# sieste/greb-climate-model

Measured on AMD Instinct MI355X. Metric: simulated-years/sec at 96x48 grid (ensemble aggregate); diffusion HBM GB/s vs roofline, higher is better.
Workload: dtype f32; 1 GPU; 96x48 GREB ensemble, 512 members/GPU x 1 GPU, CO2 sweep 280-1120 ppm, 32 scenario years after 1 flux-correction year, dt=12h, dt_crcl=0.5h; members_per_gpu=512, arithmetic=fast, gather=none (1 GPU)

## Files before the change

greb_climate_model_amd/csrc/greb_device.h:

```cpp
#pragma once
#include <hip/hip_runtime.h>

namespace greb {

constexpr int kMaxNy = 192;

struct RowTables {
  float dif_ccy, adv_ccy;
  float dif_ccx[kMaxNy], adv_ccx[kMaxNy];
  float dif_ccx2[kMaxNy], adv_ccx2[kMaxNy];
  int dif_time2[kMaxNy], adv_time2[kMaxNy];
  int subcycled[kMaxNy];
};

struct f4 {
  float v[4];
};

typedef __attribute__((address_space(3))) float lfloat;
typedef float vfloat4 __attribute__((ext_vector_type(4)));

__device__ __forceinline__ f4 ld4(const float* p) {
  const vfloat4 a = *reinterpret_cast<const vfloat4*>(p);
  return f4{{a.x, a.y, a.z, a.w}};
// ... 180 lines not shown
  }
}

__device__ __forceinline__ void adv_lon_full_fast(const Flux& f, const float T[12], const float w[12],
                                                  const float u[4], float cs, float d[4]) {
#pragma unroll
  for (int i = 0; i < 4; ++i) {
    const int c = 4 + i;
    const float em2 = w[c - 2] * (T[c] - T[c - 2]), ep2 = w[c + 2] * (T[c] - T[c + 2]);
    d[i] = cs * (split_p(u[i]) * (ep2 - f.Pp[c]) - split_m(u[i]) * (f.Pm[c - 1] + em2));
  }
}

__device__ __forceinline__ void adv_lon_sub_fast(const Flux& f, const float T[12], const float w[12],
                                                 const float u[4], float cs, bool last_quad, float d[4]) {
#pragma unroll
  for (int i = 0; i < 4; ++i) {
    const int c = 4 + i;
    const float am = 10.f * f.Pm[c - 1] + (4.f * f.Pm[c - 2] + f.Pm[c - 3]);
    float ap = 10.f * f.Pp[c] + (4.f * f.Pp[c + 1] + f.Pp[c + 2]);
    if (last_quad && i == 1)
      ap = 10.f * f.Pp[c] - w[c + 3] * (T[c + 1] - T[c + 3]);
    d[i] = cs * (-split_p(u[i]) * ap - split_m(u[i]) * am);
  }
}

__device__ __forceinline__ void clamp_add_fast(float T1h[4], float d[4]) {
#pragma unroll
  for (int i = 0; i < 4; ++i) {
    d[i] = (d[i] <= -T1h[i]) ? -0.9f * T1h[i] : d[i];
    T1h[i] = T1h[i] + d[i];
  }
}

__device__ __forceinline__ void lat_fast(const f4& T0, const f4& Tm2, const f4& Tm1, const f4& Tp1,
                                         const f4& Tp2, const f4& wm2, const f4& wm1, const f4& wp1,
                                         const f4& wp2, const float v[4], float ccy_dif, float am, float ap,
                                         float ddif[4], float dadv[4]) {
#pragma unroll
  for (int i = 0; i < 4; ++i) {
    const float t0 = T0.v[i];
    const float gm1 = wm1.v[i] * (Tm1.v[i] - t0), gp1 = wp1.v[i] * (Tp1.v[i] - t0);
    const float dm2 = wm2.v[i] * (t0 - Tm2.v[i]), dp2 = wp2.v[i] * (t0 - Tp2.v[i]);
    ddif[i] = ccy_dif * (gm1 + gp1);
    dadv[i] = ap * split_p(v[i]) * (dp2 - gp1) - am * split_m(v[i]) * (dm2 - gm1);
  }
}


__device__ __forceinline__ void adv_lon_full_pm(const Flux& f, const float T[12], const float w[12],
                                                const float um[4], const float up[4], float d[4]) {
#pragma unroll
  for (int i = 0; i < 4; ++i) {
    const int c = 4 + i;
    const float em2 = w[c - 2] * (T[c] - T[c - 2]), ep2 = w[c + 2] * (T[c] - T[c + 2]);
    d[i] = up[i] * (ep2 - f.Pp[c]) - um[i] * (f.Pm[c - 1] + em2);
  }
}
__device__ __forceinline__ void adv_lon_sub_pm(const Flux& f, const float T[12], const float w[12],
                                               const float um[4], const float up[4], bool last_quad, float d[4]) {
#pragma unroll
  for (int i = 0; i < 4; ++i) {
    const int c = 4 + i;
    const float am = 10.f * f.Pm[c - 1] + (4.f * f.Pm[c - 2] + f.Pm[c - 3]);
    float ap = 10.f * f.Pp[c] + (4.f * f.Pp[c + 1] + f.Pp[c + 2]);
    if (last_quad && i == 1) ap = 10.f * f.Pp[c] - w[c + 3] * (T[c + 1] - T[c + 3]);
    d[i] = -up[i] * ap - um[i] * am;
  }
}
__device__ __forceinline__ void lat_pm(const f4& T0, const f4& Tm2, const f4& Tm1, const f4& Tp1, const f4& Tp2,
                                       const f4& wm2, const f4& wm1, const f4& wp1, const f4& wp2,
                                       const float vm[4], const float vp[4], float ccy_dif, float ddif[4],
                                       float dadv[4]) {
#pragma unroll
  for (int i = 0; i < 4; ++i) {
    const float t0 = T0.v[i];
    const float gm1 = wm1.v[i] * (Tm1.v[i] - t0), gp1 = wp1.v[i] * (Tp1.v[i] - t0);
    const float dm2 = wm2.v[i] * (t0 - Tm2.v[i]), dp2 = wp2.v[i] * (t0 - Tp2.v[i]);
    ddif[i] = ccy_dif * (gm1 + gp1);
    dadv[i] = vp[i] * (dp2 - gp1) - vm[i] * (dm2 - gm1);
  }
}

__device__ __forceinline__ float wave_sum(float v) {
#pragma unroll
  for (int off = 32; off > 0; off >>= 1) v += __shfl_xor(v, off, 64);
  return v;
}

template <bool EXACT> __device__ __forceinline__ float fdiv(float a, float b) { return EXACT ? a / b : a * __builtin_amdgcn_rcpf(b); }
template <bool EXACT> __device__ __forceinline__ float flog(float x) { return EXACT ? logf(x) : __logf(x); }
template <bool EXACT> __device__ __forceinline__ float fexp(float x) { return EXACT ? expf(x) : __expf(x); }
template <bool EXACT> __device__ __forceinline__ float fsqrt(float x) { return EXACT ? sqrtf(x) : __builtin_amdgcn_sqrtf(x); }

constexpr unsigned kXNoIce = 1u << 0, kXNoHydro = 1u << 1, kXNoDeepOcean = 1u << 2, kXLwLinear = 1u << 3,
                   kXNoCirc = 1u << 4, kXNoQTransport = 1u << 5, kXQDiffOnly = 1u << 6, kXSstPlus1 = 1u << 7;

struct Phys {
  float sig, ct_sens, da_ice, a_no_ice, a_cloud, Tl_ice1, Tl_ice2, To_ice1, To_ice2;
  float co_turb, ce, cq_latent, cq_rain, z_air, r_qviwv, rho_air;
  float p_emi[10];
  float cap_ocean, cap_land, cap_air;
  float dt;
};

__device__ __forceinline__ float pow4_ref(float x) {
#pragma clang fp contract(off)
  return x * x * x * x;
}

template <bool EXACT = true>
__device__ __forceinline__ void sw_radiation(const Phys& P, float Ts, float z_topo, float glacier, float cld,
                                             float sw_solar, float& albedo, float& sw, unsigned xsw = 0) {
#pragma clang fp contract(off)
  const float a_atmos = cld * P.a_cloud;
  float a_surf = 0.f;
  if (z_topo >= 0.f) {
    if (Ts <= P.Tl_ice1) a_surf = P.a_no_ice + P.da_ice;
    if (Ts >= P.Tl_ice2) a_surf = P.a_no_ice;
    if (Ts > P.Tl_ice1 && Ts < P.Tl_ice2)
      a_surf = P.a_no_ice + P.da_ice * (1.f - fdiv<EXACT>(Ts - P.Tl_ice1, P.Tl_ice2 - P.Tl_ice1));
  } else {
    if (Ts <= P.To_ice1) a_surf = P.a_no_ice + P.da_ice;
    if (Ts >= P.To_ice2) a_surf = P.a_no_ice;
    if (Ts > P.To_ice1 && Ts < P.To_ice2)
      a_surf = P.a_no_ice + P.da_ice * (1.f - fdiv<EXACT>(Ts - P.To_ice1, P.To_ice2 - P.To_ice1));
  }
  if (glacier > 0.5f) a_surf = P.a_no_ice + P.da_ice;
  if (xsw & kXNoIce) a_surf = P.a_no_ice;
  albedo = a_surf + a_atmos - a_surf * a_atmos;
  sw = sw_solar * (1.f - albedo);
}

template <bool EXACT = true>
__device__ __forceinline__ void lw_radiation(const Phys& P, float Ts, float Ta, float q, float co2, float ez,
                                             float cld, float tclim, float& LWsurf, float& LWair_down,
                                             float& em, unsigned xsw = 0, float qclim = 0.f) {
#pragma clang fp contract(off)
  const float e_co2 = ez * co2;
  float e_vapor = ez * P.r_qviwv * q;
  if (xsw & kXLwLinear) e_vapor = ez * P.r_qviwv * qclim;
  float e = P.p_emi[3] * flog<EXACT>(P.p_emi[0] * e_co2 + P.p_emi[1] * e_vapor + P.p_emi[2]) + P.p_emi[6]
            + P.p_emi[4] * flog<EXACT>(P.p_emi[0] * e_co2 + P.p_emi[2])
            + P.p_emi[5] * flog<EXACT>(P.p_emi[1] * e_vapor + P.p_emi[2]);
  e = fdiv<EXACT>(P.p_emi[7] - cld, P.p_emi[8]) * (e - P.p_emi[9]) + P.p_emi[9];
  if (xsw & kXLwLinear) e = e + 0.022f / (0.15f * 24.f) * P.r_qviwv * (q - qclim);
  em = e;
  LWsurf = -P.sig * pow4_ref(Ts);
  const float dTrad = -0.16f * tclim - 5.f;
  LWair_down = -e * P.sig * pow4_ref(Ta + dTrad);
}

template <bool EXACT = true>
__device__ __forceinline__ void hydro(const Phys& P, float Ts, float q, float u, float v, float z_topo,
                                      float ez, float swet, float& Qlat, float& Qlat_air, float& dq_eva,
                                      float& dq_rain, unsigned xsw = 0) {
#pragma clang fp contract(off)
  if (xsw & kXNoHydro) { Qlat = Qlat_air = dq_eva = dq_rain = 0.f; return; }
  float abswind = fsqrt<EXACT>(u * u + v * v);
  if (z_topo > 0.f) abswind = fsqrt<EXACT>(abswind * abswind + 2.0f * 2.0f);
  if (z_topo < 0.f) abswind = fsqrt<EXACT>(abswind * abswind + 3.0f * 3.0f);
  float qs = 3.75e-3f * fexp<EXACT>(fdiv<EXACT>(17.08085f * (Ts - 273.15f), Ts - 273.15f + 234.175f));
  qs = qs * ez;
  Qlat = (q - qs) * abswind * P.cq_latent * P.rho_air * P.ce * swet;
  dq_eva = fdiv<EXACT>(fdiv<EXACT>(-Qlat, P.cq_latent), P.r_qviwv);
  dq_rain = P.cq_rain * q;
  Qlat_air = -dq_rain * P.cq_latent * P.r_qviwv;
}

template <bool EXACT = true>
__device__ __forceinline__ void deep_ocean(const Phys& P, float Ts, float To, float z_topo, float mld,
                                           float mld_prev, float z_ocean, float& dT_ocean, float& dTo,
                                           unsigned xsw = 0) {
#pragma clang fp contract(off)
  if (xsw & kXNoDeepOcean) { dT_ocean = dTo = 0.f; return; }
  float a = 0.f, b = 0.f;
  const float dmld = mld - mld_prev;
  if (z_topo < 0.f && Ts >= P.To_ice2 && dmld < 0.f) a = fdiv<EXACT>(-dmld, z_ocean - mld) * (Ts - To);
  if (z_topo < 0.f && Ts >= P.To_ice2 && dmld > 0.f) b = fdiv<EXACT>(dmld, mld) * (To - Ts);
  a = 0.5f * a; b = 0.5f * b;
  const float Tx = P.To_ice2 > Ts ? P.To_ice2 : Ts;
  a = a + fdiv<EXACT>(P.dt * P.co_turb * (Tx - To), P.cap_ocean * (z_ocean - mld));
  b = b + fdiv<EXACT>(P.dt * P.co_turb * (To - Tx), P.cap_ocean * mld);
  dTo = a; dT_ocean = b;
}

template <bool EXACT = true>
__device__ __forceinline__ float seaice(const Phys& P, float Ts, float z_topo, float glacier, float mld,
                                        float cap_surf, unsigned xsw = 0) {
#pragma clang fp contract(off)
  if (z_topo < 0.f) {
    if (Ts <= P.To_ice1) cap_surf = P.cap_land;
    if (Ts >= P.To_ice2) cap_surf = P.cap_ocean * mld;
    if (Ts > P.To_ice1 && Ts < P.To_ice2)
      cap_surf = P.cap_land + fdiv<EXACT>(P.cap_ocean * mld - P.cap_land, P.To_ice2 - P.To_ice1) * (Ts - P.To_ice1);
  }
  if (xsw & kXNoIce) {
    if (z_topo > 0.f) cap_surf = P.cap_land;
    if (z_topo < 0.f) cap_surf = P.cap_ocean * mld;
  }
  if (glacier > 0.5f) cap_surf = P.cap_land;
  return cap_surf;
}

}
```

greb_climate_model_amd/csrc/greb_engine.cpp:

```cpp
#include "../../include/greb_engine.h"

#include <hip/hip_runtime.h>

#include <cmath>
#include <cstdlib>
#include <cstdio>
#include <cstring>
#include <functional>
#include <map>
#include <mutex>
#include <new>
#include <string>
#include <vector>

#include "greb_kernels.h"
#include "greb_diag.h"
#include "greb_clim.h"
#include "greb_ens.h"

using namespace greb;

namespace {

thread_local std::string g_last_error;

int fail(greb_engine* e, int code, const std::string& msg);

#define HIP_TRY(e, expr)                                                                      \
  do {                                                                                        \
    hipError_t _err = (expr);                                                                 \
    if (_err != hipSuccess)                                                                   \
      return fail((e), (int)_err, std::string(#expr) + ": " + hipGetErrorString(_err));       \
  } while (0)

int nint_f(float x) { return (int)lroundf(x); }

void compute_row_tables(const greb_params& p, float kappa, int nx, int ny, RowTables& g) {
  std::memset(&g, 0, sizeof(g));
  const float dlon = 360.f / (float)nx, dlat = 180.f / (float)ny;
  const float deg = 2.f * p.pi * 6.371e6f / 360.f;
  const float dx = dlon, dy = dlat, dyy = dy * deg;
  const float dtc = (float)p.dt_crcl;
  g.dif_ccy = kappa * dtc / (dyy * dyy);
  g.adv_ccy = dtc / dyy / 2.f;
  for (int k = 0; k < ny; ++k) {
    const float lat = dlat * (float)(k + 1) - dlat / 2.f - 90.f;
    const float dxlat = dx * deg * cosf(2.f * p.pi / 360.f * lat);
    g.dif_ccx[k] = kappa * dtc / (dxlat * dxlat);
    g.adv_ccx[k] = dtc / dxlat / 2.f;
    g.subcycled[k] = !(dxlat > 2.5e5f);
    {
      float dd = (float)nint_f(dtc / (1.f * (dxlat * dxlat) / kappa));
      if (dd < 1.f) dd = 1.f;
      const int dtdff2 = (int)(dtc / dd);
      int t2 = dtdff2 == 0 ? 1 : nint_f(dtc / (float)dtdff2);
      g.dif_time2[k] = t2 < 1 ? 1 : t2;
      g.dif_ccx2[k] = kappa * (float)dtdff2 / (dxlat * dxlat);
    }
    {
      float dd = (float)nint_f(dtc / (dxlat / 10.0f / 1.f));
      if (dd < 1.f) dd = 1.f;
      const int dtdff2 = (int)(dtc / dd);
      int t2 = dtdff2 == 0 ? 1 : nint_f(dtc / (float)dtdff2);
      g.adv_time2[k] = t2 < 1 ? 1 : t2;
      g.adv_ccx2[k] = (float)dtdff2 / dxlat / 2.f;
    }
  }
}

Phys make_phys(const greb_params& p) {
  Phys P;
  P.sig = p.sig; P.ct_sens = p.ct_sens;
  P.da_ice = p.da_ice; P.a_no_ice = p.a_no_ice; P.a_cloud = p.a_cloud;
  P.Tl_ice1 = p.Tl_ice1; P.Tl_ice2 = p.Tl_ice2; P.To_ice1 = p.To_ice1; P.To_ice2 = p.To_ice2;
  P.co_turb = p.co_turb; P.ce = p.ce; P.cq_latent = p.cq_latent; P.cq_rain = p.cq_rain;
  P.z_air = p.z_air; P.r_qviwv = p.r_qviwv; P.rho_air = p.rho_air;
  for (int i = 0; i < 10; ++i) P.p_emi[i] = p.p_emi[i];
  P.cap_ocean = p.cp_ocean * p.rho_ocean;
  P.cap_land = p.cp_land * p.rho_land * p.d_land;
  P.cap_air = p.cp_air * p.rho_air * p.d_air;
  P.dt = (float)p.dt;
  return P;
}

template <typename T>
hipError_t dev_alloc(T** p, size_t n) { return hipMalloc(reinterpret_cast<void**>(p), n * sizeof(T)); }

struct StripPlan {
  RowsTask* step_tasks = nullptr;
  int n_step = 0;
  RowsTask head[kStepHeadTasks] = {};
  CircOrder circ;
  int form = 0;
  float ms_substep = 0.f, ms_call = 0.f;
  hipEvent_t ev[3] = {nullptr, nullptr, nullptr};
};

void free_plan(StripPlan& p) {
  if (p.step_tasks) (void)hipFree(p.step_tasks);
  circ_rows_free_order(&p.circ);
  for (hipEvent_t ev : p.ev) if (ev) (void)hipEventDestroy(ev);
  p = StripPlan{};
}

}

struct greb_engine {
  greb_params p{};
  int nx = 0, ny = 0, np = 0, nm = 0, device = 0;
  bool strict = false;
  unsigned xsw = 0;
  std::vector<unsigned> h_xsw;
  bool xsw_uniform = true;
  unsigned* xsw_dev = nullptr;
  float* co2_flux_dev = nullptr;
  int n_phys_sets = 1;
  bool shared_corr = true;
  bool fused = true;
  float *Xa = nullptr, *Xb = nullptr, *red = nullptr, *W2 = nullptr;
  hipStream_t stream = nullptr;
  hipStream_t copy_stream = nullptr;
  hipEvent_t ev_done[2] = {nullptr, nullptr};
  hipEvent_t ev_free[2] = {nullptr, nullptr};
  float *z_topo = nullptr, *glacier = nullptr, *sw_solar = nullptr;
  float *tclim = nullptr, *qclim = nullptr, *uclim = nullptr, *vclim = nullptr, *mldclim = nullptr,
        *cldclim = nullptr, *swetclim = nullptr;
  float *toclim = nullptr, *z_ocean = nullptr, *wz_air = nullptr, *wz_vapor = nullptr;
  float *state = nullptr, *acc = nullptr, *corr = nullptr;
  int *corr_index = nullptr, *tab_index = nullptr;
  RowTables* tabs = nullptr;
  Phys* phys = nullptr;
  float* co2_dev = nullptr; size_t co2_cap = 0;
  float* monthly_dev = nullptr; size_t monthly_cap = 0;
  float* bsum = nullptr;
  float* budget_dev = nullptr; size_t budget_cap = 0;
  long long budget_runs = 0;
  int n_patterns = 0, n_solar = 0;
  float *f_space = nullptr, *f_season = nullptr, *f_solar = nullptr;
  std::vector<greb_member_forcing> h_force;
  MemberForcing* force_dev = nullptr;
  int forced_members = 0;
  struct BoundSet {
    float* dev[kBoundaryFields] = {};
    bool own[kBoundaryFields] = {};
    unsigned over = 0;
    std::vector<float> t_last, q_last, toclim, z_topo, mld0;
  };
  std::vector<BoundSet> bound;
  std::vector<int> h_bset;
  int members_on_sets = 0;
  BoundarySet* bsets_dev = nullptr;
  int* bset_dev = nullptr;
  MemberForcing* neutral_force_dev = nullptr;
  float* yearly_dev = nullptr; size_t yearly_cap = 0;
  float* diag_out = nullptr; size_t diag_out_cap = 0;
  float* diag_reg = nullptr; size_t diag_reg_cap = 0;
  float* clim_out = nullptr; size_t clim_out_cap = 0;
  float* ens_out = nullptr; size_t ens_out_cap = 0;
  std::vector<RowTables> h_tabs;
  std::vector<int> h_tab_index;
  bool strips = false;
  enum { kCallNever, kCallTrial, kCallAlways } call = kCallNever;
  int cus = 0;
  int slots_granted = -1;
  std::map<int, StripPlan> plans;
  std::vector<Phys> h_phys;
  long long it_flux = 0;
  long long it_scnr = 0;
  unsigned long long* stamps = nullptr;
  std::string last_error;
};

namespace {
int fail(greb_engine* e, int code, const std::string& msg) {
  if (e) e->last_error = msg;
  g_last_error = msg;
  return code;
}

int nsub_of(const greb_params& p) {
  int t = nint_f((float)p.dt / (float)p.dt_crcl);
  return t < 1 ? 1 : t;
}

MemberArgs base_args(greb_engine* e) {
  MemberArgs a{};
  a.nx = e->nx; a.ny = e->ny; a.np = e->np;
  a.z_topo = e->z_topo; a.glacier = e->glacier; a.sw_solar = e->sw_solar;
  a.tclim = e->tclim; a.qclim = e->qclim; a.uclim = e->uclim; a.vclim = e->vclim;
  a.mldclim = e->mldclim; a.cldclim = e->cldclim; a.swetclim = e->swetclim;
  a.toclim = e->toclim; a.z_ocean = e->z_ocean; a.wz_air = e->wz_air; a.wz_vapor = e->wz_vapor;
  a.state = e->state; a.acc = e->acc; a.corr = e->corr; a.corr_index = e->corr_index;
  a.tabs = e->tabs; a.tab_index = e->tab_index; a.phys = e->phys;
  a.nsub = nsub_of(e->p);
  a.nsub = tuning_int("GREB_DEBUG_NSUB", a.nsub);
  a.co2_flux = e->p.co2_flux;
  a.ipx = e->p.ipx; a.ipy = e->p.ipy;
  a.xsw = e->xsw_uniform ? e->xsw : 0u;
  a.xsw_m = e->xsw_uniform ? nullptr : e->xsw_dev;
  a.co2_flux_m = e->co2_flux_dev;
  a.stamps = e->stamps;
  a.dbg = tuning_int("GREB_DEBUG_PHYS", 0);
  unsigned all = GREB_X_NO_CIRCULATION;
  for (unsigned x : e->h_xsw) all &= x;
  if (all) a.nsub = 0;
  if (e->members_on_sets > 0) { a.bsets = e->bsets_dev; a.bset_m = e->bset_dev; }
  return a;
}

void apply_forcing(const greb_engine* e, MemberArgs& a) {
  if (e->forced_members <= 0 && e->members_on_sets > 0) a.force_m = e->neutral_force_dev;
  if (e->forced_members <= 0) return;
  a.force_m = e->force_dev;
  a.f_space = e->f_space; a.f_season = e->f_season; a.f_solar = e->f_solar;
}

struct YearOut {
  float* mon; int mon_years, mon_y;
  float* bud = nullptr; int bud_years = 0, bud_y = 0;
};

MemberArgs scenario_args(greb_engine* e, int years, int y, const YearOut& o) {
  MemberArgs a = base_args(e);
  a.flux_phase = 0;
  a.it0 = e->it_scnr + 1 + (long long)y * kNT; a.nsteps = kNT;
  a.co2 = e->co2_dev; a.co2_stride = years; a.co2_year0 = y;
  a.monthly = o.mon; a.monthly_years = o.mon_years; a.year_out0 = o.mon_y;
  a.yearly = e->yearly_dev; a.yearly_years = years; a.yearly_year0 = y;
  if (o.bud) { a.bsum = e->bsum; a.brec = o.bud; a.brec_years = o.bud_years; a.brec_year0 = o.bud_y; }
  apply_forcing(e, a);
  return a;
}

bool is_forced(const greb_member_forcing& f) { return f.co2_pattern >= 0 || f.solar_table >= 0 || !(f.solar_scale == 1.f); }

bool calm_vapor(const greb_engine* e) { return (e->h_xsw[0] & GREB_X_VAPOR_DIFFUSION_ONLY) != 0; }

int check_transport_switches(greb_engine* e, const char* who, bool fused, const unsigned* sw, int n) {
  if (fused) return 0;
  for (int m = 1; m < n; ++m)
    if ((sw[m] ^ sw[0]) & GREB_X_VAPOR_DIFFUSION_ONLY)
      return fail(e, GREB_E_UNSUPPORTED,
                  std::string(who) + ": member " + std::to_string(m) + " differs from member 0 in GREB_X_VAPOR_DIFFUSION_ONLY, "
                  "which the any-grid engine applies to a whole launch -- run the two groups as two engines beside each "
                  "other (ensemble.run_beside)");
  return 0;
}

bool all_equal(const unsigned* sw, int n) {
  for (int m = 1; m < n; ++m) if (sw[m] != sw[0]) return false;
  return true;
}

int check_member_config(const char* who, const greb_params& p, const greb_member_config& c, int m) {
  const char* bad = nullptr;
  auto differ = [](float a, float b) { return std::memcmp(&a, &b, sizeof(float)) != 0; };
  if (differ(c.p.pi, p.pi)) bad = "pi";
  else if (differ(c.p.z_air, p.z_air)) bad = "z_air";
  else if (differ(c.p.z_vapor, p.z_vapor)) bad = "z_vapor";
  else if (c.p.dt != p.dt) bad = "dt";
  else if (c.p.dt_crcl != p.dt_crcl) bad = "dt_crcl";
  else if (c.p.ipx != p.ipx) bad = "ipx";
  else if (c.p.ipy != p.ipy) bad = "ipy";
  else if (c.p.year0 != p.year0) bad = "year0";
  if (bad)
    return fail(nullptr, GREB_E_INVALID, std::string(who) + ": member " + std::to_string(m) + ": " + bad +
                                             " differs from the engine-wide greb_params (it feeds data every member shares)");
  if (c.switches & ~0xffu)
    return fail(nullptr, GREB_E_INVALID, std::string(who) + ": member " + std::to_string(m) + ": unknown switch bits");
  return 0;
}

int ensure(greb_engine* e, float** buf, size_t* cap, size_t n) {
  if (*cap >= n) return 0;
  if (*buf) HIP_TRY(e, hipFree(*buf));
  *buf = nullptr; *cap = 0;
  HIP_TRY(e, dev_alloc(buf, n));
  *cap = n;
  return 0;
}

struct SlotLedger {
  std::mutex mu;
  struct Entry { greb_engine* e; int device, members, granted; };
  std::vector<Entry> entries;
} g_slots;

void ledger_register(greb_engine* e) {
  std::lock_guard<std::mutex> lock(g_slots.mu);
  g_slots.entries.push_back({e, e->device, e->nm, 0});
}
void ledger_release(greb_engine* e) {
  std::lock_guard<std::mutex> lock(g_slots.mu);
  for (size_t i = 0; i < g_slots.entries.size(); ++i)
    if (g_slots.entries[i].e == e) { g_slots.entries.erase(g_slots.entries.begin() + (long)i); break; }
}
int ledger_grant(greb_engine* e, int device_slots) {
  std::lock_guard<std::mutex> lock(g_slots.mu);
  long long members = 0, taken = 0;
  SlotLedger::Entry* mine = nullptr;
  for (auto& x : g_slots.entries) {
    if (x.device != e->device) continue;
    members += x.members;
    if (x.e == e) mine = &x; else taken += x.granted;
  }
  if (!mine) return 0;
  const long long share = (long long)device_slots * mine->members / std::max<long long>(1, members);
  mine->granted = (int)std::max<long long>(0, std::min<long long>(share, device_slots - taken));
  return mine->granted;
}

int check_circulation(greb_engine* e) {
  for (auto& kv : e->plans) {
    unsigned d[5] = {0, 0, 0, 0, 0};
    const int rc = circ_rows_status(kv.second.circ, d);
    if (rc == -1) {
      char buf[384];
      std::snprintf(buf, sizeof(buf),
                    "circulation launch given up: task %u waited more than %.1f s in sub-step %u for a neighbouring strip "
                    "(its count read %u, wanted %u) -- the launch was not resident as a whole (another process on the "
                    "device?); results are invalid, recreate the engine with GREB_F_NO_PERSISTENT",
                    d[0], kCircSpinTicks / 1e8, d[1], d[2], d[3]);
      return fail(e, GREB_E_STATE, buf);
    }
    if (rc) return fail(e, GREB_E_STATE, "circulation launch: status word unreadable");
  }
  return 0;
}

int make_strip_plan(greb_engine* e, int nrun, StripPlan& p) {
  if (e->cus <= 0) HIP_TRY(e, hipDeviceGetAttribute(&e->cus, hipDeviceAttributeMultiprocessorCount, e->device));
  if (e->call != greb_engine::kCallNever) {
    static const int slots_per_cu = tuning_int("GREB_CIRC_SLOTS_PER_CU", kStepRowsSlotsPerCu);
    if (e->slots_granted < 0) e->slots_granted = ledger_grant(e, e->cus * std::min(slots_per_cu, kStepRowsSlotsPerCu));
    HIP_TRY(e, circ_rows_make_order(e->h_tabs.data(), e->h_tab_index.data(), nrun, e->ny, e->slots_granted, &p.circ));
  }
  p.form = p.circ.n == 0 ? 1 : (e->call == greb_engine::kCallAlways ? 2 : 0);
  if (p.form != 2) {
    static const int step_slots = tuning_int("GREB_STEP_SLOTS_PER_CU", kStepRowsSlotsPerCu);
    HIP_TRY(e, step_rows_make_tasks(e->h_tabs.data(), e->h_tab_index.data(), nrun, e->ny, e->cus * step_slots, &p.step_tasks,
                                    &p.n_step, p.head));
  }
  if (p.form == 0)
    for (hipEvent_t& ev : p.ev) HIP_TRY(e, hipEventCreate(&ev));
  return 0;
}

int run_year(greb_engine* e, const MemberArgs& a, int nrun) {
  if (e->fused) {
    HIP_TRY(e, launch_member_kernel(a, nrun, e->strict, e->stream));
    return 0;
  }
  const size_t np = (size_t)e->np;
  StripPlan* plan = nullptr;
  if (e->strips && a.nsub > 0) {
    auto it = e->plans.find(nrun);
    if (it == e->plans.end()) {
      StripPlan p;
      if (int rc = make_strip_plan(e, nrun, p)) { free_plan(p); return rc; }
      it = e->plans.emplace(nrun, p).first;
    }
    plan = &it->second;
  }
  static const int steps = tuning_int("GREB_DEBUG_NSTEPS", kNT);
  bool trial = plan && plan->form == 0 && steps >= 16;
  int form = plan && plan->form != 1 ? 2 : 1;
  HIP_TRY(e, launch_pack_tracers(e->state, e->Xa, e->np, nrun, e->stream));
  for (int s = 0; s < steps; ++s) {
    const long long it = a.it0 + s;
    const int ityr = (int)((it - 1) % kNT) + 1;
    const size_t off = (size_t)(ityr - 1) * np;
    float *cur = e->Xa, *nxt = e->Xb;
    if (trial) {
      if (s == 2 || s == 5 || s == 8) HIP_TRY(e, hipEventRecord(plan->ev[s == 2 ? 0 : (s == 5 ? 1 : 2)], e->stream));
      if (s == 8) {
        HIP_TRY(e, hipEventSynchronize(plan->ev[2]));
        HIP_TRY(e, hipEventElapsedTime(&plan->ms_substep, plan->ev[0], plan->ev[1]));
        HIP_TRY(e, hipEventElapsedTime(&plan->ms_call, plan->ev[1], plan->ev[2]));
        form = plan->form = plan->ms_call <= plan->ms_substep ? 2 : 1;
        trial = false;
      } else form = (s >= 2 && s < 5) ? 1 : 2;
    }
    if (form == 2) {
      HIP_TRY(e, launch_circulation_rows(e->Xa, e->Xb, e->W2, e->uclim + off, e->vclim + off, e->tabs, plan->circ, e->cus * 4, e->nx, e->ny,
                                         a.nsub, e->strict, e->stream, calm_vapor(e)));
      if (a.nsub & 1) cur = e->Xb;
    } else
    for (int tt = 0; tt < a.nsub; ++tt) {
      if (plan)
        HIP_TRY(e, launch_substep_rows(cur, e->W2, e->uclim + off, e->vclim + off, nxt, e->tabs, e->tab_index, plan->step_tasks,
                                       plan->head, plan->n_step, e->cus * 4, e->nx, e->ny, e->strict, e->stream, calm_vapor(e)));
      else
        HIP_TRY(e, launch_substep_fused(cur, e->W2, e->uclim + off, e->vclim + off, nxt, e->tabs, e->tab_index, e->nx,
                                        e->ny, nrun, e->strict, e->stream, calm_vapor(e)));
      float* t = cur; cur = nxt; nxt = t;
    }
    MemberArgs b = a;
    b.it0 = it; b.nsteps = 1;
    HIP_TRY(e, launch_physics_step(b, cur, e->Xa, e->red, nrun, e->strict, e->stream));
    if (ityr == kNT && a.yearly)
      HIP_TRY(e, launch_yearly(e->red, a.yearly, e->np, e->nx, a.ipx, a.ipy, a.yearly_years, a.yearly_year0, nrun, e->strict, e->stream));
  }
  return 0;
}
}

extern "C" {

void greb_params_default(greb_params* p) {
  std::memset(p, 0, sizeof(*p));
  p->pi = 3.1416f; p->sig = 5.6704e-8f; p->rho_ocean = 999.1f; p->rho_land = 2600.f; p->rho_air = 1.2f;
  p->cp_ocean = 4186.f; p->cp_land = 926.222f; p->cp_air = 1005.f; p->eps = 1.f;
  p->d_ocean = 50.f; p->d_land = 2.f; p->d_air = 5000.f; p->ct_sens = 22.5f; p->da_ice = 0.25f;
  p->a_no_ice = 0.1f; p->a_cloud = 0.35f;
  p->Tl_ice1 = 273.15f - 10.f; p->Tl_ice2 = 273.15f; p->To_ice1 = 273.15f - 7.f; p->To_ice2 = 273.15f - 1.7f;
  p->co_turb = 5.0f; p->kappa = 8e5f; p->ce = 2e-3f; p->cq_latent = 2.257e6f;
  p->cq_rain = -0.1f / 24.f / 3600.f; p->z_air = 8400.f; p->z_vapor = 5000.f; p->r_qviwv = 2.6736e3f;
  const float pe[10] = {9.0721f, 106.7252f, 61.5562f, 0.0179f, 0.0028f, 0.0570f, 0.3462f, 2.3406f, 0.7032f, 1.0662f};
  std::memcpy(p->p_emi, pe, sizeof(pe));
  p->co2_flux = 298.f;
  p->ipx = 1; p->ipy = 1; p->year0 = 1940; p->dt = 12 * 3600; p->dt_crcl = 1800;
}

const char* greb_engine_last_error(const greb_engine* e) {
  return e ? e->last_error.c_str() : g_last_error.c_str();
}

const char* greb_device_info(int device) {
  static thread_local std::string s;
  int n = 0;
  if (hipGetDeviceCount(&n) != hipSuccess || n <= device || device < 0) {
    s = "{\"error\": \"no HIP device\"}";
    return s.c_str();
  }
  hipDeviceProp_t pr;
  if (hipGetDeviceProperties(&pr, device) != hipSuccess) { s = "{\"error\": \"hipGetDeviceProperties\"}"; return s.c_str(); }
  char buf[512];
  std::snprintf(buf, sizeof(buf),
                "{\"name\": \"%s\", \"arch\": \"%s\", \"cus\": %d, \"clock_mhz\": %d, \"mem_clock_mhz\": %d, "
                "\"hbm_gb\": %.1f, \"lds_per_block\": %zu, \"l2_mb\": %.1f, \"wave\": %d}",
                pr.name, pr.gcnArchName, pr.multiProcessorCount, pr.clockRate / 1000, pr.memoryClockRate / 1000,
                pr.totalGlobalMem / 1073741824.0, pr.sharedMemPerBlock, pr.l2CacheSize / 1048576.0, pr.warpSize);
  s = buf;
  return s.c_str();
}

}

namespace {
void derive_fields(const greb_params& p, size_t np, const float* z_topo, const float* tclim, const float* mldclim, float* toclim,
                   float* z_ocean, float* wz_air, float* wz_vapor) {
  for (size_t i = 0; i < np; ++i) {
    if (tclim) {
      float mn = tclim[i];
      for (int t = 0; t < kNT; ++t) { const float v = tclim[(size_t)t * np + i]; if (v < mn) mn = v; }
      if (mn - 273.15f < -1.7f) mn = -1.7f + 273.15f;
      toclim[i] = mn;
    }
    if (mldclim) {
      float mx = 0.f;
      for (int t = 0; t < kNT; ++t) { const float d = mldclim[(size_t)t * np + i]; if (d > mx) mx = d; }
      z_ocean[i] = 3.0f * mx;
    }
    if (z_topo) {
      wz_air[i] = expf(-z_topo[i] / p.z_air);
      wz_vapor[i] = expf(-z_topo[i] / p.z_vapor);
    }
  }
}

void initial_state(const greb_engine::BoundSet& b, const Phys& P, size_t np, float* st) {
  for (size_t i = 0; i < np; ++i) {
    st[i] = b.t_last[i]; st[np + i] = st[i]; st[2 * np + i] = b.toclim[i]; st[3 * np + i] = b.q_last[i];
    float c = 0.f;
    if (b.z_topo[i] > 0.f) c = P.cap_land;
    if (b.z_topo[i] <= 0.f) c = P.cap_ocean * b.mld0[i];
    st[4 * np + i] = c;
  }
}

const char* const kBoundaryNames[kBoundaryFields] = {"z_topo", "glacier", "tclim", "qclim", "uclim", "vclim", "mldclim", "cldclim",
                                                     "swetclim", "toclim", "z_ocean", "wz_air", "wz_vapor"};
enum { kBfZtopo, kBfGlacier, kBfTclim, kBfQclim, kBfUclim, kBfVclim, kBfMld, kBfCld, kBfSwet, kBfToclim, kBfZocean, kBfWzAir, kBfWzVapor };
size_t boundary_floats(int field, size_t np) { return (field >= kBfTclim && field <= kBfSwet) ? np * kNT : np; }

hipError_t copy_shared_corrections(greb_engine* e, float** corr, const char** what) {
  const size_t nm = (size_t)e->nm, set = (size_t)3 * kNT * e->np;
  hipError_t err = hipStreamSynchronize(e->stream);
  *what = "hipStreamSynchronize";
  if (err != hipSuccess) return err;
  *what = "hipMalloc of the members' correction sets";
  if ((err = dev_alloc(corr, nm * set)) != hipSuccess) return err;
  *what = "hipMemcpy";
  for (size_t m = 0; m < nm; ++m)
    if ((err = hipMemcpy(*corr + m * set, e->corr, set * sizeof(float), hipMemcpyDeviceToDevice)) != hipSuccess) return err;
  return hipSuccess;
}
hipError_t adopt_member_corrections(greb_engine* e, float* corr) {
  std::vector<int> corr_index((size_t)e->nm);
  for (int m = 0; m < e->nm; ++m) corr_index[(size_t)m] = m;
  hipError_t err = hipMemcpy(e->corr_index, corr_index.data(), corr_index.size() * sizeof(int), hipMemcpyHostToDevice);
  if (err != hipSuccess) return err;
  (void)hipFree(e->corr);
  e->corr = corr;
  e->shared_corr = false;
  return hipSuccess;
}

int create_engine(const char* who, const greb_params* p, int nx, int ny, const greb_fields* f, int n_members,
                  const greb_member_config* members, int device, unsigned flags, greb_engine** out) {
  if (!p || !f || !out || !members || n_members < 1 || nx < 12 || (nx & 3) || ny < 5 || ny > kMaxNy)
    return fail(nullptr, GREB_E_INVALID, std::string(who) + ": bad argument");
  for (int m = 0; m < n_members; ++m)
    if (int rc = check_member_config(who, *p, members[m], m)) return rc;
  int ndev = 0;
  if (hipGetDeviceCount(&ndev) != hipSuccess || ndev < 1 || device < 0 || device >= ndev)
    return fail(nullptr, GREB_E_NOGPU, std::string(who) + ": no HIP device (the engine has no CPU path)");
  bool fused = true;
  std::vector<unsigned> switches((size_t)n_members);
  for (int m = 0; m < n_members; ++m) {
    RowTables t; compute_row_tables(*p, members[m].p.kappa, nx, ny, t);
    fused = fused && member_layout_supported(t, nx, ny);
    switches[(size_t)m] = members[m].switches;
  }
  fused = fused && !(flags & GREB_F_MULTILAUNCH);
  if (p->ipx < 1 || p->ipx > nx || p->ipy < 1 || p->ipy > ny)
    return fail(nullptr, GREB_E_INVALID, std::string(who) + ": ipx/ipy outside the grid");
  if (int rc = check_transport_switches(nullptr, who, fused, switches.data(), n_members)) return rc;
  greb_engine* e = new (std::nothrow) greb_engine();
  if (!e) return fail(nullptr, GREB_E_INVALID, "out of host memory");
  *out = e;
  e->p = *p; e->nx = nx; e->ny = ny; e->np = nx * ny; e->nm = n_members; e->device = device;
  e->strict = (flags & GREB_F_STRICT) != 0;
  e->fused = fused;
  e->h_xsw = switches;
  e->xsw_uniform = all_equal(switches.data(), n_members);
  e->xsw = e->xsw_uniform ? switches[0] : 0u;
  const size_t np = (size_t)e->np, n3 = np * kNT, nm = (size_t)n_members;
  HIP_TRY(e, hipSetDevice(device));
  HIP_TRY(e, hipStreamCreate(&e->stream));

  auto up = [&](float** d, const float* h, size_t n) -> hipError_t {
    hipError_t err = dev_alloc(d, n);
    if (err != hipSuccess) return err;
    return hipMemcpy(*d, h, n * sizeof(float), hipMemcpyHostToDevice);
  };
  HIP_TRY(e, up(&e->z_topo, f->z_topo, np));
  HIP_TRY(e, up(&e->glacier, f->glacier, np));
  HIP_TRY(e, up(&e->sw_solar, f->sw_solar, (size_t)kNT * ny));
  HIP_TRY(e, up(&e->tclim, f->tclim, n3));
  HIP_TRY(e, up(&e->qclim, f->qclim, n3));
  HIP_TRY(e, up(&e->uclim, f->uclim, n3));
  HIP_TRY(e, up(&e->vclim, f->vclim, n3));
  HIP_TRY(e, up(&e->mldclim, f->mldclim, n3));
  HIP_TRY(e, up(&e->cldclim, f->cldclim, n3));
  HIP_TRY(e, up(&e->swetclim, f->swetclim, n3));

  std::vector<float> toclim(np), z_ocean(np), wz_air(np), wz_vapor(np);
  derive_fields(*p, np, f->z_topo, f->tclim, f->mldclim, toclim.data(), z_ocean.data(), wz_air.data(), wz_vapor.data());
  HIP_TRY(e, up(&e->toclim, toclim.data(), np));
  HIP_TRY(e, up(&e->z_ocean, z_ocean.data(), np));
  HIP_TRY(e, up(&e->wz_air, wz_air.data(), np));
  HIP_TRY(e, up(&e->wz_vapor, wz_vapor.data(), np));
  {
    const size_t last = (size_t)(kNT - 1) * np;
    greb_engine::BoundSet b0;
    float* const dev[kBoundaryFields] = {e->z_topo, e->glacier, e->tclim, e->qclim, e->uclim, e->vclim, e->mldclim, e->cldclim,
                                         e->swetclim, e->toclim, e->z_ocean, e->wz_air, e->wz_vapor};
    for (int i = 0; i < kBoundaryFields; ++i) b0.dev[i] = dev[i];
    b0.t_last.assign(f->tclim + last, f->tclim + last + np); b0.q_last.assign(f->qclim + last, f->qclim + last + np);
    b0.toclim = toclim; b0.z_topo.assign(f->z_topo, f->z_topo + np); b0.mld0.assign(f->mldclim, f->mldclim + np);
    e->bound.push_back(std::move(b0));
  }

  e->h_phys.resize(nm);
  std::vector<int> tab_index(nm), corr_index(nm);
  std::vector<float> kappas;
  e->shared_corr = true;
  std::vector<float> co2_flux(nm);
  bool own_co2_flux = false;
  std::vector<size_t> phys_sets;
  for (size_t m = 0; m < nm; ++m) {
    e->h_phys[m] = make_phys(members[m].p);
    const float kap = members[m].p.kappa;
    co2_flux[m] = members[m].p.co2_flux;
    own_co2_flux = own_co2_flux || !(co2_flux[m] == p->co2_flux);
    size_t ps = 0;
    for (; ps < phys_sets.size(); ++ps) if (!std::memcmp(&e->h_phys[phys_sets[ps]], &e->h_phys[m], sizeof(Phys))) break;
    if (ps == phys_sets.size()) phys_sets.push_back(m);
    size_t ti = 0;
    for (; ti < kappas.size(); ++ti) if (kappas[ti] == kap) break;
    if (ti == kappas.size()) {
      kappas.push_back(kap);
      RowTables t; compute_row_tables(*p, kap, nx, ny, t);
      e->h_tabs.push_back(t);
    }
    tab_index[m] = (int)ti;
    if (ps != 0 || ti != 0 || !(co2_flux[m] == co2_flux[0]) || switches[m] != switches[0]) e->shared_corr = false;
  }
  e->n_phys_sets = (int)phys_sets.size();
  if (own_co2_flux) {
    HIP_TRY(e, dev_alloc(&e->co2_flux_dev, nm));
    HIP_TRY(e, hipMemcpy(e->co2_flux_dev, co2_flux.data(), nm * sizeof(float), hipMemcpyHostToDevice));
  }
  if (!e->xsw_uniform) {
    HIP_TRY(e, dev_alloc(&e->xsw_dev, nm));
    HIP_TRY(e, hipMemcpy(e->xsw_dev, switches.data(), nm * sizeof(unsigned), hipMemcpyHostToDevice));
  }
  for (size_t m = 0; m < nm; ++m) corr_index[m] = e->shared_corr ? 0 : (int)m;
  HIP_TRY(e, dev_alloc(&e->phys, nm));
  HIP_TRY(e, hipMemcpy(e->phys, e->h_phys.data(), nm * sizeof(Phys), hipMemcpyHostToDevice));
  HIP_TRY(e, dev_alloc(&e->tabs, e->h_tabs.size()));
  HIP_TRY(e, hipMemcpy(e->tabs, e->h_tabs.data(), e->h_tabs.size() * sizeof(RowTables), hipMemcpyHostToDevice));
  HIP_TRY(e, dev_alloc(&e->tab_index, nm));
  HIP_TRY(e, hipMemcpy(e->tab_index, tab_index.data(), nm * sizeof(int), hipMemcpyHostToDevice));
  e->h_tab_index = tab_index;
  HIP_TRY(e, dev_alloc(&e->corr_index, nm));
  HIP_TRY(e, hipMemcpy(e->corr_index, corr_index.data(), nm * sizeof(int), hipMemcpyHostToDevice));

  const size_t ncorr = e->shared_corr ? 1 : nm;
  HIP_TRY(e, dev_alloc(&e->corr, ncorr * 3 * n3));
  HIP_TRY(e, hipMemset(e->corr, 0, ncorr * 3 * n3 * sizeof(float)));
  HIP_TRY(e, dev_alloc(&e->acc, nm * 6 * np));
  HIP_TRY(e, hipMemset(e->acc, 0, nm * 6 * np * sizeof(float)));

  std::vector<float> st(5 * np);
  HIP_TRY(e, dev_alloc(&e->state, nm * 5 * np));
  for (size_t m = 0; m < nm; ++m) {
    initial_state(e->bound[0], e->h_phys[m], np, st.data());
    HIP_TRY(e, hipMemcpy(e->state + m * 5 * np, st.data(), 5 * np * sizeof(float), hipMemcpyHostToDevice));
  }
  if (!e->fused) {
    HIP_TRY(e, dev_alloc(&e->Xa, nm * 2 * np));
    HIP_TRY(e, dev_alloc(&e->Xb, nm * 2 * np));
    HIP_TRY(e, dev_alloc(&e->red, nm * np));
    HIP_TRY(e, dev_alloc(&e->W2, 2 * np));
    HIP_TRY(e, hipMemcpy(e->W2, wz_air.data(), np * sizeof(float), hipMemcpyHostToDevice));
    HIP_TRY(e, hipMemcpy(e->W2 + np, wz_vapor.data(), np * sizeof(float), hipMemcpyHostToDevice));
    static const bool no_step_rows = tuning_int("GREB_NO_STEP_ROWS", 0) != 0;
    e->strips = !no_step_rows && (!e->strict || (flags & GREB_F_ROW_STRIPS)) &&
                n_members < (1 << (kStepFieldBits - 1)) &&
                step_rows_supported(e->h_tabs.data(), (int)e->h_tabs.size(), nx, ny);
    if (e->strips && !(flags & GREB_F_NO_PERSISTENT)) {
      e->call = (flags & GREB_F_PERSISTENT) ? greb_engine::kCallAlways : greb_engine::kCallTrial;
      ledger_register(e);
    }
  }
  return 0;
}

int clear_yearly(greb_engine* e, int years) {
  const size_t n = (size_t)e->nm * years * 2;
  if (int rc = ensure(e, &e->yearly_dev, &e->yearly_cap, n)) return rc;
  HIP_TRY(e, hipMemsetAsync(e->yearly_dev, 0, n * sizeof(float), e->stream));
  return 0;
}
int finish_years(greb_engine* e) {
  HIP_TRY(e, hipStreamSynchronize(e->stream));
  return check_circulation(e);
}
int yearly_to_host(greb_engine* e, int years, float* yearly) {
  if (yearly) HIP_TRY(e, hipMemcpy(yearly, e->yearly_dev, (size_t)e->nm * years * 2 * sizeof(float), hipMemcpyDeviceToHost));
  return 0;
}

size_t year_records(const greb_engine* e) { return (size_t)e->nm * 12 * 5 * (size_t)e->np; }
float* staging_slot(const greb_engine* e, int y) { return e->monthly_dev + (size_t)(y & 1) * year_records(e); }

hipError_t unit_to_host(greb_engine* e, float* host, int n, int u, const float* dev, size_t rec) {
  return hipMemcpy2DAsync(host + (size_t)u * rec, (size_t)n * rec * sizeof(float), dev, rec * sizeof(float), rec * sizeof(float),
                          (size_t)e->nm, hipMemcpyDeviceToHost, e->copy_stream);
}

struct YearCalls {
  std::function<int(int y, const YearOut& o)> integrate;
  std::function<int(int u)> writing;
  std::function<int(int u)> complete;
};

struct RunSink {
  std::function<int()> prepare;
  std::function<int(const YearCalls&, int y)> year;
  std::function<int(int u, int slot)> deliver;
  std::function<int()> finish;
};

int run_years(greb_engine* e, int years, const float* co2_ppm, float* yearly, const RunSink& s) {
  HIP_TRY(e, hipSetDevice(e->device));
  const size_t nm = (size_t)e->nm;
  if (int rc = ensure(e, &e->co2_dev, &e->co2_cap, nm * years)) return rc;
  HIP_TRY(e, hipMemcpyAsync(e->co2_dev, co2_ppm, nm * years * sizeof(float), hipMemcpyHostToDevice, e->stream));
  if (int rc = clear_yearly(e, years)) return rc;
  const bool delivers = (bool)s.deliver;
  if (delivers) if (int rc = ensure(e, &e->monthly_dev, &e->monthly_cap, 2 * year_records(e))) return rc;
  if (int rc = s.prepare()) { e->last_error = g_last_error; return rc; }
  if (delivers && !e->copy_stream) HIP_TRY(e, hipStreamCreateWithFlags(&e->copy_stream, hipStreamNonBlocking));
  for (int i = 0; delivers && i < 2; ++i) {
    if (!e->ev_done[i]) HIP_TRY(e, hipEventCreateWithFlags(&e->ev_done[i], hipEventDisableTiming));
    if (!e->ev_free[i]) HIP_TRY(e, hipEventCreateWithFlags(&e->ev_free[i], hipEventDisableTiming));
  }
  int completed = 0, delivered = 0;
  YearCalls calls;
  calls.integrate = [&](int y, const YearOut& o) -> int { return run_year(e, scenario_args(e, years, y, o), e->nm); };
  calls.writing = [&](int u) -> int {
    if (u >= 2) HIP_TRY(e, hipStreamWaitEvent(e->stream, e->ev_free[u & 1], 0));
    return 0;
  };
  calls.complete = [&](int u) -> int {
    HIP_TRY(e, hipEventRecord(e->ev_done[u & 1], e->stream));
    completed = u + 1;
    return 0;
  };
  auto deliver = [&](int u) -> int {
    HIP_TRY(e, hipStreamWaitEvent(e->copy_stream, e->ev_done[u & 1], 0));
    if (int rc = s.deliver(u, u & 1)) return rc;
    HIP_TRY(e, hipEventRecord(e->ev_free[u & 1], e->copy_stream));
    return 0;
  };
  const int rc_years = [&]() -> int {
    for (int y = 0; y < years; ++y) {
      const int before = completed;
      if (int rc = s.year(calls, y)) return rc;
      for (; delivered < before; ++delivered) if (int rc = deliver(delivered)) return rc;
    }
    for (; delivered < completed; ++delivered) if (int rc = deliver(delivered)) return rc;
    if (delivers) HIP_TRY(e, hipStreamSynchronize(e->copy_stream));
    return 0;
  }();
  if (rc_years && delivers) {
    (void)hipStreamSynchronize(e->copy_stream);
    (void)hipStreamSynchronize(e->stream);
  }
  if (rc_years) return rc_years;
  if (int rc = finish_years(e)) return rc;
  e->it_scnr += (long long)years * kNT;
  if (s.finish) if (int rc = s.finish()) return rc;
  return yearly_to_host(e, years, yearly);
}

int run_records(greb_engine* e, int years, const float* co2_ppm, float* monthly, float* budget, float* yearly,
                unsigned run_flags) {
  const size_t np = (size_t)e->np, nm = (size_t)e->nm;
  const size_t rec_year = 12 * 5 * np, bud_year = (size_t)12 * GREB_NBUDGET * np;
  const bool dev_out = (run_flags & GREB_RUN_DEVICE_OUT) != 0;
  auto budget_slot = [&](int y) { return e->budget_dev + (size_t)(y & 1) * nm * bud_year; };
  RunSink s;
  s.prepare = [&]() -> int {
    if (!budget) return 0;
    if (!e->bsum) {
      HIP_TRY(e, dev_alloc(&e->bsum, nm * GREB_NBUDGET * np));
      HIP_TRY(e, hipMemsetAsync(e->bsum, 0, nm * GREB_NBUDGET * np * sizeof(float), e->stream));
    }
    ++e->budget_runs;
    if (!dev_out) return ensure(e, &e->budget_dev, &e->budget_cap, 2 * nm * bud_year);
    return monthly ? 0 : ensure(e, &e->monthly_dev, &e->monthly_cap, year_records(e));
  };
  if (dev_out) {
    s.year = [&](const YearCalls& run, int y) -> int {
      return run.integrate(y, monthly ? YearOut{monthly, years, y, budget, years, y} : YearOut{e->monthly_dev, 1, 0, budget, years, y});
    };
    return run_years(e, years, co2_ppm, yearly, s);
  }
  s.year = [&](const YearCalls& run, int y) -> int {
    if (int rc = run.writing(y)) return rc;
    if (int rc = run.integrate(y, {staging_slot(e, y), 1, 0, budget ? budget_slot(y) : nullptr, 1, 0})) return rc;
    return run.complete(y);
  };
  s.deliver = [&](int y, int sl) -> int {
    if (monthly) HIP_TRY(e, unit_to_host(e, monthly, years, y, staging_slot(e, sl), rec_year));
    if (budget) HIP_TRY(e, unit_to_host(e, budget, years, y, budget_slot(sl), bud_year));
    return 0;
  };
  return run_years(e, years, co2_ppm, yearly, s);
}
}

extern "C" {

int greb_engine_create_members(const greb_params* p, int nx, int ny, const greb_fields* f, int n_members,
                               const greb_member_config* members, int device, unsigned flags, greb_engine** out) {
  return create_engine("greb_engine_create_members", p, nx, ny, f, n_members, members, device, flags, out);
}

int greb_engine_create(const greb_params* p, int nx, int ny, const greb_fields* f, int n_members,
                       const greb_member_overrides* overrides, int device, unsigned flags, greb_engine** out) {
  if (!p || n_members < 1) return fail(nullptr, GREB_E_INVALID, "greb_engine_create: bad argument");
  std::vector<greb_member_config> members((size_t)n_members);
  auto pick = [](float base, float ov) { return std::isnan(ov) ? base : ov; };
  for (int m = 0; m < n_members; ++m) {
    greb_member_config& c = members[(size_t)m];
    c.p = *p; c.switches = 0;
    if (!overrides) continue;
    c.p.da_ice = pick(p->da_ice, overrides[m].da_ice);
    c.p.a_no_ice = pick(p->a_no_ice, overrides[m].a_no_ice);
    c.p.a_cloud = pick(p->a_cloud, overrides[m].a_cloud);
    c.p.kappa = pick(p->kappa, overrides[m].kappa);
  }
  return create_engine("greb_engine_create", p, nx, ny, f, n_members, members.data(), device, flags, out);
}

int greb_engine_destroy(greb_engine* e) {
  if (!e) return 0;
  (void)hipSetDevice(e->device);
  void* ptrs[] = {e->z_topo, e->glacier, e->sw_solar, e->tclim, e->qclim, e->uclim, e->vclim, e->mldclim,
                  e->cldclim, e->swetclim, e->toclim, e->z_ocean, e->wz_air, e->wz_vapor, e->state, e->acc,
                  e->corr, e->corr_index, e->tab_index, e->tabs, e->phys, e->co2_dev, e->monthly_dev, e->yearly_dev,
                  e->Xa, e->Xb, e->red, e->W2, e->xsw_dev, e->co2_flux_dev, e->diag_out, e->diag_reg, e->clim_out, e->ens_out, e->bsum, e->budget_dev,
                  e->f_space, e->f_season, e->f_solar, e->force_dev, e->bsets_dev, e->bset_dev, e->neutral_force_dev};
  for (void* q : ptrs) if (q) (void)hipFree(q);
  for (size_t k = 1; k < e->bound.size(); ++k)
    for (int i = 0; i < kBoundaryFields; ++i) if (e->bound[k].own[i]) (void)hipFree(e->bound[k].dev[i]);
  for (auto& kv : e->plans) free_plan(kv.second);
  if (e->call != greb_engine::kCallNever) ledger_release(e);
  for (int i = 0; i < 2; ++i) {
    if (e->ev_done[i]) (void)hipEventDestroy(e->ev_done[i]);
    if (e->ev_free[i]) (void)hipEventDestroy(e->ev_free[i]);
  }
  if (e->copy_stream) (void)hipStreamDestroy(e->copy_stream);
  if (e->stream) (void)hipStreamDestroy(e->stream);
  delete e;
  return 0;
}

int greb_engine_flux_correction(greb_engine* e, int years, float* yearly) {
  if (!e || years < 0) return fail(e, GREB_E_INVALID, "flux_correction: bad argument");
  if (years == 0) return 0;
  HIP_TRY(e, hipSetDevice(e->device));
  const size_t np = (size_t)e->np;
  const int nrun = e->shared_corr ? 1 : e->nm;
  if (int rc = clear_yearly(e, years)) return rc;
  for (int y = 0; y < years; ++y) {
    MemberArgs a = base_args(e);
    a.flux_phase = 1;
    a.it0 = e->it_flux + 1 + (long long)y * kNT; a.nsteps = kNT;
    a.monthly = nullptr; a.monthly_years = years; a.year_out0 = y;
    a.yearly = e->yearly_dev; a.yearly_years = years; a.yearly_year0 = y;
    if (int rc = run_year(e, a, nrun)) return rc;
  }
  if (e->shared_corr && e->nm > 1) {
    for (int m = 1; m < e->nm; ++m)
      HIP_TRY(e, hipMemcpyAsync(e->state + (size_t)m * 5 * np, e->state, 5 * np * sizeof(float),
                                hipMemcpyDeviceToDevice, e->stream));
  }
  if (int rc = finish_years(e)) return rc;
  e->it_flux += (long long)years * kNT;
  if (int rc = yearly_to_host(e, years, yearly)) return rc;
  if (yearly && e->shared_corr)
    for (int m = 1; m < e->nm; ++m) std::memcpy(yearly + (size_t)m * years * 2, yearly, (size_t)years * 2 * sizeof(float));
  return 0;
}

int greb_engine_run(greb_engine* e, int years, const float* co2_ppm, float* monthly, float* yearly,
                    unsigned run_flags) {
  if (!e || years < 1 || !co2_ppm || !monthly) return fail(e, GREB_E_INVALID, "run: bad argument");
  return run_records(e, years, co2_ppm, monthly, nullptr, yearly, run_flags);
}

int greb_engine_run_budget(greb_engine* e, int years, const float* co2_ppm, float* monthly, float* budget, float* yearly,
                           unsigned run_flags) {
  if (!e || years < 1 || !co2_ppm) return fail(e, GREB_E_INVALID, "run_budget: bad argument (engine, years or co2_ppm)");
  if (!budget) return fail(e, GREB_E_INVALID, "run_budget: `budget` is NULL (greb_engine_run is the run without budget output)");
  return run_records(e, years, co2_ppm, monthly, budget, yearly, run_flags);
}

const char* greb_budget_name(int i) {
  static const char* const names[GREB_NBUDGET] = {"sw", "LW_surf", "LWair_down", "LW_abs", "Q_sens", "Q_lat", "Q_lat_air",
                                                  "dq_eva", "dq_rain", "dT_ocean", "dTo", "dTa_crcl", "dq_crcl"};
  return i >= 0 && i < GREB_NBUDGET ? names[i] : nullptr;
}

}

struct greb_diag {
  int nx = 0, ny = 0, nr = 0;
  std::vector<double> w;
  std::vector<double> inv_sum;
  struct Dev { int device; double* w; double* inv_sum; double* partials; size_t partials_cap; };
  std::vector<Dev> devs;
};

namespace {
int diag_on_device(greb_diag* d, int device, int n_members, bool regions, greb_diag::Dev** out) {
  greb_diag::Dev* dv = nullptr;
  for (auto& x : d->devs) if (x.device == device) dv = &x;
  if (!dv) {
    greb_diag::Dev n{device, nullptr, nullptr, nullptr, 0};
    HIP_TRY(nullptr, dev_alloc(&n.w, d->w.size()));
    hipError_t err = dev_alloc(&n.inv_sum, d->inv_sum.size());
    if (err == hipSuccess) err = hipMemcpy(n.w, d->w.data(), d->w.size() * sizeof(double), hipMemcpyHostToDevice);
    if (err == hipSuccess) err = hipMemcpy(n.inv_sum, d->inv_sum.data(), d->inv_sum.size() * sizeof(double), hipMemcpyHostToDevice);
    if (err != hipSuccess) {
      (void)hipFree(n.w);
      if (n.inv_sum) (void)hipFree(n.inv_sum);
      HIP_TRY(nullptr, err);
    }
    d->devs.push_back(n);
    dv = &d->devs.back();
  }
  const size_t need = regions ? diag_partials(d->nx, d->ny, n_members, d->nr) : 0;
  if (dv->partials_cap < need) {
    if (dv->partials) {
      HIP_TRY(nullptr, hipDeviceSynchronize());
      HIP_TRY(nullptr, hipFree(dv->partials));
      dv->partials = nullptr; dv->partials_cap = 0;
    }
    HIP_TRY(nullptr, dev_alloc(&dv->partials, need));
    dv->partials_cap = need;
  }
  *out = dv;
  return 0;
}

DiagArgs diag_args(const greb_diag* d, const greb_diag::Dev* dv, const float* monthly, float* regions, size_t regions_stride,
                   float* zonal, float* annual) {
  DiagArgs a{};
  a.monthly = monthly; a.nx = d->nx; a.ny = d->ny; a.nr = d->nr;
  a.w = dv->w; a.inv_sum = dv->inv_sum; a.partials = dv->partials;
  a.regions = regions; a.regions_stride = regions_stride; a.zonal = zonal; a.annual = annual;
  return a;
}
}

extern "C" {

int greb_diag_create(int nx, int ny, const float* region_w, int n_regions, greb_diag** out) {
  if (!out) return fail(nullptr, GREB_E_INVALID, "diag_create: `out` is NULL");
  *out = nullptr;
  if (nx < 12 || (nx & 3) || ny < 5 || ny > kMaxNy)
    return fail(nullptr, GREB_E_INVALID, "diag_create: grid " + std::to_string(nx) + " x " + std::to_string(ny) +
                                             " (nx % 4 == 0, nx >= 12, 5 <= ny <= " + std::to_string(kMaxNy) + ")");
  if (n_regions < 0 || n_regions > kDiagMaxRegions)
    return fail(nullptr, GREB_E_INVALID, "diag_create: n_regions = " + std::to_string(n_regions) + " (0 ... " +
                                             std::to_string(kDiagMaxRegions) + "; the globe is region 0 on top of them)");
  if (n_regions > 0 && !region_w) return fail(nullptr, GREB_E_INVALID, "diag_create: region_w is NULL with n_regions > 0");
  const size_t np = (size_t)nx * ny;
  for (int k = 0; k < n_regions; ++k)
    for (size_t i = 0; i < np; ++i) {
      const float v = region_w[(size_t)k * np + i];
      if (!(v >= 0.f && v <= 1.f)) {
        char buf[160];
        std::snprintf(buf, sizeof(buf), "diag_create: region %d: weight %g at row %zu, column %zu is not in [0, 1]", k + 1,
                      (double)v, i / (size_t)nx, i % (size_t)nx);
        return fail(nullptr, GREB_E_INVALID, buf);
      }
    }
  greb_diag* d = new (std::nothrow) greb_diag();
  if (!d) return fail(nullptr, GREB_E_INVALID, "out of host memory");
  d->nx = nx; d->ny = ny; d->nr = 1 + n_regions;
  d->w.resize((size_t)d->nr * np);
  d->inv_sum.resize((size_t)d->nr);
  const double pi = 3.14159265358979323846;
  for (int r = 0; r < d->nr; ++r) {
    double sum = 0.0;
    for (int j = 0; j < ny; ++j) {
      const double c = std::cos(((j + 0.5) * 180.0 / ny - 90.0) * pi / 180.0);
      for (int i = 0; i < nx; ++i) {
        const size_t q = (size_t)j * nx + i;
        const double w = r == 0 ? c : (double)region_w[(size_t)(r - 1) * np + q] * c;
        d->w[(size_t)r * np + q] = w;
        sum += w;
      }
    }
// ... 403 lines not shown
  }
  for (int g = 0; g < n_groups; ++g)
    if (count[(size_t)g] == 0) return fail(nullptr, GREB_E_INVALID, "ens_create: group " + std::to_string(g) + " is empty");
  EnsProbs pr{};
  if (what & GREB_S_QUANTILES) {
    if (n_probs < 1 || n_probs > kEnsMaxProbs || !probs)
      return fail(nullptr, GREB_E_INVALID, "ens_create: GREB_S_QUANTILES with n_probs = " + std::to_string(n_probs) +
                                               (probs ? "" : " and `probs` NULL") + " (1 ... " + std::to_string(kEnsMaxProbs) + ")");
    pr.n = n_probs;
    for (int i = 0; i < n_probs; ++i) {
      if (!(probs[i] >= 0.f && probs[i] <= 1.f)) {
        char buf[128];
        std::snprintf(buf, sizeof(buf), "ens_create: probability %d = %g is not in [0, 1]", i, (double)probs[i]);
        return fail(nullptr, GREB_E_INVALID, buf);
      }
      pr.p[i] = probs[i];
    }
    for (int g = 0; g < n_groups; ++g)
      if (count[(size_t)g] > kEnsMaxSorted)
        return fail(nullptr, GREB_E_UNSUPPORTED, "ens_create: GREB_S_QUANTILES with group " + std::to_string(g) + " of " +
                                                     std::to_string(count[(size_t)g]) + " members (at most " +
                                                     std::to_string(kEnsMaxSorted) + " are sorted in one compute unit's LDS)");
  }
  greb_ens* s = new (std::nothrow) greb_ens();
  if (!s) return fail(nullptr, GREB_E_INVALID, "out of host memory");
  s->nx = nx; s->ny = ny; s->nm = n_members; s->ng = n_groups; s->what = what; s->probs = pr; s->has_control = control != nullptr;
  s->offs.assign((size_t)n_groups + 1, 0);
  for (int g = 0; g < n_groups; ++g) s->offs[(size_t)g + 1] = s->offs[(size_t)g] + count[(size_t)g];
  s->member.resize((size_t)s->offs[(size_t)n_groups]);
  if (control) s->control.resize(s->member.size());
  std::vector<int> at(s->offs.begin(), s->offs.end() - 1);
  for (int m = 0; m < n_members; ++m) {
    if (group[m] < 0) continue;
    const size_t k = (size_t)at[(size_t)group[m]]++;
    s->member[k] = m;
    if (control) s->control[k] = control[m];
  }
  *out = s;
  return 0;
}

int greb_ens_destroy(greb_ens* s) {
  if (!s) return 0;
  int prev = 0;
  const bool have_prev = !s->devs.empty() && hipGetDevice(&prev) == hipSuccess;
  for (auto& x : s->devs)
    if (hipSetDevice(x.device) == hipSuccess) {
      (void)hipDeviceSynchronize();
      (void)hipFree(x.lists);
    }
  if (have_prev) (void)hipSetDevice(prev);
  delete s;
  return 0;
}

int greb_ens_reduce_dev(greb_ens* s, int device, const float* x_dev, size_t n, float* mean_dev, float* var_dev, float* min_dev,
                        float* max_dev, float* quant_dev, void* stream) {
  if (!s) return fail(nullptr, GREB_E_INVALID, "ens_reduce_dev: no plan (greb_ens is NULL)");
  if (!x_dev) return fail(nullptr, GREB_E_INVALID, "ens_reduce_dev: x_dev is NULL");
  if (reinterpret_cast<uintptr_t>(x_dev) & 15) return fail(nullptr, GREB_E_INVALID, "ens_reduce_dev: x_dev is not 16-byte aligned");
  if (n < 1) return fail(nullptr, GREB_E_INVALID, "ens_reduce_dev: n = 0");
  size_t size[5];
  ens_sizes(s, n, size);
  float* out[5] = {mean_dev, var_dev, min_dev, max_dev, quant_dev};
  for (int i = 0; i < 5; ++i) {
    if (!size[i]) { out[i] = nullptr; continue; }
    if (!out[i])
      return fail(nullptr, GREB_E_INVALID, std::string("ens_reduce_dev: ") + kEnsFlagNames[i] + " selected but `" + kEnsOutNames[i] +
                                               "_dev` is NULL");
  }
  int ndev = 0;
  if (hipGetDeviceCount(&ndev) != hipSuccess || ndev < 1 || device < 0 || device >= ndev)
    return fail(nullptr, GREB_E_NOGPU, "ens_reduce_dev: no HIP device (no CPU path)");
  HIP_TRY(nullptr, hipSetDevice(device));
  EnsLists l{};
  if (int rc = ens_on_device(s, device, &l)) return rc;
  return ens_launch(nullptr, s, l, x_dev, n, out, (hipStream_t)stream);
}

int greb_engine_run_ens(greb_engine* e, int years, const float* co2_ppm, greb_ens* s, float* mean, float* var, float* min,
                        float* max, float* quant, float* yearly) {
  if (!s) return fail(e, GREB_E_INVALID, "run_ens: no plan (greb_ens is NULL)");
  if (years < 1) return fail(e, GREB_E_INVALID, "run_ens: years = " + std::to_string(years));
  const size_t n = (size_t)12 * 5 * s->nx * s->ny;
  size_t size[5];
  ens_sizes(s, n, size);
  float* host[5] = {mean, var, min, max, quant};
  for (int i = 0; i < 5; ++i)
    if (size[i] && !host[i])
      return fail(e, GREB_E_INVALID, std::string("run_ens: ") + kEnsFlagNames[i] + " selected but `" + kEnsOutNames[i] + "` is NULL");
  if (!e || !co2_ppm) return fail(e, GREB_E_INVALID, "run_ens: bad argument (engine or co2_ppm)");
  if (s->nx != e->nx || s->ny != e->ny)
    return fail(e, GREB_E_INVALID, "run_ens: the plan's grid " + std::to_string(s->nx) + " x " + std::to_string(s->ny) +
                                       " differs from the engine's " + std::to_string(e->nx) + " x " + std::to_string(e->ny));
  if (s->nm != e->nm)
    return fail(e, GREB_E_INVALID, "run_ens: the plan is for " + std::to_string(s->nm) + " members, the engine has " +
                                       std::to_string(e->nm));
  const size_t ng = (size_t)s->ng;
  size_t at[5], out_slot = 0;
  for (int i = 0; i < 5; ++i) { at[i] = out_slot; out_slot += ng * size[i]; }
  EnsLists l{};
  RunSink k;
  k.prepare = [&]() -> int {
    if (int rc = ensure(e, &e->ens_out, &e->ens_out_cap, 2 * out_slot)) return rc;
    return ens_on_device(s, e->device, &l);
  };
  k.year = [&](const YearCalls& run, int y) -> int {
    float* mon = staging_slot(e, y);
    if (int rc = run.integrate(y, {mon, 1, 0})) return rc;
    if (int rc = run.writing(y)) return rc;
    float* out[5];
    for (int i = 0; i < 5; ++i) out[i] = size[i] ? e->ens_out + (size_t)(y & 1) * out_slot + at[i] : nullptr;
    if (int rc = ens_launch(e, s, l, mon, n, out, e->stream)) return rc;
    return run.complete(y);
  };
  k.deliver = [&](int y, int sl) -> int {
    for (int i = 0; i < 5; ++i)
      if (size[i])
        HIP_TRY(e, hipMemcpy2DAsync(host[i] + (size_t)y * size[i], (size_t)years * size[i] * sizeof(float),
                                    e->ens_out + (size_t)sl * out_slot + at[i], size[i] * sizeof(float), size[i] * sizeof(float), ng,
                                    hipMemcpyDeviceToHost, e->copy_stream));
    return 0;
  };
  return run_years(e, years, co2_ppm, yearly, k);
}

const char* greb_engine_describe(greb_engine* e) {
  static thread_local std::string s;
  if (!e) { s = "{}"; return s.c_str(); }
  char buf[256];
  std::snprintf(buf, sizeof(buf), "{\"grid\": [%d, %d], \"members\": %d, \"arithmetic\": \"%s\", \"engine\": \"%s\"", e->nx, e->ny, e->nm,
                e->strict ? "strict" : "fast", e->fused ? "fused member kernel" : (e->strips ? "row strips" : "latitude bands"));
  s = buf;
  std::snprintf(buf, sizeof(buf), ", \"member_switches\": \"%s\", \"correction_sets\": %d, \"physics_sets\": %d",
                e->xsw_uniform ? "uniform" : "per member", e->shared_corr ? 1 : e->nm, e->n_phys_sets);
  s += buf;
  std::snprintf(buf, sizeof(buf), ", \"budget_runs\": %lld", e->budget_runs);
  s += buf;
  std::snprintf(buf, sizeof(buf), ", \"forcing\": {\"patterns\": %d, \"solar_tables\": %d, \"forced_members\": %d}", e->n_patterns,
                e->n_solar, e->forced_members);
  s += buf;
  std::snprintf(buf, sizeof(buf), ", \"boundary\": {\"sets\": %d, \"members_on_sets\": %d, \"fields\": [", (int)e->bound.size() - 1,
                e->members_on_sets);
  s += buf;
  for (size_t k = 1; k < e->bound.size(); ++k) {
    s += k > 1 ? ", [" : "[";
    bool first = true;
    for (int i = 0; i < kBoundaryInputs; ++i)
      if (e->bound[k].over & (1u << i)) { s += std::string(first ? "\"" : ", \"") + kBoundaryNames[i] + "\""; first = false; }
    s += "]";
  }
  s += "]}";
  {
    unsigned v;
    auto family = [&v](const MemberArgs& a) { return select_variant(a, &v) == hipSuccess ? variant_family(v) : "none"; };
    MemberArgs flux = base_args(e), scenario = base_args(e);
    flux.flux_phase = 1;
    apply_forcing(e, scenario);
    std::snprintf(buf, sizeof(buf), ", \"kernel_family\": {\"flux_correction\": \"%s\", \"scenario\": \"%s\"}", family(flux),
                  family(scenario));
    s += buf;
  }
  if (e->call != greb_engine::kCallNever) {
    std::snprintf(buf, sizeof(buf), ", \"wavefront_slots_granted\": %d, \"circulation\": [", e->slots_granted);
    s += buf;
    bool first = true;
    for (const auto& kv : e->plans) {
      const StripPlan& p = kv.second;
      std::snprintf(buf, sizeof(buf), "%s{\"members_run\": %d, \"tasks_of_one_launch_per_call\": %d, \"form\": \"%s\", \"trial_ms_per_3_steps\": [%.4f, %.4f]}",
                    first ? "" : ", ", kv.first, p.circ.n,
                    p.circ.n == 0 ? "one launch per sub-step (slots)" : (p.form == 2 ? "one launch per call" : (p.form == 1 ? "one launch per sub-step" : "undecided")),
                    p.ms_substep, p.ms_call);
      s += buf;
      first = false;
    }
    s += "]";
  }
  s += "}";
  return s.c_str();
}

int greb_engine_get_state(greb_engine* e, int member, float* state5) {
  if (!e || member < 0 || member >= e->nm || !state5) return fail(e, GREB_E_INVALID, "get_state: bad argument");
  HIP_TRY(e, hipSetDevice(e->device));
  HIP_TRY(e, hipMemcpy(state5, e->state + (size_t)member * 5 * e->np, (size_t)5 * e->np * sizeof(float), hipMemcpyDeviceToHost));
  return 0;
}

int greb_engine_get_corrections(greb_engine* e, int member, float* corr, float* state5) {
  if (!e || member < 0 || member >= e->nm) return fail(e, GREB_E_INVALID, "get_corrections: bad argument");
  HIP_TRY(e, hipSetDevice(e->device));
  const size_t n = (size_t)3 * kNT * e->np, ci = e->shared_corr ? 0 : (size_t)member;
  if (corr) HIP_TRY(e, hipMemcpy(corr, e->corr + ci * n, n * sizeof(float), hipMemcpyDeviceToHost));
  if (state5) return greb_engine_get_state(e, member, state5);
  return 0;
}

static_assert(GREB_V_FLUX == kVFlux && GREB_V_SWITCHES == kVExp && GREB_V_BUDGET == kVBudget && GREB_V_FORCING == kVForce &&
              GREB_V_BOUNDARY == kVBound, "variant bits mirror the ABI");
static_assert(GREB_X_NO_ICE == kXNoIce && GREB_X_NO_HYDRO == kXNoHydro && GREB_X_NO_DEEP_OCEAN == kXNoDeepOcean &&
              GREB_X_LW_LINEAR_VAPOR == kXLwLinear && GREB_X_NO_CIRCULATION == kXNoCirc &&
              GREB_X_NO_VAPOR_TRANSPORT == kXNoQTransport && GREB_X_VAPOR_DIFFUSION_ONLY == kXQDiffOnly &&
              GREB_X_SST_PLUS1 == kXSstPlus1, "device switch constants mirror the ABI");

unsigned greb_log_exp_switches(int le) {
  unsigned x = 0;
  if (le <= 5) x |= GREB_X_NO_ICE;
  if (le <= 6 || le == 13 || le == 15) x |= GREB_X_NO_HYDRO;
  if (le <= 9 || le == 11 || (le >= 14 && le <= 16)) x |= GREB_X_NO_DEEP_OCEAN;
  if (le == 11) x |= GREB_X_LW_LINEAR_VAPOR;
  if (le <= 4) x |= GREB_X_NO_CIRCULATION;
  if (le == 7 || le == 16) x |= GREB_X_NO_VAPOR_TRANSPORT;
  if (le == 8) x |= GREB_X_VAPOR_DIFFUSION_ONLY;
  if (le >= 14 && le <= 16) x |= GREB_X_SST_PLUS1;
  return x;
}

int greb_engine_set_experiment(greb_engine* e, unsigned switches) {
  if (!e || (switches & ~0xffu)) return fail(e, GREB_E_INVALID, "set_experiment: unknown switch bits");
  e->xsw = switches;
  e->h_xsw.assign((size_t)e->nm, switches);
  e->xsw_uniform = true;
  return 0;
}

int greb_engine_set_member_experiments(greb_engine* e, const uint32_t* switches) {
  if (!e || !switches) return fail(e, GREB_E_INVALID, "set_member_experiments: bad argument");
  const size_t nm = (size_t)e->nm;
  for (size_t m = 0; m < nm; ++m)
    if (switches[m] & ~0xffu)
      return fail(e, GREB_E_INVALID, "set_member_experiments: member " + std::to_string(m) + ": unknown switch bits");
  std::vector<unsigned> sw(switches, switches + nm);
  if (int rc = check_transport_switches(e, "set_member_experiments", e->fused, sw.data(), e->nm)) return rc;
  const bool uniform = all_equal(sw.data(), e->nm);
  HIP_TRY(e, hipSetDevice(e->device));
  unsigned* xsw_dev = nullptr;
  float* corr = nullptr;
  auto step = [&](hipError_t err, const char* what) -> int {
    if (err == hipSuccess) return 0;
    if (corr) (void)hipFree(corr);
    if (xsw_dev) (void)hipFree(xsw_dev);
    return fail(e, (int)err, std::string("set_member_experiments: ") + what + ": " + hipGetErrorString(err));
  };
  if (!uniform) {
    if (int rc = step(dev_alloc(&xsw_dev, nm), "hipMalloc")) return rc;
    if (int rc = step(hipMemcpy(xsw_dev, sw.data(), nm * sizeof(unsigned), hipMemcpyHostToDevice), "hipMemcpy")) return rc;
    if (e->shared_corr && nm > 1) {
      const char* what = "";
      const hipError_t err = copy_shared_corrections(e, &corr, &what);
      if (int rc = step(err, what)) return rc;
      if (int rc = step(adopt_member_corrections(e, corr), "hipMemcpy")) return rc;
    }
  }
  if (xsw_dev) {
    if (e->xsw_dev) (void)hipFree(e->xsw_dev);
    e->xsw_dev = xsw_dev;
  }
  e->h_xsw = sw;
  e->xsw_uniform = uniform;
  e->xsw = uniform ? sw[0] : 0u;
  return 0;
}

static_assert(sizeof(greb_member_forcing) == sizeof(MemberForcing) && sizeof(MemberForcing) == 16,
              "the kernels read greb_member_forcing as it is");

int greb_engine_set_forcing_tables(greb_engine* e, int n_patterns, const float* co2_space, const float* co2_season, int n_solar,
                                   const float* sw_solar) {
  const char* who = "set_forcing_tables: ";
  if (!e) return fail(nullptr, GREB_E_INVALID, std::string(who) + "no engine (greb_engine is NULL)");
  if (n_patterns < 0 || n_patterns > GREB_MAX_FORCING_TABLES)
    return fail(e, GREB_E_INVALID, who + ("n_patterns = " + std::to_string(n_patterns)) + " (0 ... " + std::to_string(GREB_MAX_FORCING_TABLES) + ")");
  if (n_solar < 0 || n_solar > GREB_MAX_FORCING_TABLES)
    return fail(e, GREB_E_INVALID, who + ("n_solar = " + std::to_string(n_solar)) + " (0 ... " + std::to_string(GREB_MAX_FORCING_TABLES) + ")");
  if (n_patterns > 0 && !co2_space) return fail(e, GREB_E_INVALID, std::string(who) + "co2_space is NULL with n_patterns > 0");
  if (n_solar > 0 && !sw_solar) return fail(e, GREB_E_INVALID, std::string(who) + "sw_solar is NULL with n_solar > 0");
  const size_t np = (size_t)e->np, nx = (size_t)e->nx, ny = (size_t)e->ny;
  char buf[200];
  for (int k = 0; k < n_patterns; ++k) {
    for (size_t i = 0; i < np; ++i) {
      const float v = co2_space[(size_t)k * np + i];
      if (!(v >= 0.f && v <= 1.f)) {
        std::snprintf(buf, sizeof(buf), "%sco2_space: pattern %d: weight %g at row %zu, column %zu is not in [0, 1]", who, k, (double)v,
                      i / nx, i % nx);
        return fail(e, GREB_E_INVALID, buf);
      }
    }
    for (int t = 0; co2_season && t < kNT; ++t) {
      const float v = co2_season[(size_t)k * kNT + t];
      if (!(v >= 0.f && v <= 1.f)) {
        std::snprintf(buf, sizeof(buf), "%sco2_season: pattern %d: weight %g at step %d is not in [0, 1]", who, k, (double)v, t + 1);
        return fail(e, GREB_E_INVALID, buf);
      }
    }
  }
  for (int t = 0; t < n_solar; ++t)
    for (size_t i = 0; i < (size_t)kNT * ny; ++i) {
      const float v = sw_solar[(size_t)t * kNT * ny + i];
      if (!(v >= 0.f && std::isfinite(v))) {
        std::snprintf(buf, sizeof(buf), "%ssw_solar: table %d: value %g at step %zu, row %zu is negative or not finite", who, t, (double)v,
                      i / ny + 1, i % ny);
        return fail(e, GREB_E_INVALID, buf);
      }
    }
  for (size_t m = 0; m < e->h_force.size(); ++m) {
    const greb_member_forcing& f = e->h_force[m];
    if (f.co2_pattern >= n_patterns || f.solar_table >= n_solar) {
      std::snprintf(buf, sizeof(buf), "%smember %zu is forced with co2_pattern %d, solar_table %d: outside the new %d patterns, %d tables "
                    "(change or clear the member forcing first)", who, m, f.co2_pattern, f.solar_table, n_patterns, n_solar);
      return fail(e, GREB_E_INVALID, buf);
    }
  }
  HIP_TRY(e, hipSetDevice(e->device));
  float *space = nullptr, *season = nullptr, *solar = nullptr;
  auto step = [&](hipError_t err, const char* what) -> int {
    if (err == hipSuccess) return 0;
    if (space) (void)hipFree(space);
    if (season) (void)hipFree(season);
    if (solar) (void)hipFree(solar);
    return fail(e, (int)err, std::string(who) + what + ": " + hipGetErrorString(err));
  };
  if (n_patterns > 0) {
    std::vector<float> ones;
    if (!co2_season) ones.assign((size_t)n_patterns * kNT, 1.f);
    if (int rc = step(dev_alloc(&space, (size_t)n_patterns * np), "hipMalloc")) return rc;
    if (int rc = step(dev_alloc(&season, (size_t)n_patterns * kNT), "hipMalloc")) return rc;
    if (int rc = step(hipMemcpy(space, co2_space, (size_t)n_patterns * np * sizeof(float), hipMemcpyHostToDevice), "hipMemcpy")) return rc;
    if (int rc = step(hipMemcpy(season, co2_season ? co2_season : ones.data(), (size_t)n_patterns * kNT * sizeof(float),
                                hipMemcpyHostToDevice), "hipMemcpy")) return rc;
  }
  if (n_solar > 0) {
    if (int rc = step(dev_alloc(&solar, (size_t)n_solar * kNT * ny), "hipMalloc")) return rc;
    if (int rc = step(hipMemcpy(solar, sw_solar, (size_t)n_solar * kNT * ny * sizeof(float), hipMemcpyHostToDevice), "hipMemcpy")) return rc;
  }
  if (int rc = step(hipStreamSynchronize(e->stream), "hipStreamSynchronize")) return rc;
  if (e->f_space) (void)hipFree(e->f_space);
  if (e->f_season) (void)hipFree(e->f_season);
  if (e->f_solar) (void)hipFree(e->f_solar);
  e->f_space = space; e->f_season = season; e->f_solar = solar;
  e->n_patterns = n_patterns; e->n_solar = n_solar;
  return 0;
}

int greb_engine_set_member_forcing(greb_engine* e, const greb_member_forcing* f) {
  const char* who = "set_member_forcing: ";
  if (!e) return fail(nullptr, GREB_E_INVALID, std::string(who) + "no engine (greb_engine is NULL)");
  if (!f) {
    e->h_force.clear();
    e->forced_members = 0;
    return 0;
  }
  const size_t nm = (size_t)e->nm;
  char buf[200];
  int forced = 0;
  for (size_t m = 0; m < nm; ++m) {
    const greb_member_forcing& x = f[m];
    buf[0] = 0;
    if (x.co2_pattern < -1 || x.co2_pattern >= e->n_patterns)
      std::snprintf(buf, sizeof(buf), "%smember %zu: co2_pattern %d is outside -1 ... %d (set_forcing_tables gave %d patterns)", who, m,
                    x.co2_pattern, e->n_patterns - 1, e->n_patterns);
    else if (x.solar_table < -1 || x.solar_table >= e->n_solar)
      std::snprintf(buf, sizeof(buf), "%smember %zu: solar_table %d is outside -1 ... %d (set_forcing_tables gave %d tables)", who, m,
                    x.solar_table, e->n_solar - 1, e->n_solar);
    else if (x.co2_pattern >= 0 && !(std::isfinite(x.co2_ref) && x.co2_ref > 0.f))
      std::snprintf(buf, sizeof(buf), "%smember %zu: co2_ref %g is not finite or not positive", who, m, (double)x.co2_ref);
    else if (!(std::isfinite(x.solar_scale) && x.solar_scale >= 0.f))
      std::snprintf(buf, sizeof(buf), "%smember %zu: solar_scale %g is not finite or negative", who, m, (double)x.solar_scale);
    if (buf[0]) return fail(e, GREB_E_INVALID, buf);
    forced += is_forced(x);
  }
  std::vector<MemberForcing> w(nm);
  for (size_t m = 0; m < nm; ++m)
    w[m] = MemberForcing{f[m].co2_pattern, f[m].co2_pattern >= 0 ? f[m].co2_ref : 1.f, f[m].solar_table, f[m].solar_scale};
  if (forced > 0) {
    HIP_TRY(e, hipSetDevice(e->device));
    MemberForcing* dev = nullptr;
    HIP_TRY(e, dev_alloc(&dev, nm));
    hipError_t err = hipMemcpy(dev, w.data(), nm * sizeof(MemberForcing), hipMemcpyHostToDevice);
    if (err == hipSuccess) err = hipStreamSynchronize(e->stream);
    if (err != hipSuccess) { (void)hipFree(dev); HIP_TRY(e, err); }
    if (e->force_dev) (void)hipFree(e->force_dev);
    e->force_dev = dev;
  }
  e->h_force.assign(f, f + nm);
  e->forced_members = forced;
  return 0;
}

static_assert(GREB_MAX_BOUNDARY_SETS == kMaxBoundarySets, "the set table's size mirrors the ABI");

int greb_engine_add_boundary_set(greb_engine* e, const greb_fields* over, int* set_id) {
  const char* who = "add_boundary_set: ";
  if (!e) return fail(nullptr, GREB_E_INVALID, std::string(who) + "no engine (greb_engine is NULL)");
  if (!over || !set_id) return fail(e, GREB_E_INVALID, std::string(who) + (over ? "set_id is NULL" : "`over` is NULL"));
  if (over->sw_solar)
    return fail(e, GREB_E_INVALID, std::string(who) + "sw_solar is not part of a boundary set: insolation tables are per-member forcing "
                                   "(greb_engine_set_forcing_tables, greb_engine_set_member_forcing)");
  const float* const src[kBoundaryInputs] = {over->z_topo, over->glacier, over->tclim, over->qclim, over->uclim, over->vclim,
                                             over->mldclim, over->cldclim, over->swetclim};
  unsigned mask = 0;
  for (int i = 0; i < kBoundaryInputs; ++i) if (src[i]) mask |= 1u << i;
  if (!mask) return fail(e, GREB_E_INVALID, std::string(who) + "every field of `over` is NULL: the set would be the engine's own data (set 0)");
  if ((int)e->bound.size() - 1 >= GREB_MAX_BOUNDARY_SETS)
    return fail(e, GREB_E_INVALID, who + ("the engine already has " + std::to_string(GREB_MAX_BOUNDARY_SETS)) + " boundary sets (GREB_MAX_BOUNDARY_SETS)");
  const size_t np = (size_t)e->np;
  for (int i = 0; i < kBoundaryInputs; ++i)
    for (size_t j = 0, n = src[i] ? boundary_floats(i, np) : 0; j < n; ++j)
      if (!std::isfinite(src[i][j])) {
        char buf[160];
        std::snprintf(buf, sizeof(buf), "%s%s: value %g at index %zu is not finite", who, kBoundaryNames[i], (double)src[i][j], j);
        return fail(e, GREB_E_INVALID, buf);
      }
  HIP_TRY(e, hipSetDevice(e->device));
  greb_engine::BoundSet b = e->bound[0];
  for (bool& o : b.own) o = false;
  b.over = mask;
  auto step = [&](hipError_t err, const char* what) -> int {
    if (err == hipSuccess) return 0;
    for (int i = 0; i < kBoundaryFields; ++i) if (b.own[i]) (void)hipFree(b.dev[i]);
    return fail(e, (int)err, std::string(who) + what + ": " + hipGetErrorString(err));
  };
  auto put = [&](int field, const float* host) -> int {
    float* d = nullptr;
    if (int rc = step(dev_alloc(&d, boundary_floats(field, np)), "hipMalloc")) return rc;
    b.dev[field] = d; b.own[field] = true;
    return step(hipMemcpy(d, host, boundary_floats(field, np) * sizeof(float), hipMemcpyHostToDevice), "hipMemcpy");
  };
  for (int i = 0; i < kBoundaryInputs; ++i)
    if (src[i]) if (int rc = put(i, src[i])) return rc;
  std::vector<float> toclim(over->tclim ? np : 0), z_ocean(over->mldclim ? np : 0), wz_air(over->z_topo ? np : 0), wz_vapor(over->z_topo ? np : 0);
  derive_fields(e->p, np, over->z_topo, over->tclim, over->mldclim, toclim.data(), z_ocean.data(), wz_air.data(), wz_vapor.data());
  if (over->tclim) { if (int rc = put(kBfToclim, toclim.data())) return rc; }
  if (over->mldclim) { if (int rc = put(kBfZocean, z_ocean.data())) return rc; }
  if (over->z_topo) {
    if (int rc = put(kBfWzAir, wz_air.data())) return rc;
    if (int rc = put(kBfWzVapor, wz_vapor.data())) return rc;
  }
  const size_t last = (size_t)(kNT - 1) * np;
  if (over->tclim) { b.t_last.assign(over->tclim + last, over->tclim + last + np); b.toclim = toclim; }
  if (over->qclim) b.q_last.assign(over->qclim + last, over->qclim + last + np);
  if (over->z_topo) b.z_topo.assign(over->z_topo, over->z_topo + np);
  if (over->mldclim) b.mld0.assign(over->mldclim, over->mldclim + np);
  auto entry = [](const greb_engine::BoundSet& x) {
    return BoundarySet{x.dev[0], x.dev[1], x.dev[2], x.dev[3], x.dev[4], x.dev[5], x.dev[6], x.dev[7], x.dev[8], x.dev[9], x.dev[10],
                       x.dev[11], x.dev[12]};
  };
  BoundarySet* table = e->bsets_dev;
  if (!table) {
    if (int rc = step(dev_alloc(&table, (size_t)1 + GREB_MAX_BOUNDARY_SETS), "hipMalloc")) return rc;
    const BoundarySet own = entry(e->bound[0]);
    if (int rc = step(hipMemcpy(table, &own, sizeof(own), hipMemcpyHostToDevice), "hipMemcpy")) { (void)hipFree(table); return rc; }
  }
  const BoundarySet mine = entry(b);
  if (int rc = step(hipMemcpy(table + e->bound.size(), &mine, sizeof(mine), hipMemcpyHostToDevice), "hipMemcpy")) {
    if (!e->bsets_dev) (void)hipFree(table);
    return rc;
  }
  e->bsets_dev = table;
  e->bound.push_back(std::move(b));
  *set_id = (int)e->bound.size() - 1;
  return 0;
}

int greb_engine_set_member_boundary(greb_engine* e, const int32_t* set, unsigned flags) {
  const char* who = "set_member_boundary: ";
  if (!e) return fail(nullptr, GREB_E_INVALID, std::string(who) + "no engine (greb_engine is NULL)");
  if (flags & ~GREB_BS_REINIT) return fail(e, GREB_E_INVALID, who + ("unknown flag bits in " + std::to_string(flags)));
  const size_t nm = (size_t)e->nm, np = (size_t)e->np;
  const int made = (int)e->bound.size() - 1;
  std::vector<int> bs(nm, 0);
  int on_sets = 0;
  bool uniform = true;
  for (size_t m = 0; set && m < nm; ++m) {
    if (set[m] < 0 || set[m] > made)
      return fail(e, GREB_E_INVALID, who + ("member " + std::to_string(m)) + ": set " + std::to_string(set[m]) + " is outside 0 ... " +
                                         std::to_string(made) + " (add_boundary_set made " + std::to_string(made) + ")");
    bs[m] = set[m];
    on_sets += bs[m] > 0;
    uniform = uniform && bs[m] == bs[0];
  }
  for (size_t m = 0; !e->fused && m < nm; ++m) {
    const unsigned t = e->bound[(size_t)bs[m]].over & ((1u << kBfZtopo) | (1u << kBfUclim) | (1u << kBfVclim));
    if (t)
      return fail(e, GREB_E_UNSUPPORTED,
                  who + ("member " + std::to_string(m)) + ": set " + std::to_string(bs[m]) + " overrides " +
                      kBoundaryNames[(t & (1u << kBfZtopo)) ? kBfZtopo : ((t & (1u << kBfUclim)) ? kBfUclim : kBfVclim)] +
                      ", which the any-grid engine (latitude bands, row strips) transports all members of a launch with -- create an "
                      "engine with those fields or run the groups beside each other (ensemble.run_beside)");
  }
  HIP_TRY(e, hipSetDevice(e->device));
  int* bset_dev = nullptr;
  MemberForcing* neutral = nullptr;
  float *corr = nullptr, *state = nullptr;
  auto step = [&](hipError_t err, const char* what) -> int {
    if (err == hipSuccess) return 0;
    if (bset_dev) (void)hipFree(bset_dev);
    if (neutral) (void)hipFree(neutral);
    if (corr) (void)hipFree(corr);
    if (state) (void)hipFree(state);
    return fail(e, (int)err, std::string(who) + what + ": " + hipGetErrorString(err));
  };
  if (on_sets > 0) {
    if (int rc = step(dev_alloc(&bset_dev, nm), "hipMalloc")) return rc;
    if (int rc = step(hipMemcpy(bset_dev, bs.data(), nm * sizeof(int), hipMemcpyHostToDevice), "hipMemcpy")) return rc;
    if (!e->neutral_force_dev) {
      const std::vector<MemberForcing> w(nm, MemberForcing{-1, 1.f, -1, 1.f});
      if (int rc = step(dev_alloc(&neutral, nm), "hipMalloc")) return rc;
      if (int rc = step(hipMemcpy(neutral, w.data(), nm * sizeof(MemberForcing), hipMemcpyHostToDevice), "hipMemcpy")) return rc;
    }
  }
  if (flags & GREB_BS_REINIT) {
    std::vector<float> st(5 * np);
    if (int rc = step(dev_alloc(&state, nm * 5 * np), "hipMalloc of the members' states")) return rc;
    for (size_t m = 0; m < nm; ++m) {
      initial_state(e->bound[(size_t)bs[m]], e->h_phys[m], np, st.data());
      if (int rc = step(hipMemcpy(state + m * 5 * np, st.data(), 5 * np * sizeof(float), hipMemcpyHostToDevice), "hipMemcpy")) return rc;
    }
  }
  if (int rc = step(hipStreamSynchronize(e->stream), "hipStreamSynchronize")) return rc;
  if (!uniform && e->shared_corr && nm > 1) {
    const char* what = "";
    const hipError_t err = copy_shared_corrections(e, &corr, &what);
    if (int rc = step(err, what)) return rc;
    if (int rc = step(adopt_member_corrections(e, corr), "hipMemcpy")) return rc;
  }
  if (state) { (void)hipFree(e->state); e->state = state; }
  if (neutral) e->neutral_force_dev = neutral;
  if (bset_dev) {
    if (e->bset_dev) (void)hipFree(e->bset_dev);
    e->bset_dev = bset_dev;
  }
  if (set) e->h_bset = bs; else e->h_bset.clear();
  e->members_on_sets = on_sets;
  return 0;
}

int greb_engine_set_corrections(greb_engine* e, int member, const float* corr, const float* state5) {
  if (!e || member < -1 || member >= e->nm) return fail(e, GREB_E_INVALID, "set_corrections: bad argument");
  HIP_TRY(e, hipSetDevice(e->device));
  const size_t n = (size_t)3 * kNT * e->np, s5 = (size_t)5 * e->np;
  const int m0 = member < 0 ? 0 : member, m1 = member < 0 ? e->nm : member + 1;
  for (int m = m0; m < m1; ++m) {
    const size_t ci = e->shared_corr ? 0 : (size_t)m;
    if (corr && (ci == (size_t)m || m == m0)) HIP_TRY(e, hipMemcpy(e->corr + ci * n, corr, n * sizeof(float), hipMemcpyHostToDevice));
    if (state5) HIP_TRY(e, hipMemcpy(e->state + (size_t)m * s5, state5, s5 * sizeof(float), hipMemcpyHostToDevice));
  }
  return 0;
}

int greb_engine_set_state(greb_engine* e, int member, const float* state5) {
  if (!state5) return fail(e, GREB_E_INVALID, "set_state: bad argument");
  return greb_engine_set_corrections(e, member, nullptr, state5);
}

namespace {
struct DevBuf {
  float* p = nullptr;
  ~DevBuf() { if (p) (void)hipFree(p); }
};
int batched_common(const greb_params* p, int nx, int ny, int batch, int device) {
  if (!p || nx < 12 || (nx & 3) || ny < 5 || ny > kMaxNy || batch < 1) return fail(nullptr, GREB_E_INVALID, "batched: bad argument");
  int ndev = 0;
  if (hipGetDeviceCount(&ndev) != hipSuccess || ndev < 1 || device < 0 || device >= ndev)
    return fail(nullptr, GREB_E_NOGPU, "batched: no HIP device (no CPU path)");
  hipError_t err = hipSetDevice(device);
  if (err != hipSuccess) return fail(nullptr, (int)err, "hipSetDevice");
  return 0;
}
}

#define HIP_TRY0(expr) HIP_TRY(nullptr, expr)

namespace {
struct TabCache {
  struct Entry { int device; RowTables* dev; RowTables host; unsigned long long used; };
  std::mutex mu;
  std::vector<Entry> entries;
  unsigned long long clock = 0;
  static constexpr size_t kMax = 32;
} g_tab_cache;
}

#ifdef GREB_TUNING
int greb_tuning_set_stamps(greb_engine* e, unsigned long long* stamps_dev) {
  if (!e) return GREB_E_INVALID;
  e->stamps = stamps_dev;
  return 0;
}
#endif

int greb_release_caches(void) {
  rows_release_cache();
  std::lock_guard<std::mutex> lock(g_tab_cache.mu);
  int prev = 0;
  const bool have_prev = hipGetDevice(&prev) == hipSuccess;
  for (auto& e : g_tab_cache.entries)
    if (e.dev && hipSetDevice(e.device) == hipSuccess) { (void)hipDeviceSynchronize(); (void)hipFree(e.dev); }
  g_tab_cache.entries.clear();
  if (have_prev) (void)hipSetDevice(prev);
  return 0;
}

int greb_diffusion_batched_dev(const greb_params* p, int nx, int ny, int batch, const float* T1_dev,
                               const float* wz_dev, float* dX_dev, int strict, int sweeps, void* stream) {
  if (!p || nx < 12 || (nx & 3) || ny < 5 || ny > kMaxNy || batch < 1 || sweeps < 1)
    return fail(nullptr, GREB_E_INVALID, "diffusion_batched_dev: bad argument");
  int dev = 0;
  HIP_TRY0(hipGetDevice(&dev));
  hipPointerAttribute_t attr;
  if (hipPointerGetAttributes(&attr, T1_dev) != hipSuccess || attr.device != dev) {
    (void)hipGetLastError();
    return fail(nullptr, GREB_E_INVALID, "diffusion_batched_dev: T1_dev is not a device pointer of the current device");
  }
  RowTables t; compute_row_tables(*p, p->kappa, nx, ny, t);
  RowTables* tab_dev = nullptr;
  {
    std::lock_guard<std::mutex> lock(g_tab_cache.mu);
    for (TabCache::Entry& ce : g_tab_cache.entries)
      if (ce.device == dev && std::memcmp(&t, &ce.host, sizeof(t)) == 0) { tab_dev = ce.dev; ce.used = ++g_tab_cache.clock; break; }
    if (!tab_dev && g_tab_cache.entries.size() >= TabCache::kMax) {
      size_t lru = g_tab_cache.entries.size();
      for (size_t i = 0; i < g_tab_cache.entries.size(); ++i)
        if (g_tab_cache.entries[i].device == dev && (lru == g_tab_cache.entries.size() || g_tab_cache.entries[i].used < g_tab_cache.entries[lru].used)) lru = i;
      if (lru < g_tab_cache.entries.size()) {
        HIP_TRY0(hipDeviceSynchronize());
        (void)hipFree(g_tab_cache.entries[lru].dev);
        g_tab_cache.entries.erase(g_tab_cache.entries.begin() + (long)lru);
      }
    }
    if (!tab_dev) {
      TabCache::Entry ce{dev, nullptr, t, ++g_tab_cache.clock};
      HIP_TRY0(dev_alloc(&ce.dev, 1));
      hipError_t he = hipMemcpy(ce.dev, &t, sizeof(t), hipMemcpyHostToDevice);
      if (he != hipSuccess) { (void)hipFree(ce.dev); HIP_TRY0(he); }
      g_tab_cache.entries.push_back(ce);
      tab_dev = ce.dev;
    }
  }
  for (int i = 0; i < sweeps; ++i)
    HIP_TRY0(launch_diffusion(T1_dev, wz_dev, dX_dev, tab_dev, t, nx, ny, batch, strict != 0, (hipStream_t)stream));
  return 0;
}

int greb_diffusion_launch_order(const greb_params* p, int nx, int ny, int batch, int* field, int* k0, int* k1, int* up,
                                int capacity) {
  if (!p || nx < 12 || (nx & 3) || ny < 5 || ny > kMaxNy || batch < 1 || capacity < 0 ||
      (capacity > 0 && (!field || !k0 || !k1 || !up)))
    return fail(nullptr, GREB_E_INVALID, "diffusion_launch_order: bad argument");
  RowTables t; compute_row_tables(*p, p->kappa, nx, ny, t);
  if (!rows_supported(t, nx, ny)) return 0;
  std::vector<RowsTask> tasks;
  rows_tasks(t, ny, batch, rows_default_tuning(), tasks);
  for (size_t i = 0; i < tasks.size() && (int)i < capacity; ++i) {
    field[i] = tasks[i].field; k0[i] = tasks[i].rows & 0xff; k1[i] = (tasks[i].rows >> 8) & 0x1ff;
    up[i] = (tasks[i].rows & kRowsUp) != 0;
  }
  return (int)tasks.size();
}

int greb_step_variant(int flux_phase, int switches, int budget, int forced, int on_sets, unsigned* variant) {
  if (!variant) return fail(nullptr, GREB_E_INVALID, "step_variant: bad argument");
  static float budget_words[1];
  static const MemberForcing force_words[1] = {};
  static const BoundarySet sets[1] = {};
  static const int set_of_member[1] = {};
  MemberArgs a{};
  a.flux_phase = flux_phase != 0;
  a.xsw = switches ? 1u : 0u;
  if (budget) a.bsum = a.brec = budget_words;
  if (on_sets) { a.bsets = sets; a.bset_m = set_of_member; }
  if (forced || (on_sets && !flux_phase)) a.force_m = force_words;
  if (select_variant(a, variant) != hipSuccess) return fail(nullptr, GREB_E_INVALID, "step_variant: no launch carries this combination");
  return 0;
}

int greb_step_variants(unsigned* out, int capacity) {
  if (capacity < 0 || (capacity > 0 && !out)) return fail(nullptr, GREB_E_INVALID, "step_variants: bad argument");
  for (int i = 0; i < kNVariants && i < capacity; ++i) out[i] = kVariants[i];
  return kNVariants;
}

int greb_member_deal_cover(int strict, int* counts) {
  if (!counts) return fail(nullptr, GREB_E_INVALID, "member_deal_cover: bad argument");
  member_deal_cover(strict != 0, counts);
  return 0;
}

int greb_substep_launch_order(const greb_params* p, int nx, int ny, int n_members, const float* kappa, int* field, int* k0,
                              int* k1, int capacity) {
  if (!p || nx < 12 || (nx & 3) || ny < 5 || ny > kMaxNy || n_members < 1 || capacity < 0 || (capacity > 0 && (!field || !k0 || !k1)))
    return fail(nullptr, GREB_E_INVALID, "substep_launch_order: bad argument");
  std::vector<RowTables> tabs((size_t)n_members);
  std::vector<int> idx((size_t)n_members);
  for (int m = 0; m < n_members; ++m) { compute_row_tables(*p, kappa ? kappa[m] : p->kappa, nx, ny, tabs[m]); idx[m] = m; }
  if (n_members >= (1 << (kStepFieldBits - 1)) || !step_rows_supported(tabs.data(), n_members, nx, ny)) return 0;
  std::vector<RowsTask> tasks;
  step_rows_tasks(tabs.data(), idx.data(), n_members, ny, 256 * kStepRowsSlotsPerCu, tasks);
  for (size_t i = 0; i < tasks.size() && (int)i < capacity; ++i) {
    field[i] = tasks[i].field & ((1 << kStepFieldBits) - 1); k0[i] = tasks[i].rows & 0xff; k1[i] = (tasks[i].rows >> 8) & 0x1ff;
  }
  return (int)tasks.size();
}

int greb_circulation_launch_plan(const greb_params* p, int nx, int ny, int n_members, const float* kappa, int slots,
                                 int* field, int* k0, int* k1, int* chain, int* dep4, int capacity) {
  if (!p || nx < 12 || (nx & 3) || ny < 5 || ny > kMaxNy || n_members < 1 || slots < 1 || capacity < 0 ||
      (capacity > 0 && (!field || !k0 || !k1 || !chain || !dep4)))
    return fail(nullptr, GREB_E_INVALID, "circulation_launch_plan: bad argument");
  std::vector<RowTables> tabs((size_t)n_members);
  std::vector<int> idx((size_t)n_members);
  for (int m = 0; m < n_members; ++m) { compute_row_tables(*p, kappa ? kappa[m] : p->kappa, nx, ny, tabs[m]); idx[m] = m; }
  if (n_members >= (1 << (kStepFieldBits - 1)) || !step_rows_supported(tabs.data(), n_members, nx, ny)) return 0;
  std::vector<CircTask> tasks;
  circ_rows_tasks(tabs.data(), idx.data(), n_members, ny, slots, tasks);
  if ((int)tasks.size() > slots) return 0;
  for (size_t i = 0; i < tasks.size() && (int)i < capacity; ++i) {
    field[i] = tasks[i].field & ((1 << kStepFieldBits) - 1); k0[i] = tasks[i].rows & 0xff; k1[i] = (tasks[i].rows >> 8) & 0x1ff;
    chain[i] = (tasks[i].rows & kCircChain) != 0;
    for (int j = 0; j < 4; ++j) dep4[4 * i + j] = tasks[i].dep[j];
  }
  return (int)tasks.size();
}

int greb_diffusion_batched(const greb_params* p, int nx, int ny, int batch, const float* T1, const float* wz,
                           float* dX, int strict, int device) {
  if (int rc = batched_common(p, nx, ny, batch, device)) return rc;
  const size_t n = (size_t)batch * nx * ny;
  DevBuf a, b, c;
  HIP_TRY0(dev_alloc(&a.p, n)); HIP_TRY0(dev_alloc(&b.p, n)); HIP_TRY0(dev_alloc(&c.p, n));
  HIP_TRY0(hipMemcpy(a.p, T1, n * 4, hipMemcpyHostToDevice));
  HIP_TRY0(hipMemcpy(b.p, wz, n * 4, hipMemcpyHostToDevice));
  if (int rc = greb_diffusion_batched_dev(p, nx, ny, batch, a.p, b.p, c.p, strict, 1, nullptr)) return rc;
  HIP_TRY0(hipDeviceSynchronize());
  HIP_TRY0(hipMemcpy(dX, c.p, n * 4, hipMemcpyDeviceToHost));
  return 0;
}

static int adv_or_circ(bool circ, const greb_params* p, int nx, int ny, int batch, const float* X, const float* wz,
                       const float* u, const float* v, float* dX, int strict, int device) {
  if (int rc = batched_common(p, nx, ny, batch, device)) return rc;
  const size_t n = (size_t)batch * nx * ny;
  DevBuf a, b, c, d, o, scr;
  RowTables t; compute_row_tables(*p, p->kappa, nx, ny, t);
  RowTables* tab_dev = nullptr;
  HIP_TRY0(dev_alloc(&tab_dev, 1));
  DevBuf tabhold; tabhold.p = reinterpret_cast<float*>(tab_dev);
  HIP_TRY0(hipMemcpy(tab_dev, &t, sizeof(t), hipMemcpyHostToDevice));
  HIP_TRY0(dev_alloc(&a.p, n)); HIP_TRY0(dev_alloc(&b.p, n)); HIP_TRY0(dev_alloc(&c.p, n));
  HIP_TRY0(dev_alloc(&d.p, n)); HIP_TRY0(dev_alloc(&o.p, n));
  HIP_TRY0(hipMemcpy(a.p, X, n * 4, hipMemcpyHostToDevice));
  HIP_TRY0(hipMemcpy(b.p, wz, n * 4, hipMemcpyHostToDevice));
  HIP_TRY0(hipMemcpy(c.p, u, n * 4, hipMemcpyHostToDevice));
  HIP_TRY0(hipMemcpy(d.p, v, n * 4, hipMemcpyHostToDevice));
  if (circ) {
    HIP_TRY0(dev_alloc(&scr.p, 3 * n));
    HIP_TRY0(launch_circulation(a.p, b.p, c.p, d.p, o.p, scr.p, tab_dev, t, nx, ny, batch, nsub_of(*p), strict != 0, nullptr));
  } else {
    HIP_TRY0(launch_advection(a.p, b.p, c.p, d.p, o.p, tab_dev, nx, ny, batch, strict != 0, nullptr));
  }
  HIP_TRY0(hipDeviceSynchronize());
  HIP_TRY0(hipMemcpy(dX, o.p, n * 4, hipMemcpyDeviceToHost));
  return 0;
}

int greb_advection_batched(const greb_params* p, int nx, int ny, int batch, const float* T1, const float* wz,
                           const float* u, const float* v, float* dX, int strict, int device) {
  return adv_or_circ(false, p, nx, ny, batch, T1, wz, u, v, dX, strict, device);
}

int greb_circulation_batched(const greb_params* p, int nx, int ny, int batch, const float* X, const float* wz,
                             const float* u, const float* v, float* dX, int strict, int device) {
  return adv_or_circ(true, p, nx, ny, batch, X, wz, u, v, dX, strict, device);
}

int greb_engine_point_physics(greb_engine* e, int ityr, float co2, const float* in5, float* out15) {
  if (!e || ityr < 1 || ityr > kNT || !in5 || !out15) return fail(e, GREB_E_INVALID, "point_physics: bad argument");
  HIP_TRY(e, hipSetDevice(e->device));
  const size_t np = (size_t)e->np;
  DevBuf in, out;
  HIP_TRY(e, dev_alloc(&in.p, 5 * np)); HIP_TRY(e, dev_alloc(&out.p, 15 * np));
  HIP_TRY(e, hipMemcpy(in.p, in5, 5 * np * 4, hipMemcpyHostToDevice));
  PointArgs a{};
  a.nx = e->nx; a.ny = e->ny; a.np = e->np; a.ityr = ityr; a.co2 = co2;
  a.z_topo = e->z_topo; a.glacier = e->glacier; a.sw_solar = e->sw_solar; a.tclim = e->tclim;
  a.uclim = e->uclim; a.vclim = e->vclim; a.mldclim = e->mldclim; a.cldclim = e->cldclim; a.swetclim = e->swetclim;
  a.z_ocean = e->z_ocean; a.wz_air = e->wz_air; a.phys = e->h_phys[0]; a.in5 = in.p; a.out15 = out.p;
  a.xsw = e->h_xsw[0]; a.qclim = e->qclim;
  HIP_TRY(e, launch_point_physics(a, e->stream));
  HIP_TRY(e, hipStreamSynchronize(e->stream));
  HIP_TRY(e, hipMemcpy(out15, out.p, 15 * np * 4, hipMemcpyDeviceToHost));
  return 0;
}

}
```

greb_climate_model_amd/csrc/greb_kernels.h:

```cpp
#pragma once
#include <hip/hip_runtime.h>

#include <cstdlib>
#include <utility>
#include <vector>

#include "greb_device.h"

namespace greb {

constexpr int kNT = 730;

#ifdef GREB_TUNING
inline int tuning_int(const char* name, int dflt) {
  const char* e = getenv(name);
  return e ? atoi(e) : dflt;
}
#else
constexpr int tuning_int(const char*, int dflt) { return dflt; }
#endif

constexpr int kMaxDynamicLds = 160 * 1024;

struct MemberForcing {
  int co2_pattern;
  float co2_ref;
  int solar_table;
  float solar_scale;
};

struct BoundarySet {
  const float *z_topo, *glacier;
  const float *tclim, *qclim, *uclim, *vclim, *mldclim, *cldclim, *swetclim;
  const float *toclim, *z_ocean, *wz_air, *wz_vapor;
};
constexpr int kBoundaryFields = 13;
constexpr int kBoundaryInputs = 9;
constexpr int kMaxBoundarySets = 16;

struct MemberArgs {
  int nx, ny, np;
  const float *z_topo, *glacier, *sw_solar;
  const float *tclim, *qclim, *uclim, *vclim, *mldclim, *cldclim, *swetclim;
  const float *toclim, *z_ocean, *wz_air, *wz_vapor;
  float* state;
  float* acc;
  float* corr;
  const int* corr_index;
  const RowTables* tabs;
  const int* tab_index;
  const Phys* phys;
  int flux_phase;
  long long it0;
  int nsteps;
  int nsub;
  const float* co2;
  int co2_stride;
  int co2_year0;
  float co2_flux;
  float* monthly;
  int monthly_years;
  int year_out0;
  float* yearly;
  int yearly_years, yearly_year0;
  int ipx, ipy;
  unsigned xsw;
  unsigned long long* stamps;
  int dbg;
  const unsigned* xsw_m;
  const float* co2_flux_m;
  float* bsum;
  float* brec;
  int brec_years;
  int brec_year0;
  const MemberForcing* force_m;
  const float* f_space;
  const float* f_season;
  const float* f_solar;
  const BoundarySet* bsets;
  const int* bset_m;
};

enum { kBsw, kBLWsurf, kBLWdown, kBLWabs, kBQsens, kBQlat, kBQlatAir, kBdqEva, kBdqRain, kBdTocean, kBdTo, kBdTaCrcl, kBdqCrcl, kNBudget };

enum : unsigned { kVFlux = 1, kVExp = 2, kVBudget = 4, kVForce = 8, kVBound = 16 };
constexpr bool variant_valid(unsigned v) {
  const bool flux = v & kVFlux, exp = v & kVExp, budget = v & kVBudget, force = v & kVForce, bound = v & kVBound;
  return v < 32u && !(budget && flux) && (!force || (exp && !flux)) && (!bound || (exp && (flux || force)));
}
constexpr unsigned kVariants[] = {0u, kVFlux, kVExp, kVFlux | kVExp, kVBudget, kVExp | kVBudget, kVExp | kVForce,
                                  kVExp | kVBudget | kVForce, kVFlux | kVExp | kVBound, kVExp | kVForce | kVBound,
                                  kVExp | kVBudget | kVForce | kVBound};
constexpr int kNVariants = (int)(sizeof(kVariants) / sizeof(kVariants[0]));

inline hipError_t select_variant(const MemberArgs& a, unsigned* v) {
  const bool flux = a.flux_phase != 0, budget = a.bsum != nullptr;
  if (budget && (flux || !a.brec)) return hipErrorInvalidValue;
  unsigned r = (flux ? kVFlux : 0u) | (budget ? kVBudget : 0u);
  if (a.bset_m) {
    if (!a.bsets || (!flux && !a.force_m)) return hipErrorInvalidValue;
    r |= kVExp | kVBound | (flux ? 0u : kVForce);
  } else if (a.force_m) {
    if (flux) return hipErrorInvalidValue;
    r |= kVExp | kVForce;
  } else if (a.xsw || a.xsw_m) r |= kVExp;
  *v = r;
  return hipSuccess;
}
inline const char* variant_family(unsigned v) {
  return (v & kVBound) ? "boundary" : (v & kVForce) ? "forcing" : (v & kVExp) ? "switches" : "default";
}
template <template <bool, unsigned> class Family, size_t... I>
auto pick_variant(bool strict, unsigned v, std::index_sequence<I...>) {
  decltype(Family<false, 0u>::kernel()) k = nullptr;
  ((kVariants[I] == v ? (void)(k = strict ? Family<true, kVariants[I]>::kernel() : Family<false, kVariants[I]>::kernel()) : (void)0), ...);
  return k;
}
template <template <bool, unsigned> class Family>
auto pick_variant(bool strict, unsigned v) { return pick_variant<Family>(strict, v, std::make_index_sequence<kNVariants>{}); }

bool member_layout_supported(const RowTables& tab, int nx, int ny);
void member_deal_cover(bool strict, int* counts);
hipError_t launch_member_kernel(const MemberArgs& a, int n_members, bool strict, hipStream_t s);
hipError_t launch_circulation_g96(const float* X, const float* wz, const float* u, const float* v, float* dX,
                                  const RowTables* tab_dev, int batch, int nsub, bool strict, hipStream_t s);

hipError_t launch_diffusion(const float* T1, const float* wz, float* dX, const RowTables* tab_dev,
                            const RowTables& tab_host, int nx, int ny, int batch, bool strict, hipStream_t s);
bool rows_supported(const RowTables& t, int nx, int ny);
struct RowsTask { int field, rows; };
constexpr int kRowsUp = 1 << 20;
struct RowsTuning {
  int chain_target;
  int chain_span;
  int parts[4];
  int level_tasks[4];
};
inline RowsTuning rows_default_tuning() { return RowsTuning{3000, 70, {8, 8, 16, 39}, {0, 0, 2048, 1024}}; }
void rows_tasks(const RowTables& t, int ny, int batch, const RowsTuning& tu, std::vector<RowsTask>& tasks);
void rows_release_cache();
hipError_t launch_diffusion_rows(const float* T1, const float* wz, float* dX, const RowTables& t, int ny, int batch,
                                 bool strict, hipStream_t s);
bool step_rows_supported(const RowTables* tabs, int n_tabs, int nx, int ny);
constexpr int kStepRowsSlotsPerCu = 8;
void step_rows_tasks(const RowTables* tabs, const int* tab_index, int n_members, int ny, int n_slots,
                     std::vector<RowsTask>& tasks);
constexpr int kStepFieldBits = 16;
constexpr int kStepHeadTasks = 16;
hipError_t step_rows_make_tasks(const RowTables* tabs_host, const int* tab_index_host, int n_members, int ny,
                                int n_slots, RowsTask** dev, int* n, RowsTask* head );
hipError_t launch_substep_rows(const float* X, const float* W2, const float* u, const float* v, float* Xnew,
                               const RowTables* tabs_dev, const int* tab_index_dev, const RowsTask* tasks, const RowsTask* head_host,
                               int n_tasks, int n_simd, int nx, int ny, bool strict, hipStream_t s, bool calm_vapor);
struct CircTask {
  int field;
  int rows;
  int dep[4];
  int issue;
  int pad;
};
constexpr int kCircChain = 1 << 21;
constexpr int kChainTaskMinSweeps = 64;
constexpr unsigned kCircSpinTicks = 100u * 1000u * 1000u;
void circ_rows_tasks(const RowTables* tabs, const int* tab_index, int n_members, int ny, int n_slots,
                     std::vector<CircTask>& tasks);
struct CircOrder {
  CircTask* tasks = nullptr;
  unsigned* flags = nullptr;
  unsigned* ctrl = nullptr;
  int n = 0;
  unsigned epoch = 0;
};
hipError_t circ_rows_make_order(const RowTables* tabs_host, const int* tab_index_host, int n_members, int ny, int n_slots,
                                CircOrder* out);
void circ_rows_free_order(CircOrder* o);
hipError_t launch_circulation_rows(float* X0, float* X1, const float* W2, const float* u, const float* v,
                                   const RowTables* tabs_dev, CircOrder& order, int n_simd, int nx, int ny, int nsub, bool strict,
                                   hipStream_t s, bool calm_vapor);
int circ_rows_status(const CircOrder& o, unsigned* diag5);
hipError_t launch_advection(const float* T1, const float* wz, const float* u, const float* v, float* dX,
                            const RowTables* tab_dev, int nx, int ny, int batch, bool strict, hipStream_t s);
hipError_t launch_circulation(const float* X, const float* wz, const float* u, const float* v, float* dX,
                              float* scratch , const RowTables* tab_dev, const RowTables& tab_host,
                              int nx, int ny, int batch, int nsub, bool strict, hipStream_t s);

hipError_t launch_substep_fused(const float* X, const float* W2, const float* u, const float* v, float* Xnew,
                                const RowTables* tabs, const int* tab_index, int nx, int ny, int n_members,
                                bool strict, hipStream_t s, bool calm_vapor = false);
hipError_t launch_physics_step(const MemberArgs& a, const float* X, float* Xout, float* red, int n_members,
                               bool strict, hipStream_t s);
hipError_t launch_yearly(const float* red, float* yearly, int np, int nx, int ipx, int ipy, int yearly_years,
                         int year_index, int n_members, bool strict, hipStream_t s);
hipError_t launch_pack_tracers(const float* state, float* X, int np, int n_members, hipStream_t s);

struct PointArgs {
  int nx, ny, np, ityr;
  float co2;
  const float *z_topo, *glacier, *sw_solar, *tclim, *uclim, *vclim, *mldclim, *cldclim, *swetclim;
  const float *z_ocean, *wz_air;
  Phys phys;
  unsigned xsw;
  const float* qclim;
  const float* in5;
  float* out15;
};
hipError_t launch_point_physics(const PointArgs& a, hipStream_t s);

}
```

greb_climate_model_amd/csrc/greb_member.hip:

```cpp
#include <cstdlib>

#include "greb_kernels.h"
#include "greb_pair.h"
#include "greb_physics_step.h"
#include "greb_stencil.h"

namespace greb {

constexpr int NX = 96, NY = 48, NQ = 24, NP = 4608;
constexpr int kThreads = 512;
constexpr int RS = 2 * NX + 16;
constexpr int XB = (NY + 2) * RS;
constexpr int kOffX = RS;
constexpr int kOffW = 2 * XB + RS;
constexpr int kOffWX = 3 * XB;
constexpr int kOffWY = kOffWX + NP;
constexpr int kOffRowK = kOffWY + NP;
constexpr int kRowKCsDif = 7;
constexpr int kLdsFloats = kOffRowK + NY * kRowKWords;
constexpr size_t kLdsBytes = (size_t)kLdsFloats * sizeof(float);

bool member_layout_supported(const RowTables& t, int nx, int ny) {
  if (nx != NX || ny != NY) return false;
  for (int k = 0; k < NY; ++k) {
// ... 554 lines not shown
    const bool calm_q = NOT_CALM ? false : calm_runtime;
    constexpr bool kPolar = is_polar_wave<STRICT>(WAVE);
    BulkTasks tasks;
    BulkSigns signs;
    QuadChain quad;
    if constexpr (!kPolar) tasks = make_tasks<STRICT>(WAVE, lane);
    else if constexpr (!STRICT) quad_chain_setup(lds, cur, lane, calm_q, quad);
    if constexpr (!kPolar && !STRICT) make_signs<WAVE>(lds, tasks, signs);
    float ccy_dif = 0.f;
    if constexpr (!kPolar && !STRICT) ccy_dif = __int_as_float(__builtin_amdgcn_readfirstlane(__float_as_int(lds[kOffRowK + 2])));
#pragma unroll 1
    for (int tt = 0; tt < nsub; ++tt) {
#ifdef GREB_TUNING
      const unsigned long long t0 = stamp ? __builtin_amdgcn_s_memtime() : 0;
#endif
      if constexpr (kPolar && STRICT) { if (!(dbg & 4)) chain_substep_strict(lds, cur, WAVE - 2, lane, calm_q); }
      else if constexpr (kPolar) { if (!(dbg & 4)) quad_chain_substep(lds, cur, quad); }
      else bulk_substep<STRICT, WAVE>(lds, cur, tasks, signs, ccy_dif, dbg, calm_q);
#ifdef GREB_TUNING
      if (stamp) busy += __builtin_amdgcn_s_memtime() - t0;
#endif
      __syncthreads();
      cur ^= 1;
    }
  }
  __device__ __forceinline__ void substeps(lfloat* lds, int cur, int nsub, int dbg = 0, bool calm_q = false
#ifdef GREB_TUNING
                                           , bool stamp = false, unsigned long long* busy = nullptr
#endif
  ) {
    int lane = threadIdx.x & 63;
    asm volatile("" : "+v"(lane));
#ifdef GREB_TUNING
    unsigned long long b = 0;
#define GREB_ROLE(W) case W: if (!STRICT && !calm_q) role_loop<W, true>(lds, cur, nsub, lane, dbg, false, stamp, b); \
                             else role_loop<W, false>(lds, cur, nsub, lane, dbg, calm_q, stamp, b); break;
#else
#define GREB_ROLE(W) case W: if (!STRICT && !calm_q) role_loop<W, true>(lds, cur, nsub, lane, dbg, false); \
                             else role_loop<W, false>(lds, cur, nsub, lane, dbg, calm_q); break;
#endif
    switch (__builtin_amdgcn_readfirstlane(threadIdx.x >> 6)) {
      GREB_ROLE(0) GREB_ROLE(1) GREB_ROLE(2) GREB_ROLE(3) GREB_ROLE(4) GREB_ROLE(5) GREB_ROLE(6) GREB_ROLE(7)
    }
#undef GREB_ROLE
#ifdef GREB_TUNING
    if (busy) *busy += b;
#endif
  }
};

template <bool STRICT>
__global__ __launch_bounds__(kThreads) void circulation_g96_kernel(const float* __restrict__ Xin,
                                                                   const float* __restrict__ wz,
                                                                   const float* __restrict__ ug,
                                                                   const float* __restrict__ vg,
                                                                   float* __restrict__ dX,
                                                                   const RowTables* __restrict__ tab, int nsub,
                                                                   int dbg) {
  extern __shared__ __align__(16) float lds_raw[];
  lfloat* lds = (lfloat*)lds_raw;
  const size_t fo = (size_t)blockIdx.x * NP;
  Circ<STRICT> c;
  c.init(lds, wz + fo, wz + fo, tab);
  for (int i = threadIdx.x; i < NP / 4; i += kThreads) {
    const f4 x = ld4(Xin + fo + 4 * i);
    st8(lds + kOffX + (i / NQ) * RS, i % NQ, zip(x, x));
  }
  __syncthreads();
  stage_winds<STRICT>(lds, ug + fo, vg + fo, tab);
  __syncthreads();
  c.substeps(lds, 0, nsub, dbg);
  const int cur = nsub & 1;
  for (int i = threadIdx.x; i < NP / 4; i += kThreads) {
    const f4 a = comp(ld8(lds + kOffX + cur * XB + (i / NQ) * RS, i % NQ), 0), b = ld4(Xin + fo + 4 * i);
    st4(dX + fo + 4 * i, f4{{a.v[0] - b.v[0], a.v[1] - b.v[1], a.v[2] - b.v[2], a.v[3] - b.v[3]}});
  }
}

hipError_t launch_circulation_g96(const float* X, const float* wz, const float* u, const float* v, float* dX,
                                  const RowTables* tab_dev, int batch, int nsub, bool strict, hipStream_t s) {
  auto kern = strict ? circulation_g96_kernel<true> : circulation_g96_kernel<false>;
  hipError_t e = hipFuncSetAttribute(reinterpret_cast<const void*>(kern),
                                     hipFuncAttributeMaxDynamicSharedMemorySize, (int)kLdsBytes);
  if (e != hipSuccess) return e;
  hipLaunchKernelGGL(kern, dim3(batch), dim3(kThreads), kLdsBytes, s, X, wz, u, v, dX, tab_dev, nsub,
                     tuning_int("GREB_DEBUG_SKIP", 0));
  return hipGetLastError();
}

template <bool STRICT, unsigned V>
__global__ __launch_bounds__(kThreads) void member_kernel(MemberArgs a) {
  constexpr bool FLUX = V & kVFlux, EXP = V & kVExp, BUDGET = V & kVBudget, FORCE = V & kVForce, BOUND = V & kVBound;
  extern __shared__ __align__(16) float lds_raw[];
  lfloat* lds = (lfloat*)lds_raw;
  const int m = blockIdx.x, tid = threadIdx.x;
  float* state = a.state + (size_t)m * 5 * NP;
  float* acc = a.acc + (size_t)m * 6 * NP;
  float* corr = a.corr + (size_t)a.corr_index[m] * 3 * kNT * NP;
  const RowTables* tab = a.tabs + a.tab_index[m];

#ifdef GREB_TUNING
  for (int i = 0; i < (a.dbg >> 8) * (m & 7); ++i) __builtin_amdgcn_s_sleep(16);
#endif
  Circ<STRICT> circ;
  const int bset = member_bset<BOUND>(a, m);
  {
    const BoundPtr B = member_boundary<BOUND>(a, bset);
    circ.init(lds, BOUND ? (const float*)B->wz_air : a.wz_air, BOUND ? (const float*)B->wz_vapor : a.wz_vapor, tab);
  }
  for (int i = tid; i < NP / 4; i += kThreads)
    st8(lds + kOffX + (i / NQ) * RS, i % NQ, zip(ld4(state + NP + 4 * i), ld4(state + 3 * NP + 4 * i)));
  int cur = 0;
  const unsigned xsw = EXP ? member_switches(a, m) : 0u;
  const int nsub = (EXP && (xsw & kXNoCirc)) ? 0 : a.nsub;
  const float co2_flux = FLUX ? (a.co2_flux_m ? a.co2_flux_m[m] : a.co2_flux) : 0.f;
  __syncthreads();
#ifdef GREB_TUNING
  const bool stamp = a.stamps != nullptr;
  unsigned long long st_wind = 0, st_circ = 0, st_busy = 0, st_phys = 0;
  const unsigned long long st_c0 = stamp ? __builtin_amdgcn_s_memtime() : 0, st_r0 = stamp ? __builtin_amdgcn_s_memrealtime() : 0;
#define GREB_STAMP(var) const unsigned long long var = stamp ? __builtin_amdgcn_s_memtime() : 0
#else
#define GREB_STAMP(var)
#endif

#pragma unroll 1
  for (int s = 0; s < a.nsteps; ++s) {
    const long long it = a.it0 + s;
    const StepClock ck = step_clock<FLUX>(a, it, NP);
    const int ityr = ck.ityr, yr_rel = ck.yr_rel;
    const size_t off = ck.off;

    GREB_STAMP(t_a);
    {
      const BoundPtr B = member_boundary<BOUND>(a, bset);
      stage_winds<STRICT, EXP && !STRICT>(lds, (BOUND ? (const float*)B->uclim : a.uclim) + off,
                                          (BOUND ? (const float*)B->vclim : a.vclim) + off, tab);
    }
    __syncthreads();
    GREB_STAMP(t_b);

#ifdef GREB_TUNING
    circ.substeps(lds, cur, nsub, 0, EXP && (xsw & kXQDiffOnly), stamp, &st_busy);
#else
    circ.substeps(lds, cur, nsub, 0, EXP && (xsw & kXQDiffOnly));
#endif
    cur ^= nsub & 1;
    GREB_STAMP(t_c);

    const Phys P = a.phys[m];
    const float co2 = FLUX ? co2_flux : a.co2[(size_t)m * a.co2_stride + a.co2_year0 + yr_rel];
    const MemberForce mf = member_force<FORCE>(a, m, ck);
    const BoundPtr B = member_boundary<BOUND>(a, bset);
    lfloat* Xf = lds + kOffX + cur * XB;
    lfloat* red = lds + kOffX + (cur ^ 1) * XB;
    if constexpr (BUDGET) {
      const BudgetSink bs = budget_sink<true>(a, m, ck);
#pragma unroll 1
      for (int qd = tid; qd < NP / 4; qd += kThreads) {
        const q8 xpair = ld8(Xf + (qd / NQ) * RS, qd % NQ);
        const PhysIn in = physics_load<V>(a, qd, ck, state, acc, corr, xsw, mf, B);
        (void)physics_compute<STRICT, V | kVBudget>(a, P, in, co2, comp(xpair, 0), comp(xpair, 1), xsw, bs, 4 * qd, mf);
      }
    }
#pragma unroll 1
    for (int qd = tid; qd < NP / 4; qd += kThreads) {
#ifdef GREB_TUNING
      if ((a.dbg & 4) && qd >= kThreads) break;
#endif
      const q8 xpair = ld8(Xf + (qd / NQ) * RS, qd % NQ);
      f4 oTa, oq, tsm;
      physics_quad<STRICT, V & ~kVBudget>(a, P, m, qd, ck, co2, state, acc, corr, comp(xpair, 0), comp(xpair, 1), oTa, oq, tsm, xsw, mf, B);
      st8(Xf + (qd / NQ) * RS, qd % NQ, zip(oTa, oq));
      if (ityr == kNT) st4(red + 4 * qd, tsm);
    }
    if (ityr == kNT) {
      __syncthreads();
      if (STRICT) {
        if (tid == 0 && a.yearly) {
#pragma clang fp contract(off)
          float sum = 0.f;
          for (int i = 0; i < NP; ++i) sum += red[i];
          float* y = a.yearly + ((size_t)m * a.yearly_years + (a.yearly_year0 + yr_rel)) * 2;
          y[0] = sum / (float)NP - 273.15f;
          y[1] = red[(a.ipy - 1) * NX + (a.ipx - 1)] - 273.15f;
        }
      } else if (a.yearly) {
        int t0 = tid;
        if (EXP) asm volatile("" : "+v"(t0));
        float part = 0.f;
        for (int i = t0; i < NP; i += kThreads) part += red[i];
        part = wave_sum(part);
        const float point = red[(a.ipy - 1) * NX + (a.ipx - 1)];
        __syncthreads();
        if ((tid & 63) == 0) red[tid >> 6] = part;
        __syncthreads();
        if (tid == 0) {
          float sum = 0.f;
          for (int w = 0; w < kThreads / 64; ++w) sum += red[w];
          float* y = a.yearly + ((size_t)m * a.yearly_years + (a.yearly_year0 + yr_rel)) * 2;
          y[0] = sum / (float)NP - 273.15f;
          y[1] = point - 273.15f;
        }
      }
    }
    __syncthreads();
#ifdef GREB_TUNING
    if (stamp) {
      const unsigned long long t_d = __builtin_amdgcn_s_memtime();
      st_wind += t_b - t_a; st_circ += t_c - t_b; st_phys += t_d - t_c;
    }
#endif
  }
#ifdef GREB_TUNING
  if (stamp && (tid & 63) == 0) {
    unsigned long long* o = a.stamps + ((size_t)m * (kThreads / 64) + (tid >> 6)) * 8;
    o[0] = __builtin_amdgcn_s_memtime() - st_c0; o[1] = __builtin_amdgcn_s_memrealtime() - st_r0;
    o[2] = st_wind; o[3] = st_circ; o[4] = st_busy; o[5] = st_phys; o[6] = (unsigned long long)a.nsteps; o[7] = (unsigned long long)nsub;
  }
#endif
}

template <bool STRICT, unsigned V>
struct MemberFamily { static auto kernel() { return &member_kernel<STRICT, V>; } };

hipError_t launch_member_kernel(const MemberArgs& a, int n_members, bool strict, hipStream_t s) {
  if (a.nx != NX || a.ny != NY) return hipErrorInvalidValue;
  unsigned v;
  if (hipError_t e = select_variant(a, &v); e != hipSuccess) return e;
  const auto kern = pick_variant<MemberFamily>(strict, v);
  if (!kern) return hipErrorInvalidValue;
  hipError_t e = hipFuncSetAttribute(reinterpret_cast<const void*>(kern),
                                     hipFuncAttributeMaxDynamicSharedMemorySize, (int)kLdsBytes);
  if (e != hipSuccess) return e;
  hipLaunchKernelGGL(kern, dim3(n_members), dim3(kThreads), kLdsBytes, s, a);
  return hipGetLastError();
}

}
```

greb_climate_model_amd/csrc/greb_physics_step.h:

```cpp
#pragma once
#include "greb_kernels.h"

namespace greb {

__device__ __constant__ int kMonthEnd[12] = {31, 59, 90, 120, 151, 181, 212, 243, 273, 304, 334, 365};
__device__ __constant__ int kMonthDays[12] = {31, 28, 31, 30, 31, 30, 31, 31, 30, 31, 30, 31};

struct StepClock {
  int ityr, mon, yr_rel;
  size_t off, offm;
};
template <bool FLUX>
__device__ __forceinline__ StepClock step_clock(const MemberArgs& a, long long it, int np) {
  StepClock c;
  c.ityr = (int)((it - 1) % kNT) + 1;
  const int jday = (int)(((it - 1) / 2) % 365) + 1;
  c.off = (size_t)(c.ityr - 1) * np;
  c.offm = (size_t)(c.ityr > 1 ? c.ityr - 2 : kNT - 1) * np;
  c.yr_rel = (int)((it - 1) / kNT - (a.it0 - 1) / kNT);
  c.mon = -1;
  if (!FLUX && (it % 2 == 0))
    for (int mm = 0; mm < 12; ++mm) if (jday == kMonthEnd[mm]) c.mon = mm;
  return c;
}

__device__ __forceinline__ unsigned member_switches(const MemberArgs& a, int m) {
  return (unsigned)__builtin_amdgcn_readfirstlane((int)(a.xsw_m ? a.xsw_m[m] : a.xsw));
}

struct MemberForce {
  const float* space;
  const float* solar;
  float season;
  float ref, scale;
};
__device__ __forceinline__ float uniform_f(float x) { return __int_as_float(__builtin_amdgcn_readfirstlane(__float_as_int(x))); }
template <bool FORCE>
__device__ __forceinline__ MemberForce member_force(const MemberArgs& a, int m, const StepClock& ck) {
  MemberForce f{nullptr, a.sw_solar, 1.f, 0.f, 1.f};
  if (FORCE) {
    const MemberForcing w = a.force_m[m];
    const int k = __builtin_amdgcn_readfirstlane(w.co2_pattern), t = __builtin_amdgcn_readfirstlane(w.solar_table);
    f.ref = uniform_f(w.co2_ref); f.scale = uniform_f(w.solar_scale);
    if (k >= 0) {
      f.space = a.f_space + (size_t)k * a.np;
      f.season = uniform_f(a.f_season[(size_t)k * kNT + (ck.ityr - 1)]);
    }
    if (t >= 0) f.solar = a.f_solar + (size_t)t * kNT * a.ny;
  }
  return f;
}
__device__ __forceinline__ float forced_co2(const MemberForce& f, float w_space, float co2) {
#pragma clang fp contract(off)
  const float w = w_space * f.season;
  const float part = w * co2;
  const float rest = (1.f - w) * f.ref;
  return part + rest;
}

typedef const BoundarySet __attribute__((address_space(4)))* BoundPtr;
template <bool BOUND>
__device__ __forceinline__ int member_bset(const MemberArgs& a, int m) {
  return BOUND ? __builtin_amdgcn_readfirstlane(a.bset_m[m]) : 0;
}
template <bool BOUND>
__device__ __forceinline__ BoundPtr member_boundary(const MemberArgs& a, int bset) {
  unsigned long long p = 0;
  if (BOUND) {
    p = (unsigned long long)(a.bsets + bset);
    asm volatile("" : "+s"(p));
  }
  return (BoundPtr)p;
}
#define GREB_BF(f) (BOUND ? (const float*)B->f : a.f)

struct PhysIn {
  f4 Ts, Ta, To, q, cap;
  f4 zt, gl, zo, ez;
  f4 tcl, cld, mld, mldm, swet, u, v;
  f4 c0, c1, c2;
  f4 acc0, acc1, acc2, acc3, acc4, acc5;
  f4 qcl, tclp;
  f4 fw;
  float solar;
};
struct PhysOut {
  f4 Ts, Ta, To, q, cap, TF, qF, ToF, tsmn;
  f4 s0, s1, s2, s3, s4;
};

template <unsigned V>
__device__ __forceinline__ PhysIn physics_load(const MemberArgs& a, int qd, const StepClock& ck, const float* __restrict__ state,
                                               const float* __restrict__ acc, const float* __restrict__ corr, unsigned xsw_member,
                                               const MemberForce& F, BoundPtr B) {
  constexpr bool FLUX = V & kVFlux, EXP = V & kVExp, FORCE = V & kVForce, BOUND = V & kVBound;
  static_assert(variant_valid(V), "no such variant of the step kernels");
  const int nx = a.nx, ny = a.ny, np = a.np, p0 = 4 * qd;
  const size_t off = ck.off, offm = ck.offm;
  const unsigned xsw = EXP ? xsw_member : 0u;
  PhysIn i;
  i.Ts = ld4(state + p0); i.Ta = ld4(state + np + p0); i.To = ld4(state + 2 * np + p0); i.q = ld4(state + 3 * np + p0);
  i.cap = ld4(state + 4 * np + p0);
  i.zt = ld4(GREB_BF(z_topo) + p0); i.gl = ld4(GREB_BF(glacier) + p0); i.zo = ld4(GREB_BF(z_ocean) + p0); i.ez = ld4(GREB_BF(wz_air) + p0);
  i.tcl = ld4(GREB_BF(tclim) + off + p0); i.cld = ld4(GREB_BF(cldclim) + off + p0); i.mld = ld4(GREB_BF(mldclim) + off + p0);
  i.mldm = ld4(GREB_BF(mldclim) + offm + p0); i.swet = ld4(GREB_BF(swetclim) + off + p0); i.u = ld4(GREB_BF(uclim) + off + p0);
  i.v = ld4(GREB_BF(vclim) + off + p0);
  if (FORCE) {
#pragma clang fp contract(off)
    i.solar = F.solar[(size_t)(ck.ityr - 1) * ny + p0 / nx] * F.scale;
  } else i.solar = a.sw_solar[(size_t)(ck.ityr - 1) * ny + p0 / nx];
  if (FLUX) { i.c0 = ld4(GREB_BF(toclim) + p0); i.c1 = ld4(GREB_BF(qclim) + off + p0); i.c2 = zero4(); }
  else { i.c0 = ld4(corr + off + p0); i.c1 = ld4(corr + (size_t)kNT * np + off + p0); i.c2 = ld4(corr + (size_t)2 * kNT * np + off + p0); }
  i.acc0 = i.acc1 = i.acc2 = i.acc3 = i.acc4 = zero4();
#ifdef GREB_TUNING
  const bool no_acc = a.dbg & 1;
#else
  constexpr bool no_acc = false;
#endif
  i.acc5 = no_acc ? zero4() : ld4(acc + 5 * np + p0);
  if (!FLUX && !no_acc) {
    i.acc0 = ld4(acc + p0); i.acc1 = ld4(acc + np + p0); i.acc2 = ld4(acc + 2 * np + p0); i.acc3 = ld4(acc + 3 * np + p0);
    i.acc4 = ld4(acc + 4 * np + p0);
  }
  i.qcl = zero4(); i.tclp = zero4();
  if (EXP && (xsw & kXLwLinear)) i.qcl = FLUX ? i.c1 : ld4(GREB_BF(qclim) + off + p0);
  if (EXP && !FLUX && (xsw & kXSstPlus1)) i.tclp = ld4(GREB_BF(tclim) + offm + p0);
  i.fw = zero4();
  if (FORCE && F.space) i.fw = ld4(F.space + p0);
  return i;
}

struct BudgetSink {
  float* sum;
  float* rec;
  float ndm;
};
template <bool BUDGET>
__device__ __forceinline__ BudgetSink budget_sink(const MemberArgs& a, int m, const StepClock& ck) {
  BudgetSink b{nullptr, nullptr, 1.f};
  if (BUDGET) {
    b.sum = a.bsum + (size_t)m * kNBudget * a.np;
    if (ck.mon >= 0) {
      b.ndm = (float)(kMonthDays[ck.mon] * 2);
      b.rec = a.brec + (((size_t)m * a.brec_years + (a.brec_year0 + ck.yr_rel)) * 12 + ck.mon) * kNBudget * a.np;
    }
  }
  return b;
}
template <bool BUDGET>
__device__ __forceinline__ void budget_add(const BudgetSink& b, int np, int term, int p, float x) {
  if (BUDGET) {
#pragma clang fp contract(off)
    float* s = b.sum + (size_t)term * np + p;
    float v = *s + x;
    if (b.rec) {
      __builtin_nontemporal_store(v / b.ndm, b.rec + (size_t)term * np + p);
      v = 0.f;
    }
    *s = v;
  }
}

template <bool STRICT, unsigned V>
__device__ __forceinline__ PhysOut physics_compute(const MemberArgs& a, const Phys& P, const PhysIn& in, float co2, const f4& xTa,
                                                   const f4& xq, unsigned xsw_member, const BudgetSink& bs, int p0,
                                                   const MemberForce& F) {
  constexpr bool FLUX = V & kVFlux, EXP = V & kVExp, BUDGET = V & kVBudget, FORCE = V & kVForce;
  static_assert(variant_valid(V), "no such variant of the step kernels");
  const unsigned xsw = EXP ? xsw_member : 0u;
  const int np = a.np;
  PhysOut o;
  o.TF = o.qF = o.ToF = zero4();
#pragma unroll
  for (int e = 0; e < 4; ++e) {
#pragma clang fp contract(off)
    float Ts1 = in.Ts.v[e];
    const float Ta1 = in.Ta.v[e], To1 = in.To.v[e], q1 = in.q.v[e], cap = in.cap.v[e];
    const float zt = in.zt.v[e], gl = in.gl.v[e], ez = in.ez.v[e], tcl = in.tcl.v[e], cld = in.cld.v[e], mld = in.mld.v[e];
    if (EXP && !FLUX && (xsw & kXSstPlus1) && zt < 0.0f) Ts1 = in.tclp.v[e] + 1.0f;
    const bool calm = EXP && (xsw & kXNoCirc);
    const float dTa_crcl = calm ? 0.f : xTa.v[e] - Ta1;
    const float dq_crcl = (calm || (EXP && (xsw & kXNoQTransport))) ? 0.f : xq.v[e] - q1;
    budget_add<BUDGET>(bs, np, kBdTaCrcl, p0 + e, dTa_crcl); budget_add<BUDGET>(bs, np, kBdqCrcl, p0 + e, dq_crcl);
    float albedo, sw, LWsurf, LWdown, em, Qlat, Qlat_air, dq_eva, dq_rain, dT_ocean, dTo;
    sw_radiation<STRICT>(P, Ts1, zt, gl, cld, in.solar, albedo, sw, xsw);
    budget_add<BUDGET>(bs, np, kBsw, p0 + e, sw);
    const float co2_e = (FORCE && F.space) ? forced_co2(F, in.fw.v[e], co2) : co2;
    lw_radiation<STRICT>(P, Ts1, Ta1, q1, co2_e, ez, cld, tcl, LWsurf, LWdown, em, xsw, in.qcl.v[e]);
    budget_add<BUDGET>(bs, np, kBLWsurf, p0 + e, LWsurf); budget_add<BUDGET>(bs, np, kBLWdown, p0 + e, LWdown);
    const float LWabs = em * LWsurf;
    budget_add<BUDGET>(bs, np, kBLWabs, p0 + e, LWabs);
    const float Qsens = P.ct_sens * (Ta1 - Ts1);
    budget_add<BUDGET>(bs, np, kBQsens, p0 + e, Qsens);
    hydro<STRICT>(P, Ts1, q1, in.u.v[e], in.v.v[e], zt, ez, in.swet.v[e], Qlat, Qlat_air, dq_eva, dq_rain, xsw);
    budget_add<BUDGET>(bs, np, kBQlat, p0 + e, Qlat); budget_add<BUDGET>(bs, np, kBQlatAir, p0 + e, Qlat_air);
    budget_add<BUDGET>(bs, np, kBdqEva, p0 + e, dq_eva); budget_add<BUDGET>(bs, np, kBdqRain, p0 + e, dq_rain);
    deep_ocean<STRICT>(P, Ts1, To1, zt, mld, in.mldm.v[e], in.zo.v[e], dT_ocean, dTo, xsw);
    budget_add<BUDGET>(bs, np, kBdTocean, p0 + e, dT_ocean); budget_add<BUDGET>(bs, np, kBdTo, p0 + e, dTo);
    const float LWup = LWdown;
    float Ts0, Ta0, To0, q0;
    if (FLUX) {
      const float dTs = fdiv<STRICT>(P.dt * (sw + LWsurf - LWdown + Qlat + Qsens), cap);
      Ts0 = Ts1 + dTs + dT_ocean;
      const float dTa = fdiv<STRICT>(P.dt * (LWup + LWdown - em * LWsurf + Qlat_air - Qsens), P.cap_air);
      Ta0 = Ta1 + dTa + dTa_crcl;
      To0 = To1 + dTo;
      const float dq = P.dt * (dq_eva + dq_rain);
      q0 = q1 + dq + dq_crcl;
      const float TF = fdiv<STRICT>((tcl - Ts0) * cap, P.dt);
      Ts0 = Ts1 + dTs + dT_ocean + fdiv<STRICT>(TF * P.dt, cap);
      const float ToF = in.c0.v[e] - To0;
      To0 = To1 + dTo + ToF;
      const float qF = in.c1.v[e] - q0;
      q0 = q1 + dq + dq_crcl + qF;
      o.TF.v[e] = TF; o.qF.v[e] = qF; o.ToF.v[e] = ToF;
    } else {
      const float TF = in.c0.v[e], qF = in.c1.v[e], ToF = in.c2.v[e];
      Ts0 = Ts1 + dT_ocean + fdiv<STRICT>(P.dt * (sw + LWsurf - LWdown + Qlat + Qsens + TF), cap);
      Ta0 = Ta1 + dTa_crcl + fdiv<STRICT>(P.dt * (LWup + LWdown - em * LWsurf + Qlat_air - Qsens), P.cap_air);
      To0 = To1 + dTo + ToF;
      float dq = P.dt * (dq_eva + dq_rain) + dq_crcl + qF;
      if (dq <= -q1) dq = -0.9f * q1;
      q0 = q1 + dq;
    }
    o.Ts.v[e] = Ts0; o.Ta.v[e] = Ta0; o.To.v[e] = To0; o.q.v[e] = q0;
    o.cap.v[e] = seaice<STRICT>(P, Ts0, zt, gl, mld, cap, xsw);
    o.tsmn.v[e] = in.acc5.v[e] + Ts0;
    o.s0.v[e] = in.acc0.v[e] + Ts0; o.s1.v[e] = in.acc1.v[e] + Ta0; o.s2.v[e] = in.acc2.v[e] + To0;
    o.s3.v[e] = in.acc3.v[e] + q0; o.s4.v[e] = in.acc4.v[e] + albedo;
  }
  return o;
}

template <bool FLUX>
__device__ __forceinline__ void physics_store(const MemberArgs& a, int m, int qd, const StepClock& ck,
                                              const PhysOut& o, float* __restrict__ state, float* __restrict__ acc,
                                              float* __restrict__ corr, f4& tsmn_mean) {
  const int np = a.np, p0 = 4 * qd, mon = ck.mon;
  const size_t off = ck.off;
#ifdef GREB_TUNING
  const bool no_acc = a.dbg & 1, no_wb = a.dbg & 2;
#else
  constexpr bool no_acc = false, no_wb = false;
#endif
  if (!no_wb) {
    st4(state + p0, o.Ts); st4(state + np + p0, o.Ta); st4(state + 2 * np + p0, o.To); st4(state + 3 * np + p0, o.q);
    st4(state + 4 * np + p0, o.cap);
  }
  if (FLUX) {
    st4(corr + off + p0, o.TF); st4(corr + (size_t)kNT * np + off + p0, o.qF); st4(corr + (size_t)2 * kNT * np + off + p0, o.ToF);
  } else {
#pragma clang fp contract(off)
    f4 s0 = o.s0, s1 = o.s1, s2 = o.s2, s3 = o.s3, s4 = o.s4;
    if (mon >= 0) {
      const float ndm = (float)(kMonthDays[mon] * 2);
      float* rec = a.monthly + (((size_t)m * a.monthly_years + (a.year_out0 + ck.yr_rel)) * 12 + mon) * 5 * np;
      f4 r0, r1, r2, r3, r4;
#pragma unroll
      for (int e = 0; e < 4; ++e) {
        r0.v[e] = s0.v[e] / ndm; r1.v[e] = s1.v[e] / ndm; r2.v[e] = s2.v[e] / ndm; r3.v[e] = s3.v[e] / ndm; r4.v[e] = s4.v[e] / ndm;
      }
      st4_nt(rec + p0, r0); st4_nt(rec + np + p0, r1); st4_nt(rec + 2 * np + p0, r2); st4_nt(rec + 3 * np + p0, r3); st4_nt(rec + 4 * np + p0, r4);
      s0 = s1 = s2 = s3 = s4 = zero4();
    }
    if (!no_acc) { st4(acc + p0, s0); st4(acc + np + p0, s1); st4(acc + 2 * np + p0, s2); st4(acc + 3 * np + p0, s3); st4(acc + 4 * np + p0, s4); }
  }
  if (ck.ityr == kNT) {
#pragma clang fp contract(off)
    f4 t;
#pragma unroll
    for (int e = 0; e < 4; ++e) t.v[e] = o.tsmn.v[e] / (float)kNT;
    tsmn_mean = t;
    if (!no_acc) st4(acc + 5 * np + p0, zero4());
  } else {
    if (!no_acc) st4(acc + 5 * np + p0, o.tsmn);
  }
}

template <bool STRICT, unsigned V>
__device__ __forceinline__ void physics_quad(const MemberArgs& a, const Phys& P, int m, int qd, const StepClock& ck,
                                             float co2, float* __restrict__ state, float* __restrict__ acc,
                                             float* __restrict__ corr, const f4& xTa, const f4& xq, f4& oTa_out,
                                             f4& oq_out, f4& tsmn_mean, unsigned xsw, const MemberForce& F, BoundPtr B) {
  constexpr bool FLUX = V & kVFlux, BUDGET = V & kVBudget;
  const PhysIn in = physics_load<V>(a, qd, ck, state, acc, corr, xsw, F, B);
  const PhysOut o = physics_compute<STRICT, V>(a, P, in, co2, xTa, xq, xsw, budget_sink<BUDGET>(a, m, ck), 4 * qd, F);
  physics_store<FLUX>(a, m, qd, ck, o, state, acc, corr, tsmn_mean);
  oTa_out = o.Ta; oq_out = o.q;
}
#undef GREB_BF

}
```

greb_climate_model_amd/engine.py:

```python
from __future__ import annotations

import ctypes as C
import json
import os

import numpy as np

from . import abi, build, workload

_lib = None


class GrebError(RuntimeError):
    def __init__(self, code: int, msg: str):
        super().__init__(f"greb engine error {code}: {msg}")
        self.code = code


_lib_path = build.LIB


def use_tuning_build() -> None:
    global _lib_path
    if _lib is not None:
        raise GrebError(-100, "use_tuning_build() after the library was loaded")
    _lib_path = build.LIB_TUNING


def lib() -> C.CDLL:
    global _lib
    if _lib is None:
        if not os.path.exists(_lib_path):
            raise GrebError(-100, f"{_lib_path} not built; run `python -c 'import __graft_entry__ as g; g.build()'`")
        L = C.CDLL(_lib_path)
        L.greb_engine_last_error.restype = C.c_char_p
        L.greb_engine_last_error.argtypes = [C.c_void_p]
        L.greb_device_info.restype = C.c_char_p
        L.greb_params_default.restype = None
        abi.ens_prototypes(L)
        _lib = L
    return _lib


EXPORTS = ["greb_params_default", "greb_engine_create", "greb_engine_flux_correction", "greb_engine_run",
           "greb_engine_get_corrections", "greb_engine_set_corrections", "greb_engine_get_state",
           "greb_engine_last_error", "greb_engine_destroy", "greb_device_info", "greb_diffusion_batched",
           "greb_advection_batched", "greb_circulation_batched", "greb_diffusion_batched_dev",
           "greb_engine_point_physics", "greb_log_exp_switches", "greb_engine_set_experiment",
           "greb_ensemble_moments_dev", "greb_ensemble_quantiles_dev", "greb_engine_set_state", "greb_release_caches", "greb_diffusion_launch_order",
           "greb_substep_launch_order", "greb_circulation_launch_plan", "greb_engine_describe",
           "greb_engine_create_members", "greb_engine_set_member_experiments", "greb_diag_create", "greb_diag_destroy",
           "greb_diag_reduce_dev", "greb_engine_run_diag", "greb_engine_run_budget", "greb_budget_name",
           "greb_member_deal_cover", "greb_engine_set_forcing_tables", "greb_engine_set_member_forcing",
           "greb_engine_add_boundary_set", "greb_engine_set_member_boundary", "greb_step_variant", "greb_step_variants",
           "greb_clim_create", "greb_clim_destroy", "greb_clim_add_year_dev", "greb_clim_finish_dev", "greb_engine_run_clim",
           "greb_ens_create", "greb_ens_destroy", "greb_ens_reduce_dev", "greb_engine_run_ens"]


def _check(rc: int, h=None):
    if rc != 0:
        msg = lib().greb_engine_last_error(h)
        raise GrebError(rc, msg.decode() if msg else "")


def device_info(device: int = 0) -> dict:
    return json.loads(lib().greb_device_info(device).decode())


def budget_name(i: int) -> str | None:
    f = lib().greb_budget_name
    f.restype = C.c_char_p
    s = f(int(i))
    return None if s is None else s.decode()


def log_exp_switches(log_exp: int) -> int:
    f = lib().greb_log_exp_switches
    f.restype = C.c_uint
    return int(f(int(log_exp)))


def member_configs(params: abi.GrebParams, members):
    floats = set(abi.GrebParams.PHYSICS_NAMES) | {"co2_flux"}
    arr = (abi.GrebMemberConfig * len(members))()
    for c, d in zip(arr, members):
        C.memmove(C.byref(c.p), C.byref(params), C.sizeof(abi.GrebParams))
        c.switches = 0
        if "switches" in d and "log_exp" in d:
            raise GrebError(-1, "members: give `switches` or `log_exp`, not both")
        for k, v in d.items():
            if k == "switches":
                c.switches = int(v)
            elif k == "log_exp":
                c.switches = log_exp_switches(int(v))
            elif k == "p_emi":
                if len(v) != 10:
                    raise GrebError(-1, "members: p_emi takes ten values")
                for i, x in enumerate(v):
                    c.p.p_emi[i] = float(x)
            elif k in floats:
                setattr(c.p, k, float(v))
            else:
                raise GrebError(-1, f"members: unknown key {k!r}")
    return arr


def boundary_fields(nx: int, ny: int, fields: dict) -> dict:
    out = {}
    for name, x in fields.items():
        if name == "sw_solar":
            raise GrebError(-1, "add_boundary_set: sw_solar is not part of a boundary set: insolation tables are per-member "
                                "forcing (set_forcing_tables, set_member_forcing)")
        if name not in abi.BOUNDARY_FIELDS:
            raise GrebError(-1, f"add_boundary_set: unknown field {name!r} (one of {', '.join(abi.BOUNDARY_FIELDS)})")
        if x is None:
            continue
        x = np.asarray(x)
        if x.dtype.kind not in "fiu":
            raise GrebError(-1, f"add_boundary_set: {name} has dtype {x.dtype}, expected real numbers (float32)")
        want = (ny, nx) if abi.BOUNDARY_FIELDS[name] == 2 else (abi.NSTEP_YR, ny, nx)
        if x.shape != want:
            raise GrebError(-1, f"add_boundary_set: {name} has shape {x.shape}, expected {list(want)}")
        out[name] = np.ascontiguousarray(x, np.float32)
    if not out:
        raise GrebError(-1, "add_boundary_set: no field given: the set would be the engine's own data (set 0)")
    return out


def params_default() -> abi.GrebParams:
    p = abi.GrebParams()
    lib().greb_params_default(C.byref(p))
    return p


class Engine:

    def __init__(self, inp: workload.Inputs, params: abi.GrebParams | None = None, n_members: int = 1,
                 overrides=None, device: int = 0, strict: bool = False, multilaunch: bool = False,
                 row_strips: bool = False, persistent: bool | None = None, members=None):
        L = lib()
        self.params = params or params_default()
        if members is not None:
            if overrides is not None:
                raise GrebError(-1, "Engine: give `members` or `overrides`, not both")
            members = list(members)
            n_members = len(members)
        self.nx, self.ny, self.np, self.nm = inp.nx, inp.ny, inp.nx * inp.ny, n_members
        fields, self._keep = abi.make_fields(inp)
        ov = None
        if overrides is not None:
            ov = (abi.GrebMemberOverrides * n_members)()
            for i, o in enumerate(overrides):
                for k in ("da_ice", "a_no_ice", "a_cloud", "kappa"):
                    setattr(ov[i], k, float(o.get(k, float("nan"))))
        self.h = C.c_void_p()
        flags = ((abi.F_STRICT if strict else 0) | (abi.F_MULTILAUNCH if multilaunch else 0) |
                 (abi.F_ROW_STRIPS if row_strips else 0) |
                 (0 if persistent is None else (abi.F_PERSISTENT if persistent else abi.F_NO_PERSISTENT)))
        if members is not None:
            rc = L.greb_engine_create_members(C.byref(self.params), inp.nx, inp.ny, C.byref(fields), n_members,
                                              member_configs(self.params, members), device, flags, C.byref(self.h))
        else:
            rc = L.greb_engine_create(C.byref(self.params), inp.nx, inp.ny, C.byref(fields), n_members, ov, device, flags,
                                      C.byref(self.h))
        if rc != 0:
            msg = L.greb_engine_last_error(self.h).decode()
            if self.h:
                L.greb_engine_destroy(self.h)
                self.h = None
            raise GrebError(rc, msg)

    def describe(self) -> dict:
        f = lib().greb_engine_describe
        f.restype = C.c_char_p
        return json.loads(f(self.h).decode())

    def close(self):
        if getattr(self, "h", None):
            lib().greb_engine_destroy(self.h)
            self.h = None

    def __del__(self):
        try:
            self.close()
        except Exception:
            pass

    def flux_correction(self, years: int) -> np.ndarray:
        yearly = np.zeros((self.nm, max(years, 1), 2), np.float32)
        _check(lib().greb_engine_flux_correction(self.h, int(years), abi.fptr(yearly)), self.h)
        return yearly[:, :years]

    def _run_arrays(self, years: int, co2_ppm):
        co2 = np.ascontiguousarray(np.broadcast_to(np.asarray(co2_ppm, np.float32), (self.nm, years)))
        return co2, np.zeros((self.nm, years, 2), np.float32)

    def run(self, years: int, co2_ppm, monthly_dev_ptr: int | None = None, out: np.ndarray | None = None):
        co2, yearly = self._run_arrays(years, co2_ppm)
        if monthly_dev_ptr is None:
            shape = (self.nm, years, 12, 5, self.ny, self.nx)
            if out is None:
                monthly = np.empty(shape, np.float32)
            else:
                if out.dtype != np.float32 or not out.flags.c_contiguous or out.size != int(np.prod(shape)):
                    raise GrebError(-1, "run: `out` must be C-contiguous float32 with n_members*years*12*5*ny*nx elements")
                monthly = out.reshape(shape)
            _check(lib().greb_engine_run(self.h, int(years), abi.fptr(co2), abi.fptr(monthly), abi.fptr(yearly), 0), self.h)
            return monthly, yearly
        _check(lib().greb_engine_run(self.h, int(years), abi.fptr(co2), C.c_void_p(monthly_dev_ptr), abi.fptr(yearly),
                                     abi.RUN_DEVICE_OUT), self.h)
        return None, yearly

    def run_budget(self, years: int, co2_ppm, want_monthly: bool = True, monthly_dev_ptr: int | None = None,
                   budget_dev_ptr: int | None = None):
        co2, yearly = self._run_arrays(years, co2_ppm)
        f = lib().greb_engine_run_budget
        if budget_dev_ptr is not None:
            _check(f(self.h, int(years), abi.fptr(co2), None if monthly_dev_ptr is None else C.c_void_p(monthly_dev_ptr),
                     C.c_void_p(budget_dev_ptr), abi.fptr(yearly), abi.RUN_DEVICE_OUT), self.h)
            return None, None, yearly
        if monthly_dev_ptr is not None:
            raise GrebError(-1, "run_budget: monthly_dev_ptr needs budget_dev_ptr (one run delivers to one side)")
        monthly = np.empty((self.nm, years, 12, 5, self.ny, self.nx), np.float32) if want_monthly else None
        budget = np.empty((self.nm, years, 12, abi.NBUDGET, self.ny, self.nx), np.float32)
        _check(f(self.h, int(years), abi.fptr(co2), None if monthly is None else abi.fptr(monthly), abi.fptr(budget),
                 abi.fptr(yearly), 0), self.h)
        return monthly, budget, yearly

    def run_diag(self, years: int, co2_ppm, plan, what: int | None = None):
        from . import diag
        what = diag.ALL if what is None else int(what)
        co2, yearly = self._run_arrays(years, co2_ppm)
        regions = np.empty((self.nm, years, 12, 5, plan.nr), np.float32) if what & abi.D_REGIONS else None
        zonal = np.empty((self.nm, years, 12, 5, self.ny), np.float32) if what & abi.D_ZONAL else None
        annual = np.empty((self.nm, years, 5, self.ny, self.nx), np.float32) if what & abi.D_ANNUAL else None
        ptr = [None if a is None else abi.fptr(a) for a in (regions, zonal, annual)]
        _check(lib().greb_engine_run_diag(self.h, int(years), abi.fptr(co2), plan.h, C.c_uint(what), *ptr, abi.fptr(yearly)),
               self.h)
        return diag.Result(regions, zonal, annual, yearly, plan.names)

    def run_clim(self, years: int, co2_ppm, plan, periods):
        from . import clim
        co2, yearly = self._run_arrays(years, co2_ppm)
        per = np.ascontiguousarray(periods, np.int32).reshape(-1, 2)
        first, count = np.ascontiguousarray(per[:, 0]), np.ascontiguousarray(per[:, 1])
        out = clim.empty_products(plan.what, (self.nm, len(per)), self.ny, self.nx)
        ip = lambda a: a.ctypes.data_as(C.POINTER(C.c_int32))
        _check(lib().greb_engine_run_clim(self.h, int(years), abi.fptr(co2), plan.h, len(per), ip(first), ip(count),
                                          *[None if a is None else abi.fptr(a) for a in out], abi.fptr(yearly)), self.h)
        return clim.Result(*out, yearly)

    def run_ens(self, years: int, co2_ppm, plan):
        from . import ens
        co2, yearly = self._run_arrays(years, co2_ppm)
        out = ens.empty_products(plan, (years,), (12, 5, self.ny, self.nx))
        _check(lib().greb_engine_run_ens(self.h, int(years), abi.fptr(co2), plan.h,
                                         *[None if a is None else abi.fptr(a) for a in out], abi.fptr(yearly)), self.h)
        return ens.Result(*out, yearly)

    def state(self, member: int = 0) -> np.ndarray:
        s = np.empty((5, self.ny, self.nx), np.float32)
        _check(lib().greb_engine_get_state(self.h, member, abi.fptr(s)), self.h)
        return s

    def get_corrections(self, member: int = 0):
        corr = np.empty((3, abi.NSTEP_YR, self.ny, self.nx), np.float32)
        st = np.empty((5, self.ny, self.nx), np.float32)
        _check(lib().greb_engine_get_corrections(self.h, member, abi.fptr(corr), abi.fptr(st)), self.h)
        return corr, st

    def set_corrections(self, corr, state5, member: int = -1):
        corr = None if corr is None else np.ascontiguousarray(corr, np.float32)
        state5 = None if state5 is None else np.ascontiguousarray(state5, np.float32)
        _check(lib().greb_engine_set_corrections(self.h, member, None if corr is None else abi.fptr(corr),
                                                 None if state5 is None else abi.fptr(state5)), self.h)

    def set_experiment(self, switches: int):
        _check(lib().greb_engine_set_experiment(self.h, C.c_uint(int(switches))), self.h)

    def set_member_experiments(self, switches):
        sw = np.ascontiguousarray(switches, np.uint32)
        if sw.shape != (self.nm,):
            raise GrebError(-1, f"set_member_experiments: {self.nm} switch words expected")
        _check(lib().greb_engine_set_member_experiments(self.h, sw.ctypes.data_as(C.POINTER(C.c_uint32))), self.h)

    def set_forcing_tables(self, space, season=None, solar=None):
        def arr(x, tail, what):
            if x is None:
                return None
            x = np.ascontiguousarray(x, np.float32)
            if x.ndim == len(tail):
                x = x[None]
            if x.shape[1:] != tail:
                raise GrebError(-1, f"set_forcing_tables: {what} has shape {x.shape}, expected [n]{list(tail)}")
            return x
        space = arr(space, (self.ny, self.nx), "space")
        season = arr(season, (abi.NSTEP_YR,), "season")
        solar = arr(solar, (abi.NSTEP_YR, self.ny), "solar")
        if season is not None and (space is None or len(season) != len(space)):
            raise GrebError(-1, "set_forcing_tables: season needs one row of 730 per pattern of space")
        ptr = lambda x: None if x is None else abi.fptr(x)
        _check(lib().greb_engine_set_forcing_tables(self.h, 0 if space is None else len(space), ptr(space), ptr(season),
                                                    0 if solar is None else len(solar), ptr(solar)), self.h)

    def set_member_forcing(self, forcing):
        if forcing is None:
            _check(lib().greb_engine_set_member_forcing(self.h, None), self.h)
            return
        forcing = list(forcing)
        if len(forcing) != self.nm:
            raise GrebError(-1, f"set_member_forcing: {self.nm} entries expected")
        arr = (abi.GrebMemberForcing * self.nm)()
        for f, d in zip(arr, forcing):
            d = dict(d or {})
            f.co2_pattern = int(d.pop("co2_pattern", -1)); f.co2_ref = float(d.pop("co2_ref", 340.0))
            f.solar_table = int(d.pop("solar_table", -1)); f.solar_scale = float(d.pop("solar_scale", 1.0))
            if d:
                raise GrebError(-1, f"set_member_forcing: unknown key {sorted(d)[0]!r}")
        _check(lib().greb_engine_set_member_forcing(self.h, arr), self.h)

    def add_boundary_set(self, **fields) -> int:
        arrs = boundary_fields(self.nx, self.ny, fields)
        f = abi.GrebFields()
        for name, x in arrs.items():
            setattr(f, name, abi.fptr(x))
        sid = C.c_int(0)
        _check(lib().greb_engine_add_boundary_set(self.h, C.byref(f), C.byref(sid)), self.h)
        return int(sid.value)

    def set_member_boundary(self, sets, reinit: bool = False):
        flags = abi.BS_REINIT if reinit else 0
        if sets is None:
            _check(lib().greb_engine_set_member_boundary(self.h, None, C.c_uint(flags)), self.h)
            return
        ids = np.ascontiguousarray(sets, np.int32)
        if ids.shape != (self.nm,):
            raise GrebError(-1, f"set_member_boundary: {self.nm} set ids expected")
        _check(lib().greb_engine_set_member_boundary(self.h, ids.ctypes.data_as(C.POINTER(C.c_int32)), C.c_uint(flags)), self.h)

    def point_physics(self, ityr: int, co2: float, in5) -> np.ndarray:
        in5 = np.ascontiguousarray(in5, np.float32)
        out = np.empty((15, self.ny, self.nx), np.float32)
        _check(lib().greb_engine_point_physics(self.h, int(ityr), C.c_float(co2), abi.fptr(in5), abi.fptr(out)), self.h)
        return out


POINT_FIELDS = ("albedo", "sw", "LWsurf", "LWair_down", "em", "Q_sens", "Qlat", "Qlat_air", "dq_eva", "dq_rain",
                "dT_ocean", "dTo", "cap_surf_new")


def _batched(fn_name, params, arrays, strict, device):
    arrs = [np.ascontiguousarray(a, np.float32) for a in arrays]
    shape = arrs[0].shape
    if arrs[0].ndim == 2:
        arrs = [a[None] for a in arrs]
    b, ny, nx = arrs[0].shape
    out = np.empty((b, ny, nx), np.float32)
    p = params or params_default()
    fn = getattr(lib(), fn_name)
    _check(fn(C.byref(p), nx, ny, b, *[abi.fptr(a) for a in arrs], abi.fptr(out), int(bool(strict)), device))
    return out.reshape(shape)


def diffusion(T1, wz, params=None, strict=False, device=0):
    return _batched("greb_diffusion_batched", params, (T1, wz), strict, device)


def advection(T1, wz, u, v, params=None, strict=False, device=0):
    return _batched("greb_advection_batched", params, (T1, wz, u, v), strict, device)


def circulation(X, wz, u, v, params=None, strict=False, device=0):
    return _batched("greb_circulation_batched", params, (X, wz, u, v), strict, device)


def diffusion_launch_order(params, nx, ny, batch):
    params = params if params is not None else params_default()
    f = lib().greb_diffusion_launch_order
    n = f(C.byref(params), nx, ny, batch, None, None, None, None, 0)
    if n < 0:
        _check(n)
    out = [np.zeros(n, np.int32) for _ in range(4)]
    if n:
        ptr = [a.ctypes.data_as(C.POINTER(C.c_int)) for a in out]
        assert f(C.byref(params), nx, ny, batch, *ptr, n) == n
    return out


def substep_launch_order(params, nx, ny, n_members, kappa=None):
    params = params if params is not None else params_default()
    kap = None if kappa is None else np.ascontiguousarray(kappa, np.float32)
    kp = None if kap is None else kap.ctypes.data_as(C.POINTER(C.c_float))
    f = lib().greb_substep_launch_order
    n = f(C.byref(params), nx, ny, n_members, kp, None, None, None, 0)
    if n < 0:
        _check(n)
    out = [np.zeros(n, np.int32) for _ in range(3)]
    if n:
        ptr = [a.ctypes.data_as(C.POINTER(C.c_int)) for a in out]
        assert f(C.byref(params), nx, ny, n_members, kp, *ptr, n) == n
    return out


def member_deal_cover(strict=False):
    out = np.zeros((48, 24), np.int32)
    _check(lib().greb_member_deal_cover(int(bool(strict)), out.ctypes.data_as(C.POINTER(C.c_int))))
    return out


def step_variant(flux_phase=False, switches=False, budget=False, forced=False, on_sets=False):
    v = C.c_uint(0xFFFFFFFF)
    rc = lib().greb_step_variant(int(bool(flux_phase)), int(bool(switches)), int(bool(budget)), int(bool(forced)),
                                 int(bool(on_sets)), C.byref(v))
    return v.value if rc == 0 else None


def step_variants():
    n = lib().greb_step_variants(None, 0)
    out = (C.c_uint * n)()
    assert lib().greb_step_variants(out, n) == n
    return list(out)


def circulation_launch_plan(params, nx, ny, n_members, kappa=None, slots=2048):
    params = params if params is not None else params_default()
    kap = None if kappa is None else np.ascontiguousarray(kappa, np.float32)
    kp = None if kap is None else kap.ctypes.data_as(C.POINTER(C.c_float))
    f = lib().greb_circulation_launch_plan
    n = f(C.byref(params), nx, ny, n_members, kp, slots, None, None, None, None, None, 0)
    if n < 0:
        _check(n)
    out = [np.zeros(n, np.int32) for _ in range(4)] + [np.zeros((n, 4), np.int32)]
    if n:
        ptr = [a.ctypes.data_as(C.POINTER(C.c_int)) for a in out]
        assert f(C.byref(params), nx, ny, n_members, kp, slots, *ptr, n) == n
    return out


def diffusion_dev(params, nx, ny, batch, T1_ptr, wz_ptr, dX_ptr, strict=False, sweeps=1, stream=0):
    _check(lib().greb_diffusion_batched_dev(C.byref(params), nx, ny, batch, C.c_void_p(T1_ptr), C.c_void_p(wz_ptr),
                                            C.c_void_p(dX_ptr), int(bool(strict)), int(sweeps), C.c_void_p(stream)))
```

include/greb_engine.h:

```cpp
#ifndef GREB_ENGINE_H
#define GREB_ENGINE_H

#include <stddef.h>
#include <stdint.h>

#ifdef __cplusplus
extern "C" {
#endif

#define GREB_NSTEP_YR 730
#define GREB_NVAR_OUT 5

#define GREB_E_INVALID   (-1)
#define GREB_E_NOGPU     (-2)
#define GREB_E_STATE     (-3)
#define GREB_E_UNSUPPORTED (-4)

typedef struct greb_params {
  float pi, sig, rho_ocean, rho_land, rho_air, cp_ocean, cp_land, cp_air, eps;
  float d_ocean, d_land, d_air, ct_sens, da_ice, a_no_ice, a_cloud;
  float Tl_ice1, Tl_ice2, To_ice1, To_ice2;
  float co_turb, kappa, ce, cq_latent, cq_rain, z_air, z_vapor, r_qviwv;
  float p_emi[10];
  float co2_flux;
// ... 23 lines not shown
} greb_member_overrides;

typedef struct greb_member_config {
  greb_params p;
  uint32_t switches;
} greb_member_config;

#define GREB_F_STRICT 1u
#define GREB_F_MULTILAUNCH 2u

#define GREB_F_ROW_STRIPS 4u
#define GREB_F_NO_PERSISTENT 8u
#define GREB_F_PERSISTENT 16u

typedef struct greb_engine greb_engine;

int greb_engine_create(const greb_params* p, int nx, int ny, const greb_fields* f, int n_members,
                       const greb_member_overrides* overrides, int device, unsigned flags,
                       greb_engine** out);

int greb_engine_create_members(const greb_params* p, int nx, int ny, const greb_fields* f, int n_members,
                               const greb_member_config* members, int device, unsigned flags, greb_engine** out);

int greb_engine_flux_correction(greb_engine* e, int years, float* yearly);

const char* greb_engine_describe(greb_engine* e);

#define GREB_RUN_DEVICE_OUT 1u
int greb_engine_run(greb_engine* e, int years, const float* co2_ppm, float* monthly, float* yearly,
                    unsigned run_flags);

#define GREB_NBUDGET 13
#define GREB_B_SW          0
#define GREB_B_LW_SURF     1
#define GREB_B_LWAIR_DOWN  2
#define GREB_B_LW_ABS      3
#define GREB_B_Q_SENS      4
#define GREB_B_Q_LAT       5
#define GREB_B_Q_LAT_AIR   6
#define GREB_B_DQ_EVA      7
#define GREB_B_DQ_RAIN     8
#define GREB_B_DT_OCEAN    9
#define GREB_B_DTO         10
#define GREB_B_DTA_CRCL    11
#define GREB_B_DQ_CRCL     12
const char* greb_budget_name(int i);
int greb_engine_run_budget(greb_engine* e, int years, const float* co2_ppm, float* monthly, float* budget, float* yearly,
                           unsigned run_flags);

#define GREB_D_REGIONS 1u
#define GREB_D_ZONAL   2u
#define GREB_D_ANNUAL  4u
typedef struct greb_diag greb_diag;
int greb_diag_create(int nx, int ny, const float* region_w, int n_regions, greb_diag** out);
int greb_diag_destroy(greb_diag* d);
int greb_diag_reduce_dev(greb_diag* d, int device, const float* monthly_year_dev, int n_members, float* regions_dev,
                         float* zonal_dev, float* annual_dev, void* stream);
int greb_engine_run_diag(greb_engine* e, int years, const float* co2_ppm, greb_diag* d, unsigned what, float* regions,
                         float* zonal, float* annual, float* yearly);

#define GREB_C_MEAN     1u
#define GREB_C_SEASONS  2u
#define GREB_C_TREND    4u
#define GREB_C_RESPONSE 8u
typedef struct greb_clim greb_clim;
int greb_clim_create(int nx, int ny, int n_members, const int32_t* control, unsigned what, greb_clim** out);
int greb_clim_destroy(greb_clim* c);
int greb_clim_add_year_dev(greb_clim* c, int device, const float* monthly_year_dev, int k, void* stream);
int greb_clim_finish_dev(greb_clim* c, int device, int n_years, float* mean_dev, float* seasons_dev, float* trend_dev,
                         float* mean_resp_dev, float* seasons_resp_dev, void* stream);
int greb_engine_run_clim(greb_engine* e, int years, const float* co2_ppm, greb_clim* c, int n_periods, const int32_t* first_year,
                         const int32_t* n_years, float* mean, float* seasons, float* trend, float* mean_resp, float* seasons_resp,
                         float* yearly);

#define GREB_S_MEAN      1u
#define GREB_S_VAR       2u
#define GREB_S_RANGE     4u
#define GREB_S_QUANTILES 8u
#define GREB_ENS_MAX_GROUPS 64
#define GREB_ENS_MAX_PROBS  16
#define GREB_ENS_MAX_SORTED 4096
typedef struct greb_ens greb_ens;
int greb_ens_create(int nx, int ny, int n_members, const int32_t* group, int n_groups, const int32_t* control,
                    const float* probs, int n_probs, unsigned what, greb_ens** out);
int greb_ens_destroy(greb_ens* s);
int greb_ens_reduce_dev(greb_ens* s, int device, const float* x_dev, size_t n, float* mean_dev, float* var_dev, float* min_dev,
                        float* max_dev, float* quant_dev, void* stream);
int greb_engine_run_ens(greb_engine* e, int years, const float* co2_ppm, greb_ens* s, float* mean, float* var, float* min,
                        float* max, float* quant, float* yearly);

#define GREB_MAX_FORCING_TABLES 16
int greb_engine_set_forcing_tables(greb_engine* e,
      int n_patterns, const float* co2_space  ,
                      const float* co2_season ,
      int n_solar,    const float* sw_solar   );
typedef struct greb_member_forcing {
  int32_t co2_pattern;
  float   co2_ref;
  int32_t solar_table;
  float   solar_scale;
} greb_member_forcing;
int greb_engine_set_member_forcing(greb_engine* e, const greb_member_forcing* f);

#define GREB_MAX_BOUNDARY_SETS 16
int greb_engine_add_boundary_set(greb_engine* e, const greb_fields* over, int* set_id);
#define GREB_BS_REINIT 1u
int greb_engine_set_member_boundary(greb_engine* e, const int32_t* set, unsigned flags);

#define GREB_X_NO_ICE            (1u << 0)
#define GREB_X_NO_HYDRO          (1u << 1)
#define GREB_X_NO_DEEP_OCEAN     (1u << 2)
#define GREB_X_LW_LINEAR_VAPOR   (1u << 3)
#define GREB_X_NO_CIRCULATION    (1u << 4)
#define GREB_X_NO_VAPOR_TRANSPORT (1u << 5)
#define GREB_X_VAPOR_DIFFUSION_ONLY (1u << 6)
#define GREB_X_SST_PLUS1         (1u << 7)
unsigned greb_log_exp_switches(int log_exp);
int greb_engine_set_experiment(greb_engine* e, unsigned switches);
int greb_engine_set_member_experiments(greb_engine* e, const uint32_t* switches);

int greb_engine_get_corrections(greb_engine* e, int member, float* corr, float* state5);
int greb_engine_set_corrections(greb_engine* e, int member, const float* corr, const float* state5);

int greb_engine_get_state(greb_engine* e, int member, float* state5);
int greb_engine_set_state(greb_engine* e, int member, const float* state5);

const char* greb_engine_last_error(const greb_engine* e);
int greb_engine_destroy(greb_engine* e);

const char* greb_device_info(int device);

int greb_diffusion_batched(const greb_params* p, int nx, int ny, int batch, const float* T1,
                           const float* wz, float* dX, int strict, int device);
int greb_advection_batched(const greb_params* p, int nx, int ny, int batch, const float* T1,
                           const float* wz, const float* u, const float* v, float* dX, int strict,
                           int device);
int greb_circulation_batched(const greb_params* p, int nx, int ny, int batch, const float* X,
                             const float* wz, const float* u, const float* v, float* dX, int strict,
                             int device);
int greb_diffusion_batched_dev(const greb_params* p, int nx, int ny, int batch, const float* T1_dev,
                               const float* wz_dev, float* dX_dev, int strict, int sweeps,
                               void* stream);
int greb_release_caches(void);
int greb_diffusion_launch_order(const greb_params* p, int nx, int ny, int batch, int* field, int* k0, int* k1, int* up,
                                int capacity);
int greb_substep_launch_order(const greb_params* p, int nx, int ny, int n_members, const float* kappa, int* field, int* k0,
                              int* k1, int capacity);

int greb_circulation_launch_plan(const greb_params* p, int nx, int ny, int n_members, const float* kappa, int slots,
                                 int* field, int* k0, int* k1, int* chain, int* dep4, int capacity);

int greb_member_deal_cover(int strict, int* counts);

#define GREB_V_FLUX 1u
#define GREB_V_SWITCHES 2u
#define GREB_V_BUDGET 4u
#define GREB_V_FORCING 8u
#define GREB_V_BOUNDARY 16u
int greb_step_variant(int flux_phase, int switches, int budget, int forced, int on_sets, unsigned* variant);
int greb_step_variants(unsigned* out, int capacity);

int greb_engine_point_physics(greb_engine* e, int ityr, float co2, const float* in5, float* out15);

int greb_ensemble_moments_dev(const float* x_dev, int n_members, size_t n, double* sum_dev, double* sumsq_dev,
                              float* min_dev, float* max_dev, void* stream);
int greb_ensemble_quantiles_dev(const float* x_dev, int n_members, size_t n, const float* probs, int n_probs,
                                float* out_dev, void* stream);

#ifdef __cplusplus
}
#endif
#endif
```

Before: 5689 simulated-years/s.

## Pack per-step boundary forcing into row-interleaved records for the fast member kernel

```diff
diff --git a/greb_climate_model_amd/csrc/greb_device.h b/greb_climate_model_amd/csrc/greb_device.h
--- a/greb_climate_model_amd/csrc/greb_device.h
+++ b/greb_climate_model_amd/csrc/greb_device.h
@@ -356,20 +356,31 @@
 }
 
 template <bool EXACT = true>
-__device__ __forceinline__ void hydro(const Phys& P, float Ts, float q, float u, float v, float z_topo,
-                                      float ez, float swet, float& Qlat, float& Qlat_air, float& dq_eva,
-                                      float& dq_rain, unsigned xsw = 0) {
-#pragma clang fp contract(off)
-  if (xsw & kXNoHydro) { Qlat = Qlat_air = dq_eva = dq_rain = 0.f; return; }
+__device__ __forceinline__ float wind_speed(float u, float v, float z_topo) {
+#pragma clang fp contract(off)
   float abswind = fsqrt<EXACT>(u * u + v * v);
   if (z_topo > 0.f) abswind = fsqrt<EXACT>(abswind * abswind + 2.0f * 2.0f);
   if (z_topo < 0.f) abswind = fsqrt<EXACT>(abswind * abswind + 3.0f * 3.0f);
+  return abswind;
+}
+template <bool EXACT = true>
+__device__ __forceinline__ void hydro_wind(const Phys& P, float Ts, float q, float abswind, float ez, float swet, float& Qlat,
+                                           float& Qlat_air, float& dq_eva, float& dq_rain, unsigned xsw = 0) {
+#pragma clang fp contract(off)
+  if (xsw & kXNoHydro) { Qlat = Qlat_air = dq_eva = dq_rain = 0.f; return; }
   float qs = 3.75e-3f * fexp<EXACT>(fdiv<EXACT>(17.08085f * (Ts - 273.15f), Ts - 273.15f + 234.175f));
   qs = qs * ez;
   Qlat = (q - qs) * abswind * P.cq_latent * P.rho_air * P.ce * swet;
   dq_eva = fdiv<EXACT>(fdiv<EXACT>(-Qlat, P.cq_latent), P.r_qviwv);
   dq_rain = P.cq_rain * q;
   Qlat_air = -dq_rain * P.cq_latent * P.r_qviwv;
+}
+template <bool EXACT = true>
+__device__ __forceinline__ void hydro(const Phys& P, float Ts, float q, float u, float v, float z_topo,
+                                      float ez, float swet, float& Qlat, float& Qlat_air, float& dq_eva,
+                                      float& dq_rain, unsigned xsw = 0) {
+  if (xsw & kXNoHydro) { Qlat = Qlat_air = dq_eva = dq_rain = 0.f; return; }
+  hydro_wind<EXACT>(P, Ts, q, wind_speed<EXACT>(u, v, z_topo), ez, swet, Qlat, Qlat_air, dq_eva, dq_rain, xsw);
 }
 
 template <bool EXACT = true>
diff --git a/greb_climate_model_amd/csrc/greb_engine.cpp b/greb_climate_model_amd/csrc/greb_engine.cpp
--- a/greb_climate_model_amd/csrc/greb_engine.cpp
+++ b/greb_climate_model_amd/csrc/greb_engine.cpp
@@ -144,6 +144,7 @@
     float* dev[kBoundaryFields] = {};
     bool own[kBoundaryFields] = {};
     unsigned over = 0;
+    float* frec = nullptr;
     std::vector<float> t_last, q_last, toclim, z_topo, mld0;
   };
   std::vector<BoundSet> bound;
@@ -205,6 +206,7 @@
   for (unsigned x : e->h_xsw) all &= x;
   if (all) a.nsub = 0;
   if (e->members_on_sets > 0) { a.bsets = e->bsets_dev; a.bset_m = e->bset_dev; }
+  else if (e->bound[0].frec) a.bsets = e->bsets_dev;
   return a;
 }
 
@@ -484,6 +486,24 @@
 enum { kBfZtopo, kBfGlacier, kBfTclim, kBfQclim, kBfUclim, kBfVclim, kBfMld, kBfCld, kBfSwet, kBfToclim, kBfZocean, kBfWzAir, kBfWzVapor };
 size_t boundary_floats(int field, size_t np) { return (field >= kBfTclim && field <= kBfSwet) ? np * kNT : np; }
 
+BoundarySet set_entry(const greb_engine::BoundSet& x) {
+  return BoundarySet{x.dev[0], x.dev[1], x.dev[2], x.dev[3], x.dev[4], x.dev[5], x.dev[6], x.dev[7], x.dev[8], x.dev[9], x.dev[10],
+                     x.dev[11], x.dev[12]};
+}
+bool uses_forcing_records(const greb_engine* e) { return e->fused && !e->strict; }
+hipError_t make_forcing_record(greb_engine* e, const greb_engine::BoundSet& b, BoundarySet* table, size_t id, float** rec,
+                               const char** what) {
+  *rec = nullptr;
+  *what = "hipMalloc of the set's forcing record";
+  hipError_t err = dev_alloc(rec, kFrBytes / sizeof(float));
+  if (err != hipSuccess) { *rec = nullptr; return err; }
+  *what = "packing the set's forcing record";
+  err = launch_pack_forcing(set_entry(b), *rec, e->stream);
+  if (err == hipSuccess) { *what = "hipMemcpy"; err = hipMemcpy(set_table_records(table) + id, rec, sizeof(float*), hipMemcpyHostToDevice); }
+  if (err != hipSuccess) { (void)hipStreamSynchronize(e->stream); (void)hipFree(*rec); *rec = nullptr; }
+  return err;
+}
+
 hipError_t copy_shared_corrections(greb_engine* e, float** corr, const char** what) {
   const size_t nm = (size_t)e->nm, set = (size_t)3 * kNT * e->np;
   hipError_t err = hipStreamSynchronize(e->stream);
@@ -571,6 +591,15 @@
     b0.t_last.assign(f->tclim + last, f->tclim + last + np); b0.q_last.assign(f->qclim + last, f->qclim + last + np);
     b0.toclim = toclim; b0.z_topo.assign(f->z_topo, f->z_topo + np); b0.mld0.assign(f->mldclim, f->mldclim + np);
     e->bound.push_back(std::move(b0));
+  }
+  if (uses_forcing_records(e)) {
+    const BoundarySet own = set_entry(e->bound[0]);
+    HIP_TRY(e, hipMalloc(reinterpret_cast<void**>(&e->bsets_dev), kSetTableBytes));
+    HIP_TRY(e, hipMemset(e->bsets_dev, 0, kSetTableBytes));
+    HIP_TRY(e, hipMemcpy(e->bsets_dev, &own, sizeof(own), hipMemcpyHostToDevice));
+    const char* what = "";
+    const hipError_t err = make_forcing_record(e, e->bound[0], e->bsets_dev, 0, &e->bound[0].frec, &what);
+    if (err != hipSuccess) return fail(e, (int)err, std::string(who) + ": " + what + ": " + hipGetErrorString(err));
   }
 
   e->h_phys.resize(nm);
@@ -808,6 +837,7 @@
                   e->Xa, e->Xb, e->red, e->W2, e->xsw_dev, e->co2_flux_dev, e->diag_out, e->diag_reg, e->clim_out, e->ens_out, e->bsum, e->budget_dev,
                   e->f_space, e->f_season, e->f_solar, e->force_dev, e->bsets_dev, e->bset_dev, e->neutral_force_dev};
   for (void* q : ptrs) if (q) (void)hipFree(q);
+  for (const auto& b : e->bound) if (b.frec) (void)hipFree(b.frec);
   for (size_t k = 1; k < e->bound.size(); ++k)
     for (int i = 0; i < kBoundaryFields; ++i) if (e->bound[k].own[i]) (void)hipFree(e->bound[k].dev[i]);
   for (auto& kv : e->plans) free_plan(kv.second);
@@ -1517,6 +1547,12 @@
   }
   s += "]}";
   {
+    int n = 0;
+    for (const auto& b : e->bound) n += b.frec != nullptr;
+    std::snprintf(buf, sizeof(buf), ", \"forcing_records\": {\"sets\": %d, \"bytes\": %zu}", n, (size_t)n * kFrBytes);
+    s += buf;
+  }
+  {
     unsigned v;
     auto family = [&v](const MemberArgs& a) { return select_variant(a, &v) == hipSuccess ? variant_family(v) : "none"; };
     MemberArgs flux = base_args(e), scenario = base_args(e);
@@ -1780,8 +1816,10 @@
   greb_engine::BoundSet b = e->bound[0];
   for (bool& o : b.own) o = false;
   b.over = mask;
+  b.frec = nullptr;
   auto step = [&](hipError_t err, const char* what) -> int {
     if (err == hipSuccess) return 0;
+    if (b.frec) { (void)hipStreamSynchronize(e->stream); (void)hipFree(b.frec); }
     for (int i = 0; i < kBoundaryFields; ++i) if (b.own[i]) (void)hipFree(b.dev[i]);
     return fail(e, (int)err, std::string(who) + what + ": " + hipGetErrorString(err));
   };
@@ -1806,17 +1844,18 @@
   if (over->qclim) b.q_last.assign(over->qclim + last, over->qclim + last + np);
   if (over->z_topo) b.z_topo.assign(over->z_topo, over->z_topo + np);
   if (over->mldclim) b.mld0.assign(over->mldclim, over->mldclim + np);
-  auto entry = [](const greb_engine::BoundSet& x) {
-    return BoundarySet{x.dev[0], x.dev[1], x.dev[2], x.dev[3], x.dev[4], x.dev[5], x.dev[6], x.dev[7], x.dev[8], x.dev[9], x.dev[10],
-                       x.dev[11], x.dev[12]};
-  };
   BoundarySet* table = e->bsets_dev;
   if (!table) {
-    if (int rc = step(dev_alloc(&table, (size_t)1 + GREB_MAX_BOUNDARY_SETS), "hipMalloc")) return rc;
-    const BoundarySet own = entry(e->bound[0]);
+    if (int rc = step(hipMalloc(reinterpret_cast<void**>(&table), kSetTableBytes), "hipMalloc")) return rc;
+    const BoundarySet own = set_entry(e->bound[0]);
     if (int rc = step(hipMemcpy(table, &own, sizeof(own), hipMemcpyHostToDevice), "hipMemcpy")) { (void)hipFree(table); return rc; }
   }
-  const BoundarySet mine = entry(b);
+  if (uses_forcing_records(e)) {
+    const char* what = "";
+    const hipError_t err = make_forcing_record(e, b, table, e->bound.size(), &b.frec, &what);
+    if (int rc = step(err, what)) return rc;
+  }
+  const BoundarySet mine = set_entry(b);
   if (int rc = step(hipMemcpy(table + e->bound.size(), &mine, sizeof(mine), hipMemcpyHostToDevice), "hipMemcpy")) {
     if (!e->bsets_dev) (void)hipFree(table);
     return rc;
@@ -2048,6 +2087,48 @@
 int greb_member_deal_cover(int strict, int* counts) {
   if (!counts) return fail(nullptr, GREB_E_INVALID, "member_deal_cover: bad argument");
   member_deal_cover(strict != 0, counts);
+  return 0;
+}
+
+static_assert(GREB_FORCING_RECORD_FIELDS == kFrFields, "the record's field count mirrors the ABI");
+
+long long greb_forcing_record_offset(int row, int field, int lon) {
+  if (row < 0 || row >= kFrNy || field < 0 || field >= kFrFields || lon < 0 || lon >= kFrNx) return -1;
+  return (long long)forcing_record_offset(row, field, lon);
+}
+
+long long greb_forcing_record_field_bytes(int field) {
+  if (field < 0 || field >= kFrFields) return -1;
+  return (long long)(forcing_record_offset(0, field, 0) * sizeof(float));
+}
+
+int greb_forcing_record_field_static(int field) { return (field < 0 || field >= kFrFields) ? -1 : (field < kFrStaticFields ? 1 : 0); }
+
+long long greb_forcing_record_static_floats(void) { return (long long)kFrStaticFloats; }
+
+long long greb_forcing_record_step_floats(void) { return (long long)kFrStepFloats; }
+
+long long greb_forcing_record_bytes(void) { return (long long)kFrBytes; }
+
+const char* greb_forcing_record_field_name(int field) {
+  static const char* const names[kFrFields] = {"z_topo", "glacier", "z_ocean", "wz_air", "tclim", "cldclim", "mldclim", "mldclim_prev",
+                                               "swetclim", "wind_speed"};
+  return (field < 0 || field >= kFrFields) ? nullptr : names[field];
+}
+
+int greb_engine_get_forcing_record(greb_engine* e, int set, int step, float* out) {
+  const char* who = "get_forcing_record: ";
+  if (!e) return fail(nullptr, GREB_E_INVALID, std::string(who) + "no engine (greb_engine is NULL)");
+  if (!out || set < 0 || set >= (int)e->bound.size() || step < 1 || step > kNT)
+    return fail(e, GREB_E_INVALID, std::string(who) + "bad argument (set 0 ... sets made, step 1 ... 730)");
+  if (!e->bound[(size_t)set].frec)
+    return fail(e, GREB_E_UNSUPPORTED, std::string(who) + "this engine keeps no forcing records (they belong to the FAST fused member kernel)");
+  HIP_TRY(e, hipSetDevice(e->device));
+  HIP_TRY(e, hipStreamSynchronize(e->stream));
+  const float* rec = e->bound[(size_t)set].frec;
+  HIP_TRY(e, hipMemcpy(out, rec, kFrStaticFloats * sizeof(float), hipMemcpyDeviceToHost));
+  HIP_TRY(e, hipMemcpy(out + kFrStaticFloats, rec + kFrStaticFloats + (size_t)(step - 1) * kFrStepFloats, kFrStepFloats * sizeof(float),
+                       hipMemcpyDeviceToHost));
   return 0;
 }
 
diff --git a/greb_climate_model_amd/csrc/greb_kernels.h b/greb_climate_model_amd/csrc/greb_kernels.h
--- a/greb_climate_model_amd/csrc/greb_kernels.h
+++ b/greb_climate_model_amd/csrc/greb_kernels.h
@@ -37,6 +37,20 @@
 constexpr int kBoundaryFields = 13;
 constexpr int kBoundaryInputs = 9;
 constexpr int kMaxBoundarySets = 16;
+
+constexpr int kFrNx = 96, kFrNy = 48;
+enum { kFrZtopo, kFrGlacier, kFrZocean, kFrWzAir, kFrStaticFields,
+       kFrTclim = kFrStaticFields, kFrCld, kFrMld, kFrMldPrev, kFrSwet, kFrWind, kFrFields };
+constexpr int kFrStepFields = kFrFields - kFrStaticFields;
+constexpr unsigned forcing_record_offset(int row, int field, int lon) {
+  return field < kFrStaticFields ? ((unsigned)row * kFrStaticFields + (unsigned)field) * kFrNx + (unsigned)lon
+                                 : ((unsigned)row * kFrStepFields + (unsigned)(field - kFrStaticFields)) * kFrNx + (unsigned)lon;
+}
+constexpr unsigned kFrStaticFloats = forcing_record_offset(kFrNy, 0, 0), kFrStepFloats = forcing_record_offset(kFrNy, kFrStaticFields, 0);
+constexpr size_t kFrBytes = ((size_t)kFrStaticFloats + (size_t)kNT * kFrStepFloats) * sizeof(float);
+static_assert(forcing_record_offset(0, kFrFields - 1, 0) * sizeof(float) <= 4095 && forcing_record_offset(0, kFrStaticFields - 1, 0) * sizeof(float) <= 4095,
+              "a field's offset must fit the immediate of a global load");
+static_assert(kFrBytes < (1ull << 31), "offsets into a record are 32-bit");
 
 struct MemberArgs {
   int nx, ny, np;
@@ -81,6 +95,10 @@
   const int* bset_m;
 };
 
+constexpr int kSetTableEntries = kMaxBoundarySets + 1;
+constexpr size_t kSetTableBytes = kSetTableEntries * (sizeof(BoundarySet) + sizeof(const float*));
+inline const float** set_table_records(BoundarySet* table) { return (const float**)(table + kSetTableEntries); }
+
 enum { kBsw, kBLWsurf, kBLWdown, kBLWabs, kBQsens, kBQlat, kBQlatAir, kBdqEva, kBdqRain, kBdTocean, kBdTo, kBdTaCrcl, kBdqCrcl, kNBudget };
 
 enum : unsigned { kVFlux = 1, kVExp = 2, kVBudget = 4, kVForce = 8, kVBound = 16 };
@@ -122,6 +140,7 @@
 bool member_layout_supported(const RowTables& tab, int nx, int ny);
 void member_deal_cover(bool strict, int* counts);
 hipError_t launch_member_kernel(const MemberArgs& a, int n_members, bool strict, hipStream_t s);
+hipError_t launch_pack_forcing(const BoundarySet& b, float* rec, hipStream_t s);
 hipError_t launch_circulation_g96(const float* X, const float* wz, const float* u, const float* v, float* dX,
                                   const RowTables* tab_dev, int batch, int nsub, bool strict, hipStream_t s);
 
diff --git a/greb_climate_model_amd/csrc/greb_member.hip b/greb_climate_model_amd/csrc/greb_member.hip
--- a/greb_climate_model_amd/csrc/greb_member.hip
+++ b/greb_climate_model_amd/csrc/greb_member.hip
@@ -730,6 +730,9 @@
     const float co2 = FLUX ? co2_flux : a.co2[(size_t)m * a.co2_stride + a.co2_year0 + yr_rel];
     const MemberForce mf = member_force<FORCE>(a, m, ck);
     const BoundPtr B = member_boundary<BOUND>(a, bset);
+    constexpr int ROUTE = STRICT ? kRouteArrays : kRouteRecord;
+    const float* rec = nullptr;
+    if constexpr (!STRICT) rec = member_record(a, bset);
     lfloat* Xf = lds + kOffX + cur * XB;
     lfloat* red = lds + kOffX + (cur ^ 1) * XB;
     if constexpr (BUDGET) {
@@ -737,8 +740,8 @@
 #pragma unroll 1
       for (int qd = tid; qd < NP / 4; qd += kThreads) {
         const q8 xpair = ld8(Xf + (qd / NQ) * RS, qd % NQ);
-        const PhysIn in = physics_load<V>(a, qd, ck, state, acc, corr, xsw, mf, B);
-        (void)physics_compute<STRICT, V | kVBudget>(a, P, in, co2, comp(xpair, 0), comp(xpair, 1), xsw, bs, 4 * qd, mf);
+        const PhysIn in = physics_load<V, ROUTE>(a, qd, ck, state, acc, corr, xsw, mf, B, rec);
+        (void)physics_compute<STRICT, V | kVBudget, ROUTE>(a, P, in, co2, comp(xpair, 0), comp(xpair, 1), xsw, bs, 4 * qd, mf);
       }
     }
 #pragma unroll 1
@@ -748,7 +751,7 @@
 #endif
       const q8 xpair = ld8(Xf + (qd / NQ) * RS, qd % NQ);
       f4 oTa, oq, tsm;
-      physics_quad<STRICT, V & ~kVBudget>(a, P, m, qd, ck, co2, state, acc, corr, comp(xpair, 0), comp(xpair, 1), oTa, oq, tsm, xsw, mf, B);
+      physics_quad<STRICT, V & ~kVBudget, ROUTE>(a, P, m, qd, ck, co2, state, acc, corr, comp(xpair, 0), comp(xpair, 1), oTa, oq, tsm, xsw, mf, B, rec);
       st8(Xf + (qd / NQ) * RS, qd % NQ, zip(oTa, oq));
       if (ityr == kNT) st4(red + 4 * qd, tsm);
     }
@@ -799,11 +802,40 @@
 #endif
 }
 
+static_assert(kFrNx == NX && kFrNy == NY, "the forcing record is the fused kernel's grid");
+__global__ __launch_bounds__(256) void pack_forcing_kernel(BoundarySet b, float* __restrict__ rec) {
+  const unsigned i = blockIdx.x * 256u + threadIdx.x;
+  if (i >= (unsigned)kNT * NP) return;
+  const unsigned step = i / NP, p = i - step * NP, row = p / NX, lon = p - row * NX;
+  const unsigned prev = step > 0 ? step - 1 : kNT - 1;
+  const float zt = b.z_topo[p];
+  if (step == 0) {
+    float* o = rec + forcing_record_offset((int)row, 0, (int)lon);
+    o[forcing_record_offset(0, kFrZtopo, 0)] = zt;
+    o[forcing_record_offset(0, kFrGlacier, 0)] = b.glacier[p];
+    o[forcing_record_offset(0, kFrZocean, 0)] = b.z_ocean[p];
+    o[forcing_record_offset(0, kFrWzAir, 0)] = b.wz_air[p];
+  }
+  float* o = rec + kFrStaticFloats + (size_t)step * kFrStepFloats + forcing_record_offset((int)row, kFrStaticFields, (int)lon);
+  o[forcing_record_offset(0, kFrTclim, 0)] = b.tclim[i];
+  o[forcing_record_offset(0, kFrCld, 0)] = b.cldclim[i];
+  o[forcing_record_offset(0, kFrMld, 0)] = b.mldclim[i];
+  o[forcing_record_offset(0, kFrMldPrev, 0)] = b.mldclim[(size_t)prev * NP + p];
+  o[forcing_record_offset(0, kFrSwet, 0)] = b.swetclim[i];
+  o[forcing_record_offset(0, kFrWind, 0)] = wind_speed<false>(b.uclim[i], b.vclim[i], zt);
+}
+
+hipError_t launch_pack_forcing(const BoundarySet& b, float* rec, hipStream_t s) {
+  hipLaunchKernelGGL(pack_forcing_kernel, dim3((kNT * NP + 255) / 256), dim3(256), 0, s, b, rec);
+  return hipGetLastError();
+}
+
 template <bool STRICT, unsigned V>
 struct MemberFamily { static auto kernel() { return &member_kernel<STRICT, V>; } };
 
 hipError_t launch_member_kernel(const MemberArgs& a, int n_members, bool strict, hipStream_t s) {
   if (a.nx != NX || a.ny != NY) return hipErrorInvalidValue;
+  if (!strict && !a.bsets) return hipErrorInvalidValue;
   unsigned v;
   if (hipError_t e = select_variant(a, &v); e != hipSuccess) return e;
   const auto kern = pick_variant<MemberFamily>(strict, v);
diff --git a/greb_climate_model_amd/csrc/greb_physics_step.h b/greb_climate_model_amd/csrc/greb_physics_step.h
--- a/greb_climate_model_amd/csrc/greb_physics_step.h
+++ b/greb_climate_model_amd/csrc/greb_physics_step.h
@@ -74,10 +74,21 @@
 }
 #define GREB_BF(f) (BOUND ? (const float*)B->f : a.f)
 
+enum { kRouteArrays, kRouteRecord };
+__device__ __forceinline__ const float* member_record(const MemberArgs& a, int bset) {
+  unsigned long long p = (unsigned long long)((const float* const*)(a.bsets + kSetTableEntries) + bset);
+  asm volatile("" : "+s"(p));
+  return *(const float* const __attribute__((address_space(4)))*)p;
+}
+__device__ __forceinline__ const float* at_bytes(const float* base, unsigned boff) { return (const float*)((const char*)base + boff); }
+__device__ __forceinline__ float* at_bytes(float* base, unsigned boff) { return (float*)((char*)base + boff); }
+__device__ __forceinline__ unsigned opaque_v(unsigned x) { asm("" : "+v"(x)); return x; }
+
 struct PhysIn {
   f4 Ts, Ta, To, q, cap;
   f4 zt, gl, zo, ez;
   f4 tcl, cld, mld, mldm, swet, u, v;
+  f4 wind;
   f4 c0, c1, c2;
   f4 acc0, acc1, acc2, acc3, acc4, acc5;
   f4 qcl, tclp;
@@ -90,11 +101,63 @@
 };
 
 template <unsigned V>
+__device__ __forceinline__ PhysIn physics_load_record(const MemberArgs& a, int qd, const StepClock& ck, const float* __restrict__ state,
+                                                      const float* __restrict__ acc, const float* __restrict__ corr, unsigned xsw_member,
+                                                      const MemberForce& F, BoundPtr B, const float* __restrict__ rec) {
+  constexpr bool FLUX = V & kVFlux, EXP = V & kVExp, FORCE = V & kVForce, BOUND = V & kVBound;
+  constexpr int NQ = kFrNx / 4, np = kFrNx * kFrNy;
+  const int row = qd / NQ;
+  const size_t off = ck.off, offm = ck.offm;
+  const unsigned xsw = EXP ? xsw_member : 0u;
+  const unsigned bo = opaque_v(16u * (unsigned)qd);
+  const unsigned lon4 = 4u * (unsigned)(qd - row * NQ);
+  const unsigned ro_static = opaque_v((forcing_record_offset(row, 0, 0) + lon4) * 4u);
+  const unsigned ro = opaque_v((forcing_record_offset(row, kFrStaticFields, 0) + lon4) * 4u);
+  const float* slice = rec + kFrStaticFloats + (size_t)(ck.ityr - 1) * kFrStepFloats;
+  auto fr = [&](int field) {
+    return ld4(at_bytes(field < kFrStaticFields ? rec : slice, field < kFrStaticFields ? ro_static : ro) + forcing_record_offset(0, field, 0));
+  };
+  PhysIn i;
+  i.Ts = ld4(at_bytes(state, bo)); i.Ta = ld4(at_bytes(state + np, bo)); i.To = ld4(at_bytes(state + 2 * np, bo));
+  i.q = ld4(at_bytes(state + 3 * np, bo)); i.cap = ld4(at_bytes(state + 4 * np, bo));
+  i.zt = fr(kFrZtopo); i.gl = fr(kFrGlacier); i.zo = fr(kFrZocean); i.ez = fr(kFrWzAir);
+  i.tcl = fr(kFrTclim); i.cld = fr(kFrCld); i.mld = fr(kFrMld); i.mldm = fr(kFrMldPrev); i.swet = fr(kFrSwet); i.wind = fr(kFrWind);
+  const unsigned so = opaque_v(4u * (unsigned)row);
+  if (FORCE) {
+#pragma clang fp contract(off)
+    i.solar = *at_bytes(F.solar + (size_t)(ck.ityr - 1) * kFrNy, so) * F.scale;
+  } else i.solar = *at_bytes(a.sw_solar + (size_t)(ck.ityr - 1) * kFrNy, so);
+  if (FLUX) { i.c0 = ld4(at_bytes(GREB_BF(toclim), bo)); i.c1 = ld4(at_bytes(GREB_BF(qclim) + off, bo)); i.c2 = zero4(); }
+  else {
+    i.c0 = ld4(at_bytes(corr + off, bo)); i.c1 = ld4(at_bytes(corr + (size_t)kNT * np + off, bo));
+    i.c2 = ld4(at_bytes(corr + (size_t)2 * kNT * np + off, bo));
+  }
+  i.acc0 = i.acc1 = i.acc2 = i.acc3 = i.acc4 = zero4();
+#ifdef GREB_TUNING
+  const bool no_acc = a.dbg & 1;
+#else
+  constexpr bool no_acc = false;
+#endif
+  i.acc5 = no_acc ? zero4() : ld4(at_bytes(acc + 5 * np, bo));
+  if (!FLUX && !no_acc) {
+    i.acc0 = ld4(at_bytes(acc, bo)); i.acc1 = ld4(at_bytes(acc + np, bo)); i.acc2 = ld4(at_bytes(acc + 2 * np, bo));
+    i.acc3 = ld4(at_bytes(acc + 3 * np, bo)); i.acc4 = ld4(at_bytes(acc + 4 * np, bo));
+  }
+  i.qcl = zero4(); i.tclp = zero4();
+  if (EXP && (xsw & kXLwLinear)) i.qcl = FLUX ? i.c1 : ld4(at_bytes(GREB_BF(qclim) + off, bo));
+  if (EXP && !FLUX && (xsw & kXSstPlus1)) i.tclp = ld4(at_bytes(GREB_BF(tclim) + offm, bo));
+  i.fw = zero4();
+  if (FORCE && F.space) i.fw = ld4(at_bytes(F.space, bo));
+  return i;
+}
+
+template <unsigned V, int ROUTE = kRouteArrays>
 __device__ __forceinline__ PhysIn physics_load(const MemberArgs& a, int qd, const StepClock& ck, const float* __restrict__ state,
                                                const float* __restrict__ acc, const float* __restrict__ corr, unsigned xsw_member,
-                                               const MemberForce& F, BoundPtr B) {
+                                               const MemberForce& F, BoundPtr B, const float* __restrict__ rec = nullptr) {
   constexpr bool FLUX = V & kVFlux, EXP = V & kVExp, FORCE = V & kVForce, BOUND = V & kVBound;
   static_assert(variant_valid(V), "no such variant of the step kernels");
+  if constexpr (ROUTE == kRouteRecord) return physics_load_record<V>(a, qd, ck, state, acc, corr, xsw_member, F, B, rec);
   const int nx = a.nx, ny = a.ny, np = a.np, p0 = 4 * qd;
   const size_t off = ck.off, offm = ck.offm;
   const unsigned xsw = EXP ? xsw_member : 0u;
@@ -161,7 +224,7 @@
   }
 }
 
-template <bool STRICT, unsigned V>
+template <bool STRICT, unsigned V, int ROUTE = kRouteArrays>
 __device__ __forceinline__ PhysOut physics_compute(const MemberArgs& a, const Phys& P, const PhysIn& in, float co2, const f4& xTa,
                                                    const f4& xq, unsigned xsw_member, const BudgetSink& bs, int p0,
                                                    const MemberForce& F) {
@@ -192,7 +255,8 @@
     budget_add<BUDGET>(bs, np, kBLWabs, p0 + e, LWabs);
     const float Qsens = P.ct_sens * (Ta1 - Ts1);
     budget_add<BUDGET>(bs, np, kBQsens, p0 + e, Qsens);
-    hydro<STRICT>(P, Ts1, q1, in.u.v[e], in.v.v[e], zt, ez, in.swet.v[e], Qlat, Qlat_air, dq_eva, dq_rain, xsw);
+    if constexpr (ROUTE == kRouteRecord) hydro_wind<STRICT>(P, Ts1, q1, in.wind.v[e], ez, in.swet.v[e], Qlat, Qlat_air, dq_eva, dq_rain, xsw);
+    else hydro<STRICT>(P, Ts1, q1, in.u.v[e], in.v.v[e], zt, ez, in.swet.v[e], Qlat, Qlat_air, dq_eva, dq_rain, xsw);
     budget_add<BUDGET>(bs, np, kBQlat, p0 + e, Qlat); budget_add<BUDGET>(bs, np, kBQlatAir, p0 + e, Qlat_air);
     budget_add<BUDGET>(bs, np, kBdqEva, p0 + e, dq_eva); budget_add<BUDGET>(bs, np, kBdqRain, p0 + e, dq_rain);
     deep_ocean<STRICT>(P, Ts1, To1, zt, mld, in.mldm.v[e], in.zo.v[e], dT_ocean, dTo, xsw);
@@ -233,9 +297,62 @@
 }
 
 template <bool FLUX>
+__device__ __forceinline__ void physics_store_record(const MemberArgs& a, int m, int qd, const StepClock& ck,
+                                                     const PhysOut& o, float* __restrict__ state, float* __restrict__ acc,
+                                                     float* __restrict__ corr, f4& tsmn_mean) {
+  constexpr int np = kFrNx * kFrNy;
+  const int mon = ck.mon;
+  const size_t off = ck.off;
+  const unsigned bo = opaque_v(16u * (unsigned)qd);
+#ifdef GREB_TUNING
+  const bool no_acc = a.dbg & 1, no_wb = a.dbg & 2;
+#else
+  constexpr bool no_acc = false, no_wb = false;
+#endif
+  if (!no_wb) {
+    st4(at_bytes(state, bo), o.Ts); st4(at_bytes(state + np, bo), o.Ta); st4(at_bytes(state + 2 * np, bo), o.To);
+    st4(at_bytes(state + 3 * np, bo), o.q); st4(at_bytes(state + 4 * np, bo), o.cap);
+  }
+  if (FLUX) {
+    st4(at_bytes(corr + off, bo), o.TF); st4(at_bytes(corr + (size_t)kNT * np + off, bo), o.qF);
+    st4(at_bytes(corr + (size_t)2 * kNT * np + off, bo), o.ToF);
+  } else {
+#pragma clang fp contract(off)
+    f4 s0 = o.s0, s1 = o.s1, s2 = o.s2, s3 = o.s3, s4 = o.s4;
+    if (mon >= 0) {
+      const float ndm = (float)(kMonthDays[mon] * 2);
+      float* rec = a.monthly + (((size_t)m * a.monthly_years + (a.year_out0 + ck.yr_rel)) * 12 + mon) * 5 * np;
+      f4 r0, r1, r2, r3, r4;
+#pragma unroll
+      for (int e = 0; e < 4; ++e) {
+        r0.v[e] = s0.v[e] / ndm; r1.v[e] = s1.v[e] / ndm; r2.v[e] = s2.v[e] / ndm; r3.v[e] = s3.v[e] / ndm; r4.v[e] = s4.v[e] / ndm;
+      }
+      st4_nt(at_bytes(rec, bo), r0); st4_nt(at_bytes(rec + np, bo), r1); st4_nt(at_bytes(rec + 2 * np, bo), r2);
+      st4_nt(at_bytes(rec + 3 * np, bo), r3); st4_nt(at_bytes(rec + 4 * np, bo), r4);
+      s0 = s1 = s2 = s3 = s4 = zero4();
+    }
+    if (!no_acc) {
+      st4(at_bytes(acc, bo), s0); st4(at_bytes(acc + np, bo), s1); st4(at_bytes(acc + 2 * np, bo), s2);
+      st4(at_bytes(acc + 3 * np, bo), s3); st4(at_bytes(acc + 4 * np, bo), s4);
+    }
+  }
+  if (ck.ityr == kNT) {
+#pragma clang fp contract(off)
+    f4 t;
+#pragma unroll
+    for (int e = 0; e < 4; ++e) t.v[e] = o.tsmn.v[e] / (float)kNT;
+    tsmn_mean = t;
+    if (!no_acc) st4(at_bytes(acc + 5 * np, bo), zero4());
+  } else {
+    if (!no_acc) st4(at_bytes(acc + 5 * np, bo), o.tsmn);
+  }
+}
+
+template <bool FLUX, int ROUTE = kRouteArrays>
 __device__ __forceinline__ void physics_store(const MemberArgs& a, int m, int qd, const StepClock& ck,
                                               const PhysOut& o, float* __restrict__ state, float* __restrict__ acc,
                                               float* __restrict__ corr, f4& tsmn_mean) {
+  if constexpr (ROUTE == kRouteRecord) { physics_store_record<FLUX>(a, m, qd, ck, o, state, acc, corr, tsmn_mean); return; }
   const int np = a.np, p0 = 4 * qd, mon = ck.mon;
   const size_t off = ck.off;
 #ifdef GREB_TUNING
@@ -277,15 +394,16 @@
   }
 }
 
-template <bool STRICT, unsigned V>
+template <bool STRICT, unsigned V, int ROUTE = kRouteArrays>
 __device__ __forceinline__ void physics_quad(const MemberArgs& a, const Phys& P, int m, int qd, const StepClock& ck,
                                              float co2, float* __restrict__ state, float* __restrict__ acc,
                                              float* __restrict__ corr, const f4& xTa, const f4& xq, f4& oTa_out,
-                                             f4& oq_out, f4& tsmn_mean, unsigned xsw, const MemberForce& F, BoundPtr B) {
+                                             f4& oq_out, f4& tsmn_mean, unsigned xsw, const MemberForce& F, BoundPtr B,
+                                             const float* __restrict__ rec = nullptr) {
   constexpr bool FLUX = V & kVFlux, BUDGET = V & kVBudget;
-  const PhysIn in = physics_load<V>(a, qd, ck, state, acc, corr, xsw, F, B);
-  const PhysOut o = physics_compute<STRICT, V>(a, P, in, co2, xTa, xq, xsw, budget_sink<BUDGET>(a, m, ck), 4 * qd, F);
-  physics_store<FLUX>(a, m, qd, ck, o, state, acc, corr, tsmn_mean);
+  const PhysIn in = physics_load<V, ROUTE>(a, qd, ck, state, acc, corr, xsw, F, B, rec);
+  const PhysOut o = physics_compute<STRICT, V, ROUTE>(a, P, in, co2, xTa, xq, xsw, budget_sink<BUDGET>(a, m, ck), 4 * qd, F);
+  physics_store<FLUX, ROUTE>(a, m, qd, ck, o, state, acc, corr, tsmn_mean);
   oTa_out = o.Ta; oq_out = o.q;
 }
 #undef GREB_BF
diff --git a/greb_climate_model_amd/engine.py b/greb_climate_model_amd/engine.py
--- a/greb_climate_model_amd/engine.py
+++ b/greb_climate_model_amd/engine.py
@@ -54,7 +54,10 @@
            "greb_member_deal_cover", "greb_engine_set_forcing_tables", "greb_engine_set_member_forcing",
            "greb_engine_add_boundary_set", "greb_engine_set_member_boundary", "greb_step_variant", "greb_step_variants",
            "greb_clim_create", "greb_clim_destroy", "greb_clim_add_year_dev", "greb_clim_finish_dev", "greb_engine_run_clim",
-           "greb_ens_create", "greb_ens_destroy", "greb_ens_reduce_dev", "greb_engine_run_ens"]
+           "greb_ens_create", "greb_ens_destroy", "greb_ens_reduce_dev", "greb_engine_run_ens",
+           "greb_forcing_record_offset", "greb_forcing_record_field_bytes", "greb_forcing_record_step_floats",
+           "greb_forcing_record_bytes", "greb_forcing_record_field_name", "greb_engine_get_forcing_record",
+           "greb_forcing_record_field_static", "greb_forcing_record_static_floats"]
 
 
 def _check(rc: int, h=None):
@@ -338,6 +341,14 @@
             raise GrebError(-1, f"set_member_boundary: {self.nm} set ids expected")
         _check(lib().greb_engine_set_member_boundary(self.h, ids.ctypes.data_as(C.POINTER(C.c_int32)), C.c_uint(flags)), self.h)
 
+    def forcing_record(self, step: int, set_id: int = 0) -> np.ndarray:
+        lay = forcing_record_layout()
+        out = np.empty(lay.static_floats + lay.step_floats, np.float32)
+        _check(lib().greb_engine_get_forcing_record(self.h, int(set_id), int(step), abi.fptr(out)), self.h)
+        ns = sum(lay.static)
+        return np.concatenate([out[:lay.static_floats].reshape(lay.ny, ns, lay.nx),
+                               out[lay.static_floats:].reshape(lay.ny, len(lay.names) - ns, lay.nx)], axis=1)
+
     def point_physics(self, ityr: int, co2: float, in5) -> np.ndarray:
         in5 = np.ascontiguousarray(in5, np.float32)
         out = np.empty((15, self.ny, self.nx), np.float32)
@@ -408,6 +419,30 @@
     return out
 
 
+class RecordLayout:
+
+    def __init__(self, names, static, offsets, field_bytes, static_floats, step_floats, record_bytes):
+        self.names, self.static, self.offsets, self.field_bytes = names, static, offsets, field_bytes
+        self.static_floats, self.step_floats, self.record_bytes = static_floats, step_floats, record_bytes
+        self.ny, _, self.nx = offsets.shape
+
+
+def forcing_record_layout(nx: int = 96, ny: int = 48) -> RecordLayout:
+    L = lib()
+    for f in (L.greb_forcing_record_offset, L.greb_forcing_record_field_bytes, L.greb_forcing_record_static_floats,
+              L.greb_forcing_record_step_floats, L.greb_forcing_record_bytes):
+        f.restype = C.c_longlong
+    L.greb_forcing_record_field_name.restype = C.c_char_p
+    names = []
+    while L.greb_forcing_record_field_name(len(names)) is not None:
+        names.append(L.greb_forcing_record_field_name(len(names)).decode())
+    nf = len(names)
+    off = np.array([[[L.greb_forcing_record_offset(k, f, i) for i in range(nx)] for f in range(nf)] for k in range(ny)], np.int64)
+    return RecordLayout(tuple(names), tuple(bool(L.greb_forcing_record_field_static(f)) for f in range(nf)), off,
+                        [int(L.greb_forcing_record_field_bytes(f)) for f in range(nf)], int(L.greb_forcing_record_static_floats()),
+                        int(L.greb_forcing_record_step_floats()), int(L.greb_forcing_record_bytes()))
+
+
 def step_variant(flux_phase=False, switches=False, budget=False, forced=False, on_sets=False):
     v = C.c_uint(0xFFFFFFFF)
     rc = lib().greb_step_variant(int(bool(flux_phase)), int(bool(switches)), int(bool(budget)), int(bool(forced)),
diff --git a/include/greb_engine.h b/include/greb_engine.h
--- a/include/greb_engine.h
+++ b/include/greb_engine.h
@@ -199,6 +199,16 @@
 
 int greb_member_deal_cover(int strict, int* counts);
 
+#define GREB_FORCING_RECORD_FIELDS 10
+int greb_forcing_record_field_static(int field);
+long long greb_forcing_record_offset(int row, int field, int lon);
+long long greb_forcing_record_field_bytes(int field);
+long long greb_forcing_record_static_floats(void);
+long long greb_forcing_record_step_floats(void);
+long long greb_forcing_record_bytes(void);
+const char* greb_forcing_record_field_name(int field);
+int greb_engine_get_forcing_record(greb_engine* e, int set, int step, float* out);
+
 #define GREB_V_FLUX 1u
 #define GREB_V_SWITCHES 2u
 #define GREB_V_BUDGET 4u
```

Measured after the change: 5879 simulated-years/s (median of 6 runs). 3.3% higher.
